# avikde/robobee3d

Measured on AMD Instinct MI355X. Metric: closed-loop MPC steps/sec (QP+dyn), higher is better.
Workload: dtype f32

## Files before the change

### robobee3d_amd/_lib.py

```python
import ctypes as C
import os
import subprocess

HERE = os.path.dirname(os.path.abspath(__file__))
ROOT = os.path.dirname(HERE)
SO_PATH = os.path.join(HERE, "libumpc_mi355x.so")
SRC = os.path.join(HERE, "csrc", "umpc_mi355x.hip")
SRC_BQP = os.path.join(HERE, "csrc", "umpc_bqp.hip")
OBJ_DIR = os.path.join(HERE, "csrc", "_obj")
HIPCC_FLAGS = ["--offload-arch=gfx950", "-O3", "-ffp-contract=off", "-fPIC", "-std=c++17"]

UMPC_F32, UMPC_F64 = 0, 1
STATE_ROWS, CTRL_ROWS, REF_ROWS, OUT_ROWS, STAT_ROWS = 18, 127, 9, 9, 2
NX, NC, NADATA = 45, 39, 48

EXPORTS = ["umpcInit", "umpcUpdate", "umpcS", "umpcLastStatus", "umpcRelease", "umpcLiveControllers", "umpcSetCompat",
           "umpcBatchDefaultParams", "umpcBatchCreate", "umpcBatchDestroy", "umpcBatchInitCtrl",
           "umpcBatchRollout", "umpcBatchUpdate", "umpcBatchPlant", "umpcBatchAssemble",
           "umpcBatchSize", "umpcBatchDtype", "umpcAxIdx", "umpcKKTPerm", "umpcNnzL",
           "umpcBatchSetTask", "umpcBatchTime", "umpcBatchSetWeights", "umpcBatchSetStepKernel", "umpcBatchSetGlobalBatch", "umpcBatchGlobalBatch", "umpcBatchReactive", "umpcBatchTaskReference",
           "umpcBatchSetRefTrajectory", "umpcBatchRefCursor", "umpcBatchTaskTable", "umpcBatchSetHistory", "umpcBatchHistoryCursor",
           "umpcBatchSetImpulses", "umpcBatchImpulseCursor",
           "umpcLastError", "umpcKernelName", "umpcBatchKernelName", "wlConInit", "wlConUpdate", "wlconS", "umpcBatchWLUpdate", "umpcBatchSetWL", "umpcBatchModel",
           "umpcQPDefaultSettings", "umpcQPCreate", "umpcQPDestroy", "umpcQPSetMaxIter", "umpcQPSetCheckTermination", "umpcQPSetAdaptiveRho", "umpcQPUseTables", "umpcQPSetKernel", "umpcQPKernelName", "umpcQPSolve", "umpcQPGather", "umpcQPGatherUpdate",
           "umpcP5fStep", "umpcP5fStepU", "umpcP5fLinearise", "umpcP5fTick", "umpcNAssemble", "umpcNExtract"]


class NParams(C.Structure):
    _fields_ = [(k, C.c_double) for k in ("dt", "g", "TtoWmax", "ws", "wds", "wpr", "wpf", "wvr", "wvf", "wthrust",
                                          "wmom")] + [("Ib", C.c_double * 3)]


class QPSettings(C.Structure):
    _fields_ = [(k, C.c_double) for k in ("rho", "sigma", "alpha", "eps_abs", "eps_rel", "eps_prim_inf",
                                          "eps_dual_inf")] + [("max_iter", C.c_int), ("scaling", C.c_int),
                                                              ("check_termination", C.c_int), ("adaptive_rho_interval", C.c_int)]


class FunApprox_t(C.Structure):
    _fields_ = [("k", C.c_int), ("a0", C.c_float), ("a1", C.c_float * 4), ("A2", C.c_float * 16)]

# ... 54 lines not shown
    limits = json.load(open(RESOURCE_LIMITS))
    for pat, lim in limits.items():
        hits = [k for k in res if pat in k]
        if not hits:
            raise RuntimeError("resource check: no kernel matches %r" % pat)
        for k in hits:
            r = res[k]
            for key, op in (("VGPRs", "=="), ("AGPRs", "=="), ("LDS", "=="), ("ScratchSize", "<=")):
                if key in lim and key not in r:
                    raise RuntimeError("resource check: %s missing for %s (hipcc remark format changed?)" % (key, k))
                if key in lim and not (r[key] == lim[key] if op == "==" else r[key] <= lim[key]):
                    raise RuntimeError("resource check failed for %s: %s = %d, recorded %s %d (csrc/resource_limits.json)"
                                       % (k, key, r[key], op, lim[key]))
    return res


def build(force=False, verbose=False):
    from . import asmgen, asmgen64, asmstep, codegen, codegen_n3, codegen_qp
    sw = asmgen.generator_switches()
    if sw and os.environ.get("UMPC_VARIANT_ROOT") != ROOT:
        raise RuntimeError("generator switches are set in the environment (%s): refusing to regenerate the shipped kernels; "
                           "unset them, or build a variant with tools/build_variant.py" % " ".join("%s=%s" % kv for kv in sw.items()))
    gen, _ = codegen.write()
    gn3 = codegen_n3.write()
    gasm, _ = asmgen.write()
    gasm64 = asmgen64.write()[0]
    gasm64q = asmgen64.write_quad()[0]
    gstep, _ = asmstep.write()
    gquad, _ = asmstep.write(quad=True)
    greg, gqp_units = codegen_qp.write()
    hdr = os.path.join(ROOT, "include", "umpc_mi355x.h")
    csrc = os.path.join(HERE, "csrc")
    units = [(SRC, [gen, gasm, gasm64, gasm64q, gstep, gquad, gn3, hdr] + [os.path.join(csrc, f) for f in ("umpc_step.h", "umpc_models.h", "umpc_err.h")]),
             (SRC_BQP, [hdr, greg, os.path.join(csrc, "umpc_bqp_common.h"), os.path.join(csrc, "umpc_err.h")])]
    gen_hdrs = [os.path.join(csrc, "gen", f) for f in os.listdir(os.path.join(csrc, "gen")) if f.endswith(".h")]
    units += [(u, [os.path.join(csrc, "umpc_bqp_common.h")] + gen_hdrs) for u in gqp_units]
    os.makedirs(OBJ_DIR, exist_ok=True)
    objs, relink = [], force or not os.path.exists(SO_PATH)
    todo = []
    for src, deps in units:
        obj = os.path.join(OBJ_DIR, os.path.basename(src) + ".o")
        objs.append(obj)
        if (force or not os.path.exists(obj)
                or any(os.path.getmtime(obj) < os.path.getmtime(d) for d in [src] + deps)):
            extra = ["-Rpass-analysis=kernel-resource-usage"] if src == SRC else []
            todo.append(["hipcc"] + HIPCC_FLAGS + extra + ["-c", "-o", obj, src])
            relink = True
    step_obj = os.path.join(OBJ_DIR, os.path.basename(SRC) + ".o")
    if not any(c[-1] == SRC for c in todo):
        import json
        try:
            _validate_resources(json.load(open(RESOURCES_JSON)))
        except Exception:
            todo.insert(0, ["hipcc"] + HIPCC_FLAGS + ["-Rpass-analysis=kernel-resource-usage", "-c", "-o", step_obj, SRC])
            relink = True
    for stale in set(os.listdir(OBJ_DIR)) - {os.path.basename(o) for o in objs} - {os.path.basename(RESOURCES_JSON)}:
        os.remove(os.path.join(OBJ_DIR, stale))
    running, width = [], max(1, min(len(todo), os.cpu_count() or 1))
    while todo or running:
        while todo and len(running) < width:
            cmd = todo.pop(0)
            if verbose:
                print(" ".join(cmd))
            running.append((cmd, subprocess.Popen(cmd, cwd=csrc, stderr=subprocess.PIPE)))
        cmd, p = running.pop(0)
        _, err = p.communicate()
        if p.returncode != 0:
# ... 84 lines not shown
        L.umpcBatchTime.argtypes = [C.c_void_p]
        L.umpcBatchTime.restype = C.c_double
        L.umpcBatchModel.argtypes = [C.c_int, C.c_int, C.c_int, C.c_int, C.c_double] + [C.c_void_p] * 4
        L.umpcBatchWLUpdate.argtypes =[C.POINTER(WLCon_t), C.c_int, C.c_int] + [C.c_void_p] * 5
        L.umpcBatchSetWL.argtypes = [C.c_void_p, C.POINTER(WLCon_t), C.POINTER(C.c_double), C.c_void_p, C.c_void_p]
        L.umpcUpdate.restype = C.c_int
        L.umpcQPDefaultSettings.argtypes = [C.POINTER(QPSettings)]
        L.umpcQPCreate.restype = C.c_void_p
        L.umpcQPCreate.argtypes = [C.c_void_p, C.c_int, C.c_int, C.c_int, C.POINTER(QPSettings)]
        L.umpcQPDestroy.argtypes = [C.c_void_p]
        L.umpcQPSetMaxIter.argtypes = [C.c_void_p, C.c_int]
        L.umpcQPSetCheckTermination.argtypes = [C.c_void_p, C.c_int]
        L.umpcQPSetAdaptiveRho.argtypes = [C.c_void_p, C.c_int]
        L.umpcQPUseTables.argtypes = [C.c_void_p, C.c_int]
        L.umpcQPSetKernel.argtypes = [C.c_void_p, C.c_int]
        L.umpcQPKernelName.argtypes = [C.c_void_p]
        L.umpcQPKernelName.restype = C.c_char_p
        L.umpcQPSolve.argtypes = [C.c_void_p] * 15
        L.umpcQPGather.argtypes = [C.c_int, C.c_int, C.c_int] + [C.c_void_p] * 5
        L.umpcQPGatherUpdate.argtypes = [C.c_int, C.c_int, C.c_int] + [C.c_void_p] * 5
        L.umpcP5fStep.argtypes = [C.c_int, C.c_int, C.c_int, C.c_double] + [C.c_void_p] * 4
        L.umpcP5fStepU.argtypes = [C.c_int, C.c_int, C.c_int, C.c_double, C.c_double] + [C.c_void_p] * 3
        L.umpcP5fLinearise.argtypes = [C.c_int, C.c_int, C.c_void_p, C.c_double, C.c_void_p, C.c_void_p, C.c_int, C.c_void_p,
                                       C.c_void_p, C.c_void_p, C.c_int, C.c_void_p]
        L.umpcP5fTick.argtypes = [C.c_void_p] * 14 + [C.c_double, C.c_double, C.c_void_p, C.c_void_p, C.c_int, C.c_void_p, C.c_void_p, C.c_void_p]
        L.umpcNAssemble.argtypes = [C.c_int, C.c_int, C.c_int, C.POINTER(NParams)] + [C.c_void_p] * 10
        L.umpcNExtract.argtypes = [C.c_int, C.c_int, C.c_int, C.c_double] + [C.c_void_p] * 5
        L.umpcLastStatus.restype = C.c_int
        L.umpcSetCompat.restype = C.c_int
        _lib = L
    return _lib


def default_params():
    p = BatchParams()
    lib().umpcBatchDefaultParams(C.byref(p))
    return p
```

### robobee3d_amd/asmgen.py

```python
import os
import struct

from . import symbolic

HERE = os.path.dirname(os.path.abspath(__file__))

SWITCH_PREFIXES = ("UMPC_ASM_", "UMPC_ASM64_", "UMPC_QP_", "UMPC_X_")
NOT_SWITCHES = ("UMPC_QP_KERNEL", "UMPC_QP_NO_ASM", "UMPC_ASM_SKEW_US", "UMPC_ASM_SKEW_GROUPS")


def generator_switches():
    return {k: v for k, v in sorted(os.environ.items()) if k.startswith(SWITCH_PREFIXES) and k not in NOT_SWITCHES}


def switch_banner():
    sw = generator_switches()
    return "// generator switches: " + (" ".join("%s=%s" % kv for kv in sw.items()) if sw else "none (defaults = the shipped kernels)")

XV_COUNT, XV_BASE = 0, 246
NLDS = 160
NVZ = 36
FAC_L, FAC_DI, FAC_Q, FAC_LOEQ, FAC_M = 0, 213, 297, 342, 378
FAC_ROWS = 390
WS_DS, WS_ES, WS_C, WS_XPREV, WS_DY = 390, 435, 474, 475, 520
WS_ROWS = 559

V_W, V_WZ, V_X, V_Y, V_Z = 2, 48, 88, 134, 174
V_RING, V_AT, V_TT, V_END = 214, 230, 238, 246
N_ATP = 4
NRING = 4


def ring_base(slot):
    return V_RING + 4 * slot if slot < 4 else 246 + 4 * (slot - 4)
A_L, A_D, A_Q, A_LO, A_M = 0, 53, 137, 182, 218
S_WS, S_CTRL, S_STRIDE, S_ITERS = 4, 6, 10, 11
S_P, S_CNT, S_P2 = 12, 14, 16
S_ALPHA, S_OMA, S_SIGMA, S_RINV, S_RHO = 20, 22, 24, 26, 28


def f32bits(v):
    return struct.unpack("<I", struct.pack("<f", v))[0]


def _vgprs(x):
    if not isinstance(x, str):
        return set()
    x = x.strip("-|")
    if x.startswith("v[") and x.endswith("]"):
        lo, hi = x[2:-1].split(":")
        return set(range(int(lo), int(hi) + 1))
    if x.startswith("v") and x[1:].isdigit():
        return {int(x[1:])}
    return set()


WIDE_STORES = {"ds_write_b128": 2, "ds_write_b96": 2, "global_store_dwordx4": 2, "global_store_dwordx3": 2}
WIDE_STORE_WAIT = 2


def valu_dst(t):
    m = t[0]
    if not m.startswith("v_") or m.startswith("v_cmp") or m in ("v_accvgpr_write_b32", "v_readfirstlane_b32", "v_readlane_b32"):
        return set()
    return _vgprs(t[1])


def wide_store_hazards(ins):
    out = []
    for k, t in enumerate(ins):
        if t[0] in WIDE_STORES:
            data = _vgprs(t[WIDE_STORES[t[0]]])
            ws, j = 0, k + 1
            while j < len(ins) and ws < WIDE_STORE_WAIT:
                u = ins[j]
                if u[0] == "label":
                    j += 1
                    continue
                if u[0] == "s_nop":
                    ws += int(u[1]) + 1
                elif valu_dst(u) & data:
                    out.append((k, j))
                    ws += 1
                else:
                    ws += 1
                j += 1
    return out


class Emit:

    def __init__(self):
        self.ins = []

    def __call__(self, *t):
        dst = valu_dst(t)
        if dst:
            ws = 0
            for u in reversed(self.ins[-(WIDE_STORE_WAIT + 1):]):
                if ws >= WIDE_STORE_WAIT or u[0] == "label":
                    break
                if u[0] in WIDE_STORES and _vgprs(u[WIDE_STORES[u[0]]]) & dst:
                    self.ins.append(("s_nop", WIDE_STORE_WAIT - ws - 1))
                    break
                ws += int(u[1]) + 1 if u[0] == "s_nop" else 1
        self.ins.append(t)


def _row_ptr(e, sreg, base, row):
    e("s_mul_i32", "s%d" % sreg, "s%d" % S_STRIDE, row)
    e("s_mul_hi_u32", "s%d" % (sreg + 1), "s%d" % S_STRIDE, row)
    e("s_add_u32", "s%d" % sreg, "s%d" % sreg, "s%d" % base)
    e("s_addc_u32", "s%d" % (sreg + 1), "s%d" % (sreg + 1), "s%d" % (base + 1))


def _adv(e, sreg):
    e("s_add_u32", "s%d" % sreg, "s%d" % sreg, "s%d" % S_STRIDE)
    e("s_addc_u32", "s%d" % (sreg + 1), "s%d" % (sreg + 1), 0)


def slot_maps(s):
    def one(n, ntrip):
        sl = list(range(n))
        for t in range(ntrip):
            st = 3 * t
            if st % 2:
                sl[st], sl[st + 1], sl[st + 2] = st + 1, st + 2, st
        return sl
    ntrip = 4 * s.N
    xs, zs = one(s.nx, ntrip), one(s.nc, ntrip)
    xinv, zinv = [0] * s.nx, [0] * s.nc
    for j, p in enumerate(xs):
# ... 110 lines not shown
    units = []
    k = 0
    while k < len(fwd):
        g = fwd[k]
        if len(g) == 1 and g[0][2] in couples and k + 1 < len(fwd) and len(fwd[k + 1]) == 1 and fwd[k + 1][0][2] == couples[g[0][2]]:
            units.append([g[0][2], fwd[k + 1][0][2]])
            k += 2
        else:
            units.append([o[2] for o in g])
            k += 1
    order, pending = [], []
    for u in units:
        if len(u) == 2 and len(order) % 2:
            pending.append(u)
            continue
        order += u
        while pending and len(order) % 2 == 0:
            order += pending.pop(0)
    assert not pending, "odd number of single entries before a trailing pair"
    pos = [0] * len(s.L_i)
    for p_, j in enumerate(order):
        pos[j] = p_
    for g in fwd + bwd:
        if len(g) == 2:
            a, b = pos[g[0][2]], pos[g[1][2]]
            assert a // 2 == b // 2, "paired entries must share an aligned pair"
    return fwd, bwd, pos


def l_positions(N=3, perm=None):
    return solve_plan(symbolic.analyse(N, perm))[2]


def prologue(e, s):
    import numpy as np
    for reg, val in ((S_ALPHA, 1.6), (S_OMA, float(np.float32(1.0) - np.float32(1.6))), (S_SIGMA, 1e-6),
                     (S_RINV, 0.01), (S_RHO, 100.0)):
        e("s_mov_b32", "s%d" % reg, f32bits(val))
        e("s_mov_b32", "s%d" % (reg + 1), f32bits(val))
    _row_ptr(e, S_P, S_WS, FAC_L + NLDS)
    nrest = len(s.L_i) - NLDS + s.nk + s.nx + 2 * s.N * symbolic.NY + 12
    assert A_LO == nrest - 12 - 2 * s.N * symbolic.NY and A_M == nrest - 12 and nrest <= 256
    for r in range(nrest):
        e("global_load_dword", "a%d" % r, "v0", "s[%d:%d]" % (S_P, S_P + 1))
        _adv(e, S_P)
    e("s_mov_b64", "s[%d:%d]" % (S_P, S_P + 1), "s[%d:%d]" % (S_CTRL, S_CTRL + 1))
    xs, zs, _, _ = slot_maps(s)
    for base, n, sl in ((V_X, s.nx, xs), (V_Y, s.nc, zs), (V_Z, s.nc, zs)):
        for r in range(n):
            e("global_load_dword", "v%d" % (base + sl[r]), "v0", "s[%d:%d]" % (S_P, S_P + 1))
            _adv(e, S_P)
    e("s_waitcnt", "vmcnt(0)")


def epilogue(e, s, z_is_l):
    w = 0
    xs, zs, _, _ = slot_maps(s)
    neq = 2 * s.N * symbolic.NY
    for base, n, sl in ((V_X, s.nx, xs), (V_Y, s.nc, zs), (V_Z, s.nc, zs)):
        for r in range(n):
            if base == V_Z and z_is_l and r < neq:
                t = V_RING + r % 16
                e("v_accvgpr_read_b32", "v%d" % t, "a%d" % (A_LO + r))
                e("ds_write_b32", "v1", "v%d" % t, (w // 4) * 1024 + (w % 4) * 4)
            else:
                e("ds_write_b32", "v1", "v%d" % (base + sl[r]), (w // 4) * 1024 + (w % 4) * 4)
            w += 1
    e("s_waitcnt", "vmcnt(0) lgkmcnt(0)")


class Fetcher:

    def __init__(self, e, la=3):
        self.e, self.la = e, la
        self.nds = 0
        self.waited = -1
        self.lds_ahead = int(os.environ.get("UMPC_ASM_LDS_AHEAD", "12" if NRING == 4 else "20"))
        self.merge = int(os.environ.get("UMPC_ASM_LDS_MERGE", "1" if NRING == 4 else "2"))

    def run(self, ops):
        e = self.e
        n = len(ops)
        inst_of = [None] * n
        insts = []
        slots = [None] * NRING
        for i, op in enumerate(ops):
            if op["src"] and op["src"][0] == "L":
                qd = op["src"][1] // 4
                hit = [k for k in slots if k is not None and insts[k]["quad"] == qd]
                if hit:
                    insts[hit[0]]["last"] = i
                    inst_of[i] = hit[0]
                    continue
                free = [sl for sl in range(NRING) if slots[sl] is None]
                sl = free[0] if free else min(range(NRING), key=lambda q: insts[slots[q]]["last"])
                insts.append(dict(quad=qd, first=i, last=i, slot=sl, prev=slots[sl], issued=None))
                slots[sl] = len(insts) - 1
                inst_of[i] = slots[sl]

        def issue(it):
            e("ds_read_b128", "v[%d:%d]" % (ring_base(it["slot"]), ring_base(it["slot"]) + 3), "v1",
              it["quad"] * 1024)
            it["issued"] = self.nds
            self.nds += 1

        next_inst = 0
        atemp = {}
        next_acc = 0
        acc_rr = 0
        for i in range(n):
            while next_acc < n and next_acc < i + self.la:
                op = ops[next_acc]
                if op["src"] and op["src"][0] in ("A", "A2"):
                    t = V_AT + 2 * (acc_rr % N_ATP)
                    acc_rr += 1
                    e("v_accvgpr_read_b32", "v%d" % t, "a%d" % op["src"][1])
                    if op["src"][0] == "A2":
                        e("v_accvgpr_read_b32", "v%d" % (t + 1), "a%d" % op["src"][2])
                    atemp[next_acc] = t
                next_acc += 1
            while next_inst < len(insts):
                it = insts[next_inst]
                prev = insts[it["prev"]] if it["prev"] is not None else None
                if it["first"] <= i + self.lds_ahead and (prev is None or prev["last"] < i):
                    issue(it)
                    next_inst += 1
                else:
                    break
            op = ops[i]
            if op["src"] is None:
                op["emit"](None)
            elif op["src"][0] in ("A", "A2"):
                op["emit"](atemp.pop(i))
            else:
                it = insts[inst_of[i]]
                if it["issued"] is None:
                    assert inst_of[i] == next_inst and (it["prev"] is None or insts[it["prev"]]["last"] < i)
                    issue(it)
                    next_inst += 1
                if it["first"] == i and it["issued"] > self.waited:
                    upto = min(self.nds - 1, it["issued"] + self.merge)
                    e("s_waitcnt", "lgkmcnt(%d)" % min(15, self.nds - 1 - upto))
                    self.waited = upto if self.nds - 1 - upto <= 15 else it["issued"]
                op["emit"](ring_base(it["slot"]) + op["src"][1] % 4)


def _vp(n):
    assert n % 2 == 0
# ... 9 lines not shown
    assert n % 2 == 0
    return ("s[%d:%d]" % (n, n + 1), 0, 0)


def pk(e, mnem, dst, srcs, neg=None):
    assert dst % 2 == 0
    neg = neg or [0] * len(srcs)
    mods = dict(op_sel=[s_[1] for s_ in srcs], op_sel_hi=[s_[2] for s_ in srcs], neg_lo=list(neg), neg_hi=list(neg))
    e(mnem, "v[%d:%d]" % (dst, dst + 1), *[s_[0] for s_ in srcs], mods)


def despace(ops, window=int(os.environ.get("UMPC_ASM_WINDOW", "12"))):
    pending, out = list(ops), []
    last = [frozenset(), frozenset()]
    while pending:
        best, bscore = 0, None
        blocked_w, blocked_r = set(), set()
        for k, o in enumerate(pending[:window]):
            movable = not (o["r"] & blocked_w) and not (o["w"] & blocked_w) and not (o["w"] & blocked_r)
            if movable:
                score = (2 if (o["r"] | o["w"]) & last[1] else 0) + (1 if (o["r"] | o["w"]) & last[0] else 0)
                if bscore is None or score < bscore:
                    best, bscore = k, score
                    if score == 0:
                        break
            blocked_w |= o["w"]
            blocked_r |= o["r"]
        o = pending.pop(best)
        out.append(o)
        last = [last[1], o["w"]]
    return out


def body(e, s, first, capture, plan, lv=False, delta_in_w=False, qzero=frozenset(), lzero=frozenset(), dy3_in_w=False):
    nx, nc, nk = s.nx, s.nc, s.nk
    neq = 2 * s.N * symbolic.NY
    xs, zs, xinv, zinv = slot_maps(s)
    fwd, bwd, lpos = plan

    def wreg(k):
        return w_reg(s, k, xs, zs)
    W = lambda k: "v%d" % wreg(k)
    WX = lambda j: V_W + xs[j]
    WZ = lambda i: V_WZ + zs[i]
    XR = lambda j: V_X + xs[j]
    YR = lambda i: V_Y + zs[i]
    ZR = lambda i: V_Z + zs[i]
    X = lambda j: "v%d" % XR(j)
    Y = lambda i: "v%d" % YR(i)
    Z = lambda i: "v%d" % ZR(i)
    v = lambda n: "v%d" % n
    sA, sO, sS, sRi, sRh = ("s%d" % r for r in (S_ALPHA, S_OMA, S_SIGMA, S_RINV, S_RHO))
    ptr = "s[%d:%d]" % (S_P2, S_P2 + 1)
    f = Fetcher(e)
    ops = []

    def op(src, fn, w=(), r=()):
        ops.append(dict(src=src, emit=fn, w=frozenset(w), r=frozenset(r)))

    assert NVZ == neq and not (lv and first)

    def l_src(j):
        if lpos[j] < NLDS:
            return ("L", lpos[j])
        if lv and lpos[j] < NLDS + NVZ:
            return ("V", V_Z + lpos[j] - NLDS)
        if NLDS + NVZ <= lpos[j] < NLDS + NVZ + XV_COUNT:
            return ("V", XV_BASE + lpos[j] - NLDS - NVZ)
        return ("A", A_L + lpos[j] - NLDS)

    if capture and not delta_in_w:
        _row_ptr(e, S_P2, S_WS, WS_XPREV)
        for j in range(nx):
            e("global_store_dword", "v0", X(j), ptr)
            _adv(e, S_P2)
    for p_ in range(0, nx - 1, 2):
        j0, j1 = xinv[p_], xinv[p_ + 1]
        rw = dict(w=(V_W + p_, V_W + p_ + 1), r=(V_X + p_, V_X + p_ + 1))
        if j0 in qzero and j1 in qzero:
            op(None, lambda t, p_=p_: pk(e, "v_pk_mul_f32", V_W + p_, [_sb(S_SIGMA), _vp(V_X + p_)]), **rw)
        elif j0 in qzero or j1 in qzero:
            jn, h = (j1, 1) if j0 in qzero else (j0, 0)

            def mixed(t, p_=p_, h=h):
                pk(e, "v_pk_mul_f32", V_W + p_, [_sb(S_SIGMA), _vp(V_X + p_)])
                e("v_sub_f32", v(V_W + p_ + h), v(V_W + p_ + h), v(t))
            op(("A", A_Q + jn), mixed, **rw)
        else:
            op(("A2", A_Q + j0, A_Q + j1),
               lambda t, p_=p_: pk(e, "v_pk_fma_f32", V_W + p_, [_sb(S_SIGMA), _vp(V_X + p_), _vp(t)], [0, 0, 1]), **rw)
    if nx % 2:
        jl = xinv[nx - 1]
        if jl in qzero:
# ... 24 lines not shown
        op(("A", A_M + 9 + i - neq), lambda t, i=i: e("v_fma_f32", v(WZ(i)), "-" + v(t), Y(i), Z(i)),
           w=(WZ(i),), r=(YR(i), ZR(i)))

    def solve_ops(sched):
        for g in sched:
            if len(g) == 1:
                d, sr, j = g[0]
                src = l_src(j)
                if src[0] == "V":
                    op(None, lambda t, d=d, sr=sr, r=src[1]: e("v_fmac_f32", W(d), v(r), W(sr)),
                       w=(wreg(d),), r=(wreg(d), wreg(sr)))
                else:
                    op(src, lambda t, d=d, sr=sr: e("v_fmac_f32", W(d), v(t), W(sr)),
                       w=(wreg(d),), r=(wreg(d), wreg(sr)))
                continue
            (d0, s0_, j0), (d1, s1_, j1) = g
            rd, r0, r1 = wreg(d0), wreg(s0_), wreg(s1_)
            assert rd % 2 == 0 and wreg(d1) == rd + 1 and r0 // 2 == r1 // 2 and lpos[j0] // 2 == lpos[j1] // 2
            srcp = ("v[%d:%d]" % (r0 - r0 % 2, r0 - r0 % 2 + 1), r0 % 2, r1 % 2)
            rw = dict(w=(rd, rd + 1), r=(rd, rd + 1, r0, r1))
            pe = lpos[j0] - lpos[j0] % 2
            lsel = (lpos[j0] % 2, lpos[j1] % 2)
            if pe < NLDS:
                op(("L", pe), lambda t, rd=rd, srcp=srcp, lsel=lsel:
                   pk(e, "v_pk_fma_f32", rd, [("v[%d:%d]" % (t, t + 1), lsel[0], lsel[1]), srcp, _vp(rd)], [0, 0, 0]), **rw)
            elif (lv and pe < NLDS + NVZ) or NLDS + NVZ <= pe < NLDS + NVZ + XV_COUNT:
                t = V_Z + pe - NLDS if pe < NLDS + NVZ else XV_BASE + pe - NLDS - NVZ
                op(None, lambda _t, t=t, rd=rd, srcp=srcp, lsel=lsel:
                   pk(e, "v_pk_fma_f32", rd, [("v[%d:%d]" % (t, t + 1), lsel[0], lsel[1]), srcp, _vp(rd)], [0, 0, 0]), **rw)
            else:
                src = ("A2", A_L + lpos[j0] - NLDS, A_L + lpos[j1] - NLDS)
                op(src, lambda t, rd=rd, srcp=srcp: pk(e, "v_pk_fma_f32", rd, [_vp(t), srcp, _vp(rd)], [0, 0, 0]), **rw)

    solve_ops(fwd)
    kof = {wreg(k): k for k in range(nk)}
    for r0 in range(V_W, V_Z, 2):
        k0, k1 = kof.get(r0), kof.get(r0 + 1)
        if k0 is not None and k1 is not None:
            op(("A2", A_D + k0, A_D + k1), lambda t, r0=r0: pk(e, "v_pk_mul_f32", r0, [_vp(r0), _vp(t)]),
               w=(r0, r0 + 1), r=(r0, r0 + 1))
        elif k0 is not None or k1 is not None:
            k, r = (k0, r0) if k0 is not None else (k1, r0 + 1)
            op(("A", A_D + k), lambda t, r=r: e("v_mul_f32", v(r), v(t), v(r)), w=(r,), r=(r,))
    solve_ops(bwd)
    f.run(despace(ops) if os.environ.get("UMPC_ASM_DESPACE", "0") == "1" else ops)
    for p_ in range(0, nx - 1, 2):
        t = V_TT + 2 * ((p_ // 2) % 4)
        pk(e, "v_pk_mul_f32", t, [_sb(S_OMA), _vp(V_X + p_)])
        if capture and delta_in_w:
            pk(e, "v_pk_fma_f32", t, [_sb(S_ALPHA), _vp(V_W + p_), _vp(t)])
            pk(e, "v_pk_add_f32", V_W + p_, [_vp(t), _vp(V_X + p_)], [0, 1])
            e("v_pk_mov_b32", "v[%d:%d]" % (V_X + p_, V_X + p_ + 1), "v[%d:%d]" % (t, t + 1), "v[%d:%d]" % (t, t + 1),
              dict(op_sel=[0, 1], op_sel_hi=[0, 0], neg_lo=[0, 0], neg_hi=[0, 0]))
        else:
            pk(e, "v_pk_fma_f32", V_X + p_, [_sb(S_ALPHA), _vp(V_W + p_), _vp(t)])
    if nx % 2:
        jl = xinv[nx - 1]
        e("v_mul_f32", v(V_TT), sO, X(jl))
        if capture and delta_in_w:
            e("v_fma_f32", v(V_TT), sA, v(WX(jl)), v(V_TT))
            e("v_sub_f32", v(WX(jl)), v(V_TT), X(jl))
            e("v_mov_b32", X(jl), v(V_TT))
        else:
            e("v_fma_f32", X(jl), sA, v(WX(jl)), v(V_TT))
    if capture and first and not delta_in_w:
        _row_ptr(e, S_P2, S_WS, WS_DY)
    if not first:
        for p_ in range(0, neq, 2):
            t = V_TT + 2 * ((p_ // 2) % 2)
            pk(e, "v_pk_add_f32", t, [_vp(V_WZ + p_), _vp(V_Y + p_)], [0, 1])
            if capture and delta_in_w:
                pk(e, "v_pk_mul_f32", V_WZ + p_, [_sb(S_ALPHA), _vp(t)])
            elif capture:
                pk(e, "v_pk_mul_f32", t + 4, [_sb(S_ALPHA), _vp(t)])
                for h in range(2):
                    _row_ptr(e, S_P2, S_WS, WS_DY + zinv[p_ + h])
                    e("global_store_dword", "v0", v(t + 4 + h), ptr)
            pk(e, "v_pk_fma_f32", V_Y + p_, [_sb(S_ALPHA), _vp(t), _vp(V_Y + p_)])
# ... 27 lines not shown
            e("v_fma_f32", t3, rinv, Y(i), t1)
            e("v_max_f32", t3, t3, v(V_AT + 2))
            e("v_min_f32", Z(i), t3, v(V_AT + 3))
            e("v_sub_f32", t2, t1, Z(i))
        if dy3_in_w and not eq and not capture:
            e("v_mul_f32", nu, rho, t2)
            e("v_add_f32", Y(i), Y(i), nu)
            continue
        e("v_mul_f32", t2, rho, t2)
        e("v_add_f32", Y(i), Y(i), t2)
        if capture and delta_in_w:
            e("v_mov_b32", nu, t2)
        elif capture:
            if not first:
                _row_ptr(e, S_P2, S_WS, WS_DY + i)
            e("global_store_dword", "v0", t2, ptr)
            if first:
                _adv(e, S_P2)


def program(N=3, perm=None):
    s = symbolic.analyse(N, perm)
    plan = solve_plan(s)
    e = Emit()
    prologue(e, s)
    e("s_cmp_lt_i32", "s%d" % S_ITERS, 1)
    e("s_cbranch_scc1", "9f")
    body(e, s, first=True, capture=True, plan=plan)
    for p_ in range(NVZ):
        e("v_accvgpr_read_b32", "v%d" % (V_Z + p_), "a%d" % (A_L + p_))
    e("s_sub_i32", "s%d" % S_CNT, "s%d" % S_ITERS, 2)
    e("s_cmp_lt_i32", "s%d" % S_CNT, 1)
    e("s_cbranch_scc1", "8f")
    e("label", "7")
    body(e, s, first=False, capture=False, plan=plan, lv=True)
    e("s_sub_i32", "s%d" % S_CNT, "s%d" % S_CNT, 1)
    e("s_cmp_gt_i32", "s%d" % S_CNT, 0)
    e("s_cbranch_scc1", "7b")
    e("label", "8")
    e("s_cmp_lt_i32", "s%d" % S_ITERS, 2)
    e("s_cbranch_scc1", "6f")
    body(e, s, first=False, capture=True, plan=plan, lv=True)
    e("label", "6")
    epilogue(e, s, z_is_l=True)
    e("s_branch", "5f")
    e("label", "9")
    epilogue(e, s, z_is_l=False)
    e("label", "5")
    return e.ins, s


def fmt(t):
    m = t[0]
    if m == "label":
        return "%s:" % t[1]
    mods = ""
    if isinstance(t[-1], dict):
        d = t[-1]
        t = t[:-1]
        mods = " " + " ".join("%s:[%s]" % (k, ",".join(map(str, d[k]))) for k in ("op_sel", "op_sel_hi", "neg_lo", "neg_hi"))
    a = [("0x%x" % x if (m == "s_mov_b32" and isinstance(x, int)) else str(x)) for x in t[1:]]
    if m in ("ds_read_b128", "ds_write_b128", "ds_write_b32"):
        return "%s %s, %s offset:%s" % (m, a[0], a[1], a[2])
    if m in ("global_load_dword", "global_store_dword"):
        return "%s %s, %s, %s" % (m, a[0], a[1], a[2])
    if m == "s_waitcnt":
        return "s_waitcnt " + " ".join(a)
    return "%s %s%s" % (m, ", ".join(a), mods)


def write(path=None, N=3, perm=None):
    path = path or os.path.join(HERE, "csrc", "umpc_admm_asm.h")
    ins, s = program(N, perm)
    lpos = solve_plan(s)[2]
    store_l = " ".join("LDSW_(%d) = -LX_(%d);" % (lpos[j], j) if lpos[j] < NLDS else "ROW_(%d) = -LX_(%d);" % (FAC_L + lpos[j], j)
                       for j in range(len(lpos)))
    used_s = [S_P, S_P + 1, S_CNT, S_P2, S_P2 + 1] + list(range(S_ALPHA, S_RHO + 2))
    clob = ['"memory"', '"scc"', '"vcc"'] + ['"v%d"' % i for i in range(2, V_END)] + \
           ['"a%d"' % i for i in range(256)] + ['"s%d"' % i for i in used_s]
    lab7 = [k for k, t in enumerate(ins) if t == ("label", "7")][0]
    lab8 = [k for k, t in enumerate(ins) if t == ("label", "8")][0]
    out = ["// GENERATED by robobee3d_amd/asmgen.py -- do not edit.", switch_banner(),
           "// ADMM phase of the fp32 step kernel: %d instructions, middle-iteration body %d." % (len(ins), lab8 - lab7),
           "#pragma once",
           "namespace umpcasm {",
           "constexpr int FAC_L = %d, FAC_DI = %d, FAC_Q = %d, FAC_LOEQ = %d, FAC_M = %d, FAC_ROWS = %d;" %
           (FAC_L, FAC_DI, FAC_Q, FAC_LOEQ, FAC_M, FAC_ROWS),
           "constexpr int WS_DS = %d, WS_ES = %d, WS_C = %d, WS_XPREV = %d, WS_DY = %d, WS_ROWS = %d;" %
           (WS_DS, WS_ES, WS_C, WS_XPREV, WS_DY, WS_ROWS),
           "constexpr int LDS_BYTES_PER_LANE = %d;" % (NLDS * 4),
           "}  // namespace umpcasm",
           "// Phase A -> loop hand-off of the factor: entry j of L (CSC order) goes NEGATED to its storage position (asmgen.solve_plan):",
           "// LDS word LDSW_(p) for p < %d, workspace row ROW_(FAC_L + p) (-> AGPR) otherwise." % NLDS,
           "#define UMPC_ASM_STORE_L(LDSW_, ROW_, LX_) do { %s } while (0)" % store_l,
           "// inputs: v0 = 4*robot, v1 = lane LDS address, s[4:5] = workspace, s[6:7] = ctrl, s10 = 4*B, s11 = maxIter",
           "#define UMPC_ADMM_ASM(voff, ldsaddr, ws, ctrl, stride, iters) asm volatile( \\"]
    for t in ins:
        out.append('  "%s\\n" \\' % fmt(t))
    out.append('  : : "{v0}"(voff), "{v1}"(ldsaddr), "{s[4:5]}"(ws), "{s[6:7]}"(ctrl), "{s10}"(stride), "{s11}"(iters) \\')
    out.append("  : " + ", ".join(clob) + ")")
    txt = "\n".join(out) + "\n"
    old = open(path).read() if os.path.exists(path) else None
    if old != txt:
        with open(path, "w") as fh:
            fh.write(txt)
    return path, len(ins)
# ... 19 lines not shown
```

### robobee3d_amd/asmstep.py

```python
import os
import struct

from . import asmgen, symbolic
from .asmgen import (A_D, A_L, A_LO, A_M, A_Q, NLDS, NVZ, S_ALPHA, S_CNT, S_ITERS, S_OMA, S_RHO, S_RINV, S_SIGMA,
                     V_W, V_WZ, V_X, V_Y, V_Z, Emit, f32bits, pk, _sb, _vp)

HERE = os.path.dirname(os.path.abspath(__file__))

PTRS = ["state", "ctrl", "ref", "ws", "out", "stats", "status", "info", "Ib", "gain", "aT0",
        "taskf", "weights", "wl", "wlu", "wlw",
        "done"]
NPTR_RES = 11
INTS = ["stride", "K", "maxIter", "nsub", "plant", "seq"]
TAIL_INTS = ["refstep"]
FLOATS = ["dt", "dtg", "Tmax", "wpr", "wpf", "ws_", "wvr", "wvf", "wds", "wthrust", "wmom",
          "iwpr", "iwpf", "iws", "iwvr", "iwvf", "iwds", "iwthrust", "iwmom",
          "Ib0", "Ib1", "Ib2", "Ibi0", "Ibi1", "Ibi2", "h", "hh", "h6", "taulim", "gpl", "idt", "mbg"]
WNAMES = ["wpr", "wpf", "ws_", "wvr", "wvf", "wds", "wthrust", "wmom"]
WROW = {"ws_": 0, "wds": 1, "wpr": 2, "wpf": 3, "wvr": 4, "wvf": 5, "wthrust": 6, "wmom": 7}
A_W, A_IW = 230, 238
S_PARAM = 4
S_PBLK = 2
S_PTR = {n: 40 + 2 * k for k, n in enumerate(PTRS[:NPTR_RES])}
S_PTR["taskf"], S_PTR["weights"] = 0, 96
S_PTR["wl"], S_PTR["wlu"], S_PTR["wlw"] = 30, 32, 34
S_INT = {"stride": 10, "K": 13, "maxIter": S_ITERS, "nsub": 5, "plant": 39}
S_F = {n: 64 + k for k, n in enumerate(FLOATS)}
assert max(S_F.values()) <= 95
S_STEP, S_SUB, S_RUIZ = 12, 15, 15
S_MBAD, S_MP0 = 62, 14
S_M0, S_M1, S_M2, S_M3 = 30, 32, 34, 36
S_C = {"minscal": 16, "maxscal": 17, "c45": 18, "eps10": 19, "eps": 38, "rho": 6, "rinv": 7, "rmin": 8,
       "rmininv": 9, "infty_ms": 100, "rhotol": 101}
S_TMP = 4
OFF = {}
_o = 0
for _n in PTRS:
    OFF[_n] = _o
    _o += 8
for _n in INTS + FLOATS + TAIL_INTS:
    OFF[_n] = _o
    _o += 4
PARAM_BYTES = _o
HIST_INTS = ["statestep", "outstep", "statusstep", "infostep"]
HIST_OFF = (PARAM_BYTES + 7) // 8 * 8
for _k, _n in enumerate(HIST_INTS):
    OFF[_n] = HIST_OFF + 4 * _k
HIST_BYTES = 4 * len(HIST_INTS)
S_HIST = 32
IMP_OFF = HIST_OFF + HIST_BYTES
assert IMP_OFF % 8 == 0
OFF["imp"], OFF["impstep"] = IMP_OFF, IMP_OFF + 8
IMP_BYTES = 16
S_IMP = 32

VFIRST, VEND = 2, 256
XV_N, XV_B = 10, 246
OPT_RING = int(os.environ.get("UMPC_ASM_RING", "6"))
assert OPT_RING in (4, 6)
OPT_XV = os.environ.get("UMPC_ASM_XV", "1") == "1"
if OPT_RING == 6:
    XV_N, XV_B = 2, 254
OPT_LIMIT_FAST = os.environ.get("UMPC_ASM_LIMIT_FAST", "0") == "1"
OPT_ZSKIP = os.environ.get("UMPC_ASM_ZSKIP", "1") == "1"
OPT_NT = os.environ.get("UMPC_ASM_NT", "1")
NT_PTRS = ("state", "ctrl", "ref", "out", "stats")
# ... 882 lines not shown
                e("v_mul_f32", v(t), v(src[i]), v(RE(i)))
                e("v_accvgpr_write_b32", "a%d" % (A_LO + i), v(t))
            elif i == 5 * 6 + 2:
                e("v_mul_f32", v(t), SF("dtg"), v(RE(i)))
                e("v_accvgpr_write_b32", "a%d" % (A_LO + i), v(t))
            else:
                e("v_accvgpr_write_b32", "a%d" % (A_LO + i), v(zero))
        for k in range(N):
            e("v_mul_f32", v(t), v(LS + 15), v(RE(neq + k)))
            e("v_accvgpr_write_b32", "a%d" % (A_M + k), v(t))
            e("v_mul_f32", v(t), v(LS + 16), v(RE(neq + k)))
            e("v_accvgpr_write_b32", "a%d" % (A_M + N + k), v(t))
        pool.free(zero, t)
        pool.free_range(LS, 20)
        pool.free_range(self.VE, nc + 1)
        pool.free_range(self.VQ, st.nq + st.nq % 2)

    def factor(self):
        e, pool, st, s = self.e, self.pool, self.st, self.s
        nx, nc, nk, neq = s.nx, s.nc, s.nk, st.neq
        RP, RA = self.RP, self.RA
        lpos = st.lpos
        last_row = {}
        for c in range(nk):
            if s.L_p[c + 1] > s.L_p[c]:
                last_row[c] = s.L_i[s.L_p[c + 1] - 1]
        done_at = {}
        for c, r in last_row.items():
            done_at.setdefault(r, []).append(c)
        nL, Dinv = {}, {}
        asmgen.XV_COUNT, asmgen.XV_BASE = (XV_N if OPT_XV and not self.quad else 0), XV_B
        pool.reserve(246, 10)
        t = pool.get()

        def retire_dinv(k):
            e("v_accvgpr_write_b32", "a%d" % (A_D + k), v(Dinv[k]))
            pool.free(Dinv.pop(k))

        def retire_col(c):
            for j in range(s.L_p[c], s.L_p[c + 1]):
                pos = lpos[j]
                if pos < NLDS:
                    e("ds_write_b32", "v1", v(nL[j]), (pos // 4) * 1024 + (pos % 4) * 4)
                elif NLDS + NVZ <= pos < NLDS + NVZ + asmgen.XV_COUNT:
                    e("v_mov_b32", v(XV_B + pos - NLDS - NVZ), v(nL[j]))
                else:
                    e("v_accvgpr_write_b32", "a%d" % (A_L + pos - NLDS), v(nL[j]))
                pool.free(nL.pop(j))
            retire_dinv(c)

        for op in s.factor_ops:
            k = op["k"]
            src = s.K_src[op["diag"]]
            dk = pool.get()
            if src[0] == 'P':
                e("v_add_f32", v(dk), sg(S_SIGMA), v(RP(src[1])))
                pool.free(RP(src[1]))
            else:
                assert src[0] == 'R'
                i = src[1]
                if i < neq:
                    e("v_mul_f32", v(dk), -1.0, self._vconst_rinv())
                else:
                    e("v_accvgpr_read_b32", v(dk), "a%d" % (A_M + 9 + i - neq))
                    e("s_nop", 0)
                    e("v_mul_f32", v(dk), -1.0, v(dk))
            y = {}
            for (b, p) in op["init"]:
                assert s.K_src[p][0] == 'A'
                y[b] = (RA(s.K_src[p][1]), False)
            for (c, upd, new) in op["elim"]:
                yc, owned = y.pop(c)
                for (lj, row) in upd:
                    if row in y:
                        reg, own = y[row]
                        if own:
                            e("v_fmac_f32", v(reg), v(nL[lj]), v(yc))
                        else:
                            nr = pool.get()
                            e("v_fma_f32", v(nr), v(nL[lj]), v(yc), v(reg))
                            pool.free(reg)
                            y[row] = (nr, True)
                    else:
                        nr = pool.get()
                        e("v_mul_f32", v(nr), v(nL[lj]), v(yc))
                        y[row] = (nr, True)
                nl = pool.get()
                e("v_mul_f32", v(nl), "-" + v(yc), v(Dinv[c]))
                e("v_fmac_f32", v(dk), v(yc), v(nl))
                nL[new] = nl
                pool.free(yc)
            assert not y
            di = pool.get()
            self.rcp_nr(di, dk, t)
            pool.free(dk)
            Dinv[k] = di
            for c in done_at.get(k, []):
                retire_col(c)
            if k not in last_row:
                retire_dinv(k)
        assert not nL and not Dinv
        pool.free(t)
        if self._rinv_reg is not None:
            pool.free(self._rinv_reg)
            self._rinv_reg = None
        if st.na % 2:
            pool.free(self.VA + st.na)
        pool.free(self.VP + nx)

    _rinv_reg = None

    def _vconst_rinv(self):
        if self._rinv_reg is None:
            self._rinv_reg = self.pool.get()
            self.e("v_mov_b32", v(self._rinv_reg), sg(S_RINV))
        return v(self._rinv_reg)

    def admm(self):
        e, pool, st, s = self.e, self.pool, self.st, self.s
        nx, nc = s.nx, s.nc
        left = set(range(VFIRST, VEND)) - pool.free_ - set(range(246, 256))
        assert not left, "phase A leaked registers: %s" % sorted(left)
        pool.reserve(V_W, V_X - V_W)
        pool.reserve(V_X, V_Y - V_X)
        pool.reserve(V_Y, V_Z - V_Y)
        pool.reserve(V_Z, 40)
        voff = 245
        self.load_rows("ctrl", 0, [V_X + st.xs[r] for r in range(nx)] + [V_Y + st.zs[r] for r in range(nc)] +
                       [V_Z + st.zs[r] for r in range(nc)], voff)
        for pad in (V_X + nx, V_Y + nc, V_Z + nc, V_W + nx, V_WZ + nc):
            e("v_mov_b32", v(pad), 0)
        e("s_waitcnt", "vmcnt(0) lgkmcnt(0)")
        plan = st.plan
        zk = dict(qzero=st.qzero, lzero=st.lzero) if OPT_ZSKIP else {}
        asmgen.body(e, s, first=True, capture=True, plan=plan, delta_in_w=True, **zk)
        if self.quad:
            from . import asmquad
            lab6 = self.label()
            e("s_cmp_lt_i32", sg(S_ITERS), 2)
            e("s_cbranch_scc1", lab6 + "f")
            asmquad.section(e, asmquad.QuadPlan(st), self.label)
            e("label", lab6)
        else:
            self._admm_rest(plan, zk)
        for i in range(st.neq):
            pool.free(V_Z + st.zs[i], kill=True)
        pool.free_range(246, 10)


    def _admm_rest(self, plan, zk):
        e, s, st = self.e, self.s, self.st
        import numpy as np
        for p_ in range(NVZ):
            e("v_accvgpr_read_b32", v(V_Z + p_), "a%d" % (A_L + p_))
        lab7, lab6 = self.label(), self.label()
        e("s_sub_i32", sg(S_CNT), sg(S_ITERS), 1)
        e("s_cmp_lt_i32", sg(S_CNT), 1)
        e("s_cbranch_scc1", lab6 + "f")
        e("label", lab7)
        asmgen.body(e, s, first=False, capture=False, plan=plan, lv=True, dy3_in_w=True, **zk)
        e("s_sub_i32", sg(S_CNT), sg(S_CNT), 1)
        e("s_cmp_gt_i32", sg(S_CNT), 0)
        e("s_cbranch_scc1", lab7 + "b")
        k = float(np.float32(1.6) / (np.float32(1.6) - np.float32(1.0)))
        e("s_mov_b32", sg(S_TMP), f32bits(k))
        nx, neq = s.nx, st.neq
        for p_ in range(0, nx - 1, 2):
            pk(e, "v_pk_add_f32", V_W + p_, [P2(V_X + p_), P2(V_W + p_)], [0, 1])
        for p_ in range(0, nx - 1, 2):
            pk(e, "v_pk_mul_f32", V_W + p_, [PS(S_TMP), P2(V_W + p_)])
        if nx % 2:
            jl = st.xinv[nx - 1]
            e("v_sub_f32", v(V_W + st.xs[jl]), v(V_X + st.xs[jl]), v(V_W + st.xs[jl]))
            e("v_mul_f32", v(V_W + st.xs[jl]), sg(S_TMP), v(V_W + st.xs[jl]))
        for p_ in range(0, neq, 2):
            pk(e, "v_pk_add_f32", V_WZ + p_, [P2(V_Y + p_), P2(V_WZ + p_)], [0, 1])
        for p_ in range(0, neq, 2):
            pk(e, "v_pk_mul_f32", V_WZ + p_, [PS(S_TMP), P2(V_WZ + p_)])
        e("label", lab6)

    def phase_c(self):
        e, pool, st, s = self.e, self.pool, self.st, self.s
        N, NYv = s.N, symbolic.NY
        nx, nc, neq = s.nx, s.nc, st.neq
        SF = lambda n: sg(S_F[n])
        g_ = pool.get
        XR = lambda j: V_X + st.xs[j]
        YR = lambda i: V_Y + st.zs[i]
        ZR = lambda i: V_Z + st.zs[i]
        DXR = lambda j: V_W + st.xs[j]
        DYR = lambda i: V_WZ + st.zs[i]
        voff = g_()
        def slot_blocks(n, chunk=16):
            n2 = n + n % 2
            blocks = [(lo, pool.getn(min(chunk, n2 - lo))) for lo in range(0, n2, chunk)]
            def reg(slot):
# ... 933 lines not shown
                "static_assert(offsetof(StepArgs, i) == %d && sizeof(StepImp) == %d && offsetof(StepImp, impstep) == 8, \"StepImp layout\");" % (IMP_OFF, IMP_BYTES),
                "constexpr int STEP_LDS_BYTES_PER_LANE = %d;" % (NLDS * 4), "}  // namespace umpcasm",
                "// inputs: v0 = 4 * robot, v1 = lane LDS address, s[4:5] = &StepParams (kernarg)",
                "#define UMPC_STEP_ASM(voff, ldsaddr, params) asm volatile( \\"]
    for t in ins:
        out.append('  "%s\\n" \\' % fmt(t))
    out.append('  : : "{v0}"(voff), "{v1}"(ldsaddr), "{s[4:5]}"(params) \\')
    out.append("  : " + ", ".join(clob) + ")")
    txt = "\n".join(out) + "\n"
    old = open(path).read() if os.path.exists(path) else None
    if old != txt:
        with open(path, "w") as fh:
            fh.write(txt)
    return path, len(ins)


_KEEP_V = {0, 1} | set(range(V_W, V_Z)) | set(range(V_Z + 2 * 3 * symbolic.NY, V_Z + 40))
QUAD = {None: None}


def _quad():
    from . import isasim
    if QUAD[None] is None:
        QUAD.update({None: isasim.Quad(v=_KEEP_V, dead_v=set(range(256)) - _KEEP_V, a=range(A_LO, 256), dead_a=range(A_LO)),
                     "ruiz": isasim.Quad(a=range(256)), "plant": isasim.Quad(a=range(256))})
    return QUAD


FLAT = ("taskf", "wl")
STRIDE = 4096
PBASE = 0x00007E0080000000


def simulate(ins, arrays, ints, floats, max_exec=3000000, ptr_xform=None):
    import numpy as np
    from . import isasim
    base_of = {n: 0x00007F0080000000 + (k << 36) for k, n in enumerate(PTRS + ["impulse"])}
    ptr_xform = ptr_xform or (lambda a: a)
    blob = bytearray(IMP_OFF + IMP_BYTES)
    for n in PTRS:
        struct.pack_into("<Q", blob, OFF[n], ptr_xform(base_of[n]) if arrays.get(n) is not None else 0)
    allints = dict(ints, stride=STRIDE)
    allints.setdefault("seq", 0)
    allints.setdefault("refstep", 0)
    for n in HIST_INTS:
        allints.setdefault(n, 0)
    for n in INTS + TAIL_INTS + HIST_INTS:
        struct.pack_into("<i", blob, OFF[n], int(allints[n]))
    for n in FLOATS:
        struct.pack_into("<f", blob, OFF[n], float(floats[n]))
    allints.setdefault("impstep", 6 * STRIDE if arrays.get("impulse") is not None else 0)
    struct.pack_into("<Q", blob, OFF["imp"], ptr_xform(base_of["impulse"]) if arrays.get("impulse") is not None else 0)
    struct.pack_into("<i", blob, OFF["impstep"], int(allints["impstep"]))
    regions = [(PBASE, 4, np.frombuffer(bytes(blob), np.uint32))] + \
        [(base_of[n], 4 if n in FLAT else STRIDE, arrays[n]) for n in PTRS + ["impulse"] if arrays.get(n) is not None]
    m = isasim.Machine(ins, regions=regions, sgpr={S_PARAM: PBASE & 0xFFFFFFFF, S_PARAM + 1: PBASE >> 32}, vgpr={0: 0},
                       lds=np.zeros((1, NLDS), np.uint32), max_exec=max_exec, quad=_quad())
    isasim.run(m)
    simulate.last_quad_sections = {("admm" if k is None else k): n for k, n in m.sections.items()}
    simulate.last_quad_instructions = sum(m.sections.values())
    return m.nexec


if __name__ == "__main__":
    p, n = write()
    print("wrote", p, n, "instructions")


def host_floats(dt=5.0, g=9.81e-3, TtoWmax=2.0, ws=1e1, wds=1e3, wpr=1.0, wpf=5.0, wvr=1e3, wvf=2e3, wthrust=1e-1, wmom=1e-2,
                Ib=(3333.0, 3333.0, 1000.0), dtsim=0.2, taulim=100.0, mb=100.0):
    import numpy as np
    f = np.float32
    one = f(1.0)
    w = dict(wpr=f(wpr), wpf=f(wpf), ws_=f(ws), wvr=f(wvr), wvf=f(wvf), wds=f(wds), wthrust=f(wthrust), wmom=f(wmom))
    d = dict(dt=f(dt), dtg=f(f(dt) * f(g)), Tmax=f(f(TtoWmax) * f(g)), **w)
    for k, val in w.items():
        d["i" + k.rstrip("_")] = f(one / val)
    for i in range(3):
        d["Ib%d" % i] = f(Ib[i])
        d["Ibi%d" % i] = f(one / f(Ib[i]))
    d.update(h=f(dtsim), hh=f(f(0.5) * f(dtsim)), h6=f(f(dtsim) / f(6.0)), taulim=f(taulim), gpl=f(9.81e-3), idt=f(one / f(dt)),
             mbg=f(f(mb) * f(g)))
    assert set(d) == set(FLOATS), set(FLOATS) ^ set(d)
    return {k: float(val) for k, val in d.items()}
```

### robobee3d_amd/csrc/umpc_admm_asm.h

```cpp
#pragma once
namespace umpcasm {
constexpr int FAC_L = 0, FAC_DI = 213, FAC_Q = 297, FAC_LOEQ = 342, FAC_M = 378, FAC_ROWS = 390;
constexpr int WS_DS = 390, WS_ES = 435, WS_C = 474, WS_XPREV = 475, WS_DY = 520, WS_ROWS = 559;
constexpr int LDS_BYTES_PER_LANE = 640;
}
#define UMPC_ASM_STORE_L(LDSW_, ROW_, LX_) do { LDSW_(0) = -LX_(0); LDSW_(1) = -LX_(1); LDSW_(2) = -LX_(2); LDSW_(4) = -LX_(3); LDSW_(5) = -LX_(4); LDSW_(3) = -LX_(5); LDSW_(62) = -LX_(6); LDSW_(63) = -LX_(7); LDSW_(64) = -LX_(8); LDSW_(6) = -LX_(9); LDSW_(8) = -LX_(10); LDSW_(7) = -LX_(11); LDSW_(9) = -LX_(12); LDSW_(65) = -LX_(13); LDSW_(66) = -LX_(14); LDSW_(10) = -LX_(15); LDSW_(12) = -LX_(16); LDSW_(11) = -LX_(17); LDSW_(13) = -LX_(18); LDSW_(14) = -LX_(19); LDSW_(16) = -LX_(20); LDSW_(18) = -LX_(21); LDSW_(20) = -LX_(22); LDSW_(19) = -LX_(23); LDSW_(21) = -LX_(24); LDSW_(15) = -LX_(25); LDSW_(17) = -LX_(26); LDSW_(22) = -LX_(27); LDSW_(24) = -LX_(28); LDSW_(23) = -LX_(29); LDSW_(25) = -LX_(30); LDSW_(26) = -LX_(31); LDSW_(28) = -LX_(32); LDSW_(30) = -LX_(33); LDSW_(32) = -LX_(34); LDSW_(31) = -LX_(35); LDSW_(33) = -LX_(36); LDSW_(27) = -LX_(37); LDSW_(29) = -LX_(38); LDSW_(86) = -LX_(39); LDSW_(88) = -LX_(40); LDSW_(87) = -LX_(41); LDSW_(89) = -LX_(42); LDSW_(85) = -LX_(43); LDSW_(90) = -LX_(44); LDSW_(34) = -LX_(45); LDSW_(36) = -LX_(46); LDSW_(35) = -LX_(47); LDSW_(37) = -LX_(48); LDSW_(91) = -LX_(49); LDSW_(67) = -LX_(50); LDSW_(92) = -LX_(51); LDSW_(94) = -LX_(52); LDSW_(93) = -LX_(53); LDSW_(95) = -LX_(54); LDSW_(96) = -LX_(55); LDSW_(98) = -LX_(56); LDSW_(100) = -LX_(57); LDSW_(102) = -LX_(58); LDSW_(101) = -LX_(59); LDSW_(103) = -LX_(60); LDSW_(97) = -LX_(61); LDSW_(99) = -LX_(62); LDSW_(38) = -LX_(63); LDSW_(68) = -LX_(64); LDSW_(39) = -LX_(65); LDSW_(69) = -LX_(66); LDSW_(70) = -LX_(67); LDSW_(71) = -LX_(68); LDSW_(40) = -LX_(69); LDSW_(42) = -LX_(70); LDSW_(44) = -LX_(71); LDSW_(114) = -LX_(72); LDSW_(116) = -LX_(73); LDSW_(118) = -LX_(74); LDSW_(136) = -LX_(75); LDSW_(146) = -LX_(76); LDSW_(138) = -LX_(77); LDSW_(41) = -LX_(78); LDSW_(43) = -LX_(79); LDSW_(45) = -LX_(80); LDSW_(115) = -LX_(81); LDSW_(117) = -LX_(82); LDSW_(119) = -LX_(83); LDSW_(137) = -LX_(84); LDSW_(147) = -LX_(85); LDSW_(139) = -LX_(86); LDSW_(46) = -LX_(87); LDSW_(48) = -LX_(88); LDSW_(50) = -LX_(89); LDSW_(130) = -LX_(90); LDSW_(120) = -LX_(91); LDSW_(122) = -LX_(92); LDSW_(140) = -LX_(93); LDSW_(148) = -LX_(94); LDSW_(149) = -LX_(95); LDSW_(52) = -LX_(96); LDSW_(54) = -LX_(97); LDSW_(56) = -LX_(98); LDSW_(53) = -LX_(99); LDSW_(55) = -LX_(100); LDSW_(57) = -LX_(101); LDSW_(47) = -LX_(102); LDSW_(49) = -LX_(103); LDSW_(51) = -LX_(104); LDSW_(124) = -LX_(105); LDSW_(126) = -LX_(106); LDSW_(128) = -LX_(107); LDSW_(104) = -LX_(108); LDSW_(106) = -LX_(109); LDSW_(108) = -LX_(110); LDSW_(125) = -LX_(111); LDSW_(127) = -LX_(112); LDSW_(129) = -LX_(113); LDSW_(105) = -LX_(114); LDSW_(107) = -LX_(115); LDSW_(109) = -LX_(116); LDSW_(131) = -LX_(117); LDSW_(121) = -LX_(118); LDSW_(123) = -LX_(119); LDSW_(132) = -LX_(120); LDSW_(133) = -LX_(121); LDSW_(141) = -LX_(122); LDSW_(155) = -LX_(123); ROW_(162) = -LX_(124); LDSW_(156) = -LX_(125); ROW_(163) = -LX_(126); ROW_(164) = -LX_(127); LDSW_(157) = -LX_(128); ROW_(165) = -LX_(129); ROW_(166) = -LX_(130); ROW_(183) = -LX_(131); LDSW_(72) = -LX_(132); LDSW_(73) = -LX_(133); LDSW_(74) = -LX_(134); LDSW_(75) = -LX_(135); LDSW_(76) = -LX_(136); LDSW_(77) = -LX_(137); LDSW_(58) = -LX_(138); LDSW_(61) = -LX_(139); LDSW_(78) = -LX_(140); LDSW_(60) = -LX_(141); LDSW_(59) = -LX_(142); LDSW_(79) = -LX_(143); LDSW_(112) = -LX_(144); LDSW_(113) = -LX_(145); LDSW_(110) = -LX_(146); ROW_(170) = -LX_(147); ROW_(171) = -LX_(148); ROW_(172) = -LX_(149); ROW_(173) = -LX_(150); ROW_(174) = -LX_(151); ROW_(175) = -LX_(152); ROW_(176) = -LX_(153); ROW_(177) = -LX_(154); ROW_(178) = -LX_(155); ROW_(180) = -LX_(156); ROW_(179) = -LX_(157); ROW_(182) = -LX_(158); ROW_(181) = -LX_(159); ROW_(184) = -LX_(160); ROW_(185) = -LX_(161); ROW_(186) = -LX_(162); LDSW_(80) = -LX_(163); LDSW_(81) = -LX_(164); LDSW_(111) = -LX_(165); LDSW_(82) = -LX_(166); LDSW_(83) = -LX_(167); LDSW_(84) = -LX_(168); LDSW_(134) = -LX_(169); LDSW_(142) = -LX_(170); LDSW_(135) = -LX_(171); LDSW_(144) = -LX_(172); LDSW_(150) = -LX_(173); LDSW_(158) = -LX_(174); ROW_(160) = -LX_(175); LDSW_(151) = -LX_(176); LDSW_(152) = -LX_(177); LDSW_(143) = -LX_(178); LDSW_(153) = -LX_(179); LDSW_(154) = -LX_(180); LDSW_(145) = -LX_(181); ROW_(167) = -LX_(182); LDSW_(159) = -LX_(183); ROW_(168) = -LX_(184); ROW_(161) = -LX_(185); ROW_(169) = -LX_(186); ROW_(187) = -LX_(187); ROW_(188) = -LX_(188); ROW_(189) = -LX_(189); ROW_(190) = -LX_(190); ROW_(191) = -LX_(191); ROW_(192) = -LX_(192); ROW_(193) = -LX_(193); ROW_(196) = -LX_(194); ROW_(199) = -LX_(195); ROW_(194) = -LX_(196); ROW_(195) = -LX_(197); ROW_(200) = -LX_(198); ROW_(198) = -LX_(199); ROW_(197) = -LX_(200); ROW_(201) = -LX_(201); ROW_(202) = -LX_(202); ROW_(203) = -LX_(203); ROW_(204) = -LX_(204); ROW_(205) = -LX_(205); ROW_(206) = -LX_(206); ROW_(207) = -LX_(207); ROW_(208) = -LX_(208); ROW_(209) = -LX_(209); ROW_(210) = -LX_(210); ROW_(211) = -LX_(211); ROW_(212) = -LX_(212); } while (0)
#define UMPC_ADMM_ASM(voff, ldsaddr, ws, ctrl, stride, iters) asm volatile( \
  "s_mov_b32 s20, 0x3fcccccd\n" \
  "s_mov_b32 s21, 0x3fcccccd\n" \
  "s_mov_b32 s22, 0xbf19999a\n" \
  "s_mov_b32 s23, 0xbf19999a\n" \
  "s_mov_b32 s24, 0x358637bd\n" \
  "s_mov_b32 s25, 0x358637bd\n" \
  "s_mov_b32 s26, 0x3c23d70a\n" \
  "s_mov_b32 s27, 0x3c23d70a\n" \
  "s_mov_b32 s28, 0x42c80000\n" \
  "s_mov_b32 s29, 0x42c80000\n" \
  "s_mul_i32 s12, s10, 160\n" \
  "s_mul_hi_u32 s13, s10, 160\n" \
  "s_add_u32 s12, s12, s4\n" \
  "s_addc_u32 s13, s13, s5\n" \
  "global_load_dword a0, v0, s[12:13]\n" \
  "s_add_u32 s12, s12, s10\n" \
  "s_addc_u32 s13, s13, 0\n" \
// ... 2445 lines not shown
  "v_accvgpr_read_b32 v180, a6\n" \
  "v_accvgpr_read_b32 v181, a7\n" \
  "v_accvgpr_read_b32 v182, a8\n" \
  "v_accvgpr_read_b32 v183, a9\n" \
  "v_accvgpr_read_b32 v184, a10\n" \
  "v_accvgpr_read_b32 v185, a11\n" \
  "v_accvgpr_read_b32 v186, a12\n" \
  "v_accvgpr_read_b32 v187, a13\n" \
  "v_accvgpr_read_b32 v188, a14\n" \
  "v_accvgpr_read_b32 v189, a15\n" \
  "v_accvgpr_read_b32 v190, a16\n" \
  "v_accvgpr_read_b32 v191, a17\n" \
  "v_accvgpr_read_b32 v192, a18\n" \
  "v_accvgpr_read_b32 v193, a19\n" \
  "v_accvgpr_read_b32 v194, a20\n" \
  "v_accvgpr_read_b32 v195, a21\n" \
  "v_accvgpr_read_b32 v196, a22\n" \
  "v_accvgpr_read_b32 v197, a23\n" \
  "v_accvgpr_read_b32 v198, a24\n" \
  "v_accvgpr_read_b32 v199, a25\n" \
  "v_accvgpr_read_b32 v200, a26\n" \
  "v_accvgpr_read_b32 v201, a27\n" \
  "v_accvgpr_read_b32 v202, a28\n" \
  "v_accvgpr_read_b32 v203, a29\n" \
  "v_accvgpr_read_b32 v204, a30\n" \
  "v_accvgpr_read_b32 v205, a31\n" \
  "v_accvgpr_read_b32 v206, a32\n" \
  "v_accvgpr_read_b32 v207, a33\n" \
  "v_accvgpr_read_b32 v208, a34\n" \
  "v_accvgpr_read_b32 v209, a35\n" \
  "s_sub_i32 s14, s11, 2\n" \
  "s_cmp_lt_i32 s14, 1\n" \
  "s_cbranch_scc1 8f\n" \
  "7:\n" \
  "v_accvgpr_read_b32 v230, a137\n" \
  "v_accvgpr_read_b32 v231, a138\n" \
  "v_accvgpr_read_b32 v232, a139\n" \
  "v_accvgpr_read_b32 v233, a142\n" \
  "v_accvgpr_read_b32 v234, a140\n" \
  "v_accvgpr_read_b32 v235, a141\n" \
  "v_pk_fma_f32 v[2:3], s[24:25], v[88:89], v[230:231] op_sel:[0,0,0] op_sel_hi:[0,1,1] neg_lo:[0,0,1] neg_hi:[0,0,1]\n" \
  "v_accvgpr_read_b32 v236, a143\n" \
  "v_accvgpr_read_b32 v237, a144\n" \
  "v_pk_fma_f32 v[4:5], s[24:25], v[90:91], v[232:233] op_sel:[0,0,0] op_sel_hi:[0,1,1] neg_lo:[0,0,1] neg_hi:[0,0,1]\n" \
  "v_accvgpr_read_b32 v230, a145\n" \
  "v_accvgpr_read_b32 v231, a148\n" \
  "v_pk_fma_f32 v[6:7], s[24:25], v[92:93], v[234:235] op_sel:[0,0,0] op_sel_hi:[0,1,1] neg_lo:[0,0,1] neg_hi:[0,0,1]\n" \
  "v_accvgpr_read_b32 v232, a146\n" \
  "v_accvgpr_read_b32 v233, a147\n" \
  "v_pk_fma_f32 v[8:9], s[24:25], v[94:95], v[236:237] op_sel:[0,0,0] op_sel_hi:[0,1,1] neg_lo:[0,0,1] neg_hi:[0,0,1]\n" \
  "v_accvgpr_read_b32 v234, a149\n" \
  "v_accvgpr_read_b32 v235, a150\n" \
  "v_pk_fma_f32 v[10:11], s[24:25], v[96:97], v[230:231] op_sel:[0,0,0] op_sel_hi:[0,1,1] neg_lo:[0,0,1] neg_hi:[0,0,1]\n" \
  "v_accvgpr_read_b32 v236, a151\n" \
  "v_accvgpr_read_b32 v237, a154\n" \
  "v_pk_fma_f32 v[12:13], s[24:25], v[98:99], v[232:233] op_sel:[0,0,0] op_sel_hi:[0,1,1] neg_lo:[0,0,1] neg_hi:[0,0,1]\n" \
  "v_accvgpr_read_b32 v230, a152\n" \
  "v_accvgpr_read_b32 v231, a153\n" \
  "v_pk_fma_f32 v[14:15], s[24:25], v[100:101], v[234:235] op_sel:[0,0,0] op_sel_hi:[0,1,1] neg_lo:[0,0,1] neg_hi:[0,0,1]\n" \
  "v_accvgpr_read_b32 v232, a155\n" \
  "v_accvgpr_read_b32 v233, a156\n" \
  "v_pk_fma_f32 v[16:17], s[24:25], v[102:103], v[236:237] op_sel:[0,0,0] op_sel_hi:[0,1,1] neg_lo:[0,0,1] neg_hi:[0,0,1]\n" \
  "v_accvgpr_read_b32 v234, a157\n" \
  "v_accvgpr_read_b32 v235, a160\n" \
  "v_pk_fma_f32 v[18:19], s[24:25], v[104:105], v[230:231] op_sel:[0,0,0] op_sel_hi:[0,1,1] neg_lo:[0,0,1] neg_hi:[0,0,1]\n" \
  "v_accvgpr_read_b32 v236, a158\n" \
// ... 36 lines not shown
  "v_pk_fma_f32 v[44:45], s[24:25], v[130:131], v[232:233] op_sel:[0,0,0] op_sel_hi:[0,1,1] neg_lo:[0,0,1] neg_hi:[0,0,1]\n" \
  "v_accvgpr_read_b32 v230, a184\n" \
  "v_accvgpr_read_b32 v231, a187\n" \
  "v_fma_f32 v46, s24, v132, -v234\n" \
  "v_accvgpr_read_b32 v232, a185\n" \
  "v_accvgpr_read_b32 v233, a186\n" \
  "v_pk_fma_f32 v[48:49], s[26:27], v[134:135], v[236:237] op_sel:[0,0,0] op_sel_hi:[0,1,1] neg_lo:[1,0,0] neg_hi:[1,0,0]\n" \
  "v_accvgpr_read_b32 v234, a188\n" \
  "v_accvgpr_read_b32 v235, a189\n" \
  "v_pk_fma_f32 v[50:51], s[26:27], v[136:137], v[230:231] op_sel:[0,0,0] op_sel_hi:[0,1,1] neg_lo:[1,0,0] neg_hi:[1,0,0]\n" \
  "v_accvgpr_read_b32 v236, a190\n" \
  "v_accvgpr_read_b32 v237, a193\n" \
  "v_pk_fma_f32 v[52:53], s[26:27], v[138:139], v[232:233] op_sel:[0,0,0] op_sel_hi:[0,1,1] neg_lo:[1,0,0] neg_hi:[1,0,0]\n" \
  "v_accvgpr_read_b32 v230, a191\n" \
  "v_accvgpr_read_b32 v231, a192\n" \
  "v_pk_fma_f32 v[54:55], s[26:27], v[140:141], v[234:235] op_sel:[0,0,0] op_sel_hi:[0,1,1] neg_lo:[1,0,0] neg_hi:[1,0,0]\n" \
  "v_accvgpr_read_b32 v232, a194\n" \
  "v_accvgpr_read_b32 v233, a195\n" \
  "v_pk_fma_f32 v[56:57], s[26:27], v[142:143], v[236:237] op_sel:[0,0,0] op_sel_hi:[0,1,1] neg_lo:[1,0,0] neg_hi:[1,0,0]\n" \
  "v_accvgpr_read_b32 v234, a196\n" \
  "v_accvgpr_read_b32 v235, a199\n" \
  "v_pk_fma_f32 v[58:59], s[26:27], v[144:145], v[230:231] op_sel:[0,0,0] op_sel_hi:[0,1,1] neg_lo:[1,0,0] neg_hi:[1,0,0]\n" \
  "v_accvgpr_read_b32 v236, a197\n" \
  "v_accvgpr_read_b32 v237, a198\n" \
  "v_pk_fma_f32 v[60:61], s[26:27], v[146:147], v[232:233] op_sel:[0,0,0] op_sel_hi:[0,1,1] neg_lo:[1,0,0] neg_hi:[1,0,0]\n" \
  "v_accvgpr_read_b32 v230, a200\n" \
  "v_accvgpr_read_b32 v231, a201\n" \
  "v_pk_fma_f32 v[62:63], s[26:27], v[148:149], v[234:235] op_sel:[0,0,0] op_sel_hi:[0,1,1] neg_lo:[1,0,0] neg_hi:[1,0,0]\n" \
  "v_accvgpr_read_b32 v232, a202\n" \
  "v_accvgpr_read_b32 v233, a205\n" \
  "v_pk_fma_f32 v[64:65], s[26:27], v[150:151], v[236:237] op_sel:[0,0,0] op_sel_hi:[0,1,1] neg_lo:[1,0,0] neg_hi:[1,0,0]\n" \
  "v_accvgpr_read_b32 v234, a203\n" \
  "v_accvgpr_read_b32 v235, a204\n" \
  "ds_read_b128 v[214:217], v1 offset:0\n" \
  "v_pk_fma_f32 v[66:67], s[26:27], v[152:153], v[230:231] op_sel:[0,0,0] op_sel_hi:[0,1,1] neg_lo:[1,0,0] neg_hi:[1,0,0]\n" \
  "v_accvgpr_read_b32 v236, a206\n" \
  "v_accvgpr_read_b32 v237, a207\n" \
  "v_pk_fma_f32 v[68:69], s[26:27], v[154:155], v[232:233] op_sel:[0,0,0] op_sel_hi:[0,1,1] neg_lo:[1,0,0] neg_hi:[1,0,0]\n" \
  "v_accvgpr_read_b32 v230, a208\n" \
  "v_accvgpr_read_b32 v231, a211\n" \
  "ds_read_b128 v[218:221], v1 offset:1024\n" \
  "v_pk_fma_f32 v[70:71], s[26:27], v[156:157], v[234:235] op_sel:[0,0,0] op_sel_hi:[0,1,1] neg_lo:[1,0,0] neg_hi:[1,0,0]\n" \
  "v_accvgpr_read_b32 v232, a209\n" \
  "v_accvgpr_read_b32 v233, a210\n" \
  "v_pk_fma_f32 v[72:73], s[26:27], v[158:159], v[236:237] op_sel:[0,0,0] op_sel_hi:[0,1,1] neg_lo:[1,0,0] neg_hi:[1,0,0]\n" \
  "v_accvgpr_read_b32 v234, a212\n" \
  "v_accvgpr_read_b32 v235, a213\n" \
  "ds_read_b128 v[222:225], v1 offset:2048\n" \
  "v_pk_fma_f32 v[74:75], s[26:27], v[160:161], v[230:231] op_sel:[0,0,0] op_sel_hi:[0,1,1] neg_lo:[1,0,0] neg_hi:[1,0,0]\n" \
  "v_accvgpr_read_b32 v236, a214\n" \
  "v_accvgpr_read_b32 v237, a217\n" \
  "v_pk_fma_f32 v[76:77], s[26:27], v[162:163], v[232:233] op_sel:[0,0,0] op_sel_hi:[0,1,1] neg_lo:[1,0,0] neg_hi:[1,0,0]\n" \
  "v_accvgpr_read_b32 v230, a215\n" \
  "v_accvgpr_read_b32 v231, a216\n" \
  "ds_read_b128 v[226:229], v1 offset:3072\n" \
  "v_pk_fma_f32 v[78:79], s[26:27], v[164:165], v[234:235] op_sel:[0,0,0] op_sel_hi:[0,1,1] neg_lo:[1,0,0] neg_hi:[1,0,0]\n" \
  "v_accvgpr_read_b32 v232, a227\n" \
  "v_pk_fma_f32 v[80:81], s[26:27], v[166:167], v[236:237] op_sel:[0,0,0] op_sel_hi:[0,1,1] neg_lo:[1,0,0] neg_hi:[1,0,0]\n" \
  "v_accvgpr_read_b32 v234, a228\n" \
  "v_pk_fma_f32 v[82:83], s[26:27], v[168:169], v[230:231] op_sel:[0,0,0] op_sel_hi:[0,1,1] neg_lo:[1,0,0] neg_hi:[1,0,0]\n" \
  "v_accvgpr_read_b32 v236, a229\n" \
  "v_fma_f32 v84, -v232, v170, v210\n" \
  "v_fma_f32 v85, -v234, v171, v211\n" \
  "v_fma_f32 v86, -v236, v172, v212\n" \
  "s_waitcnt lgkmcnt(2)\n" \
  "v_pk_fma_f32 v[60:61], v[214:215], v[14:15], v[60:61] op_sel:[0,0,0] op_sel_hi:[1,1,1] neg_lo:[0,0,0] neg_hi:[0,0,0]\n" \
  "v_pk_fma_f32 v[62:63], v[216:217], v[16:17], v[62:63] op_sel:[0,0,0] op_sel_hi:[1,1,1] neg_lo:[0,0,0] neg_hi:[0,0,0]\n" \
  "ds_read_b128 v[214:217], v1 offset:4096\n" \
  "v_pk_fma_f32 v[64:65], v[218:219], v[18:19], v[64:65] op_sel:[0,0,0] op_sel_hi:[1,1,1] neg_lo:[0,0,0] neg_hi:[0,0,0]\n" \
  "v_pk_fma_f32 v[48:49], v[220:221], v[2:3], v[48:49] op_sel:[0,0,0] op_sel_hi:[1,1,1] neg_lo:[0,0,0] neg_hi:[0,0,0]\n" \
  "ds_read_b128 v[218:221], v1 offset:5120\n" \
  "s_waitcnt lgkmcnt(2)\n" \
  "v_pk_fma_f32 v[54:55], v[222:223], v[2:3], v[54:55] op_sel:[0,0,0] op_sel_hi:[1,1,1] neg_lo:[0,0,0] neg_hi:[0,0,0]\n" \
  "v_pk_fma_f32 v[60:61], v[224:225], v[8:9], v[60:61] op_sel:[0,0,0] op_sel_hi:[1,1,1] neg_lo:[0,0,0] neg_hi:[0,0,0]\n" \
  "ds_read_b128 v[222:225], v1 offset:6144\n" \
  "v_pk_fma_f32 v[54:55], v[226:227], v[8:9], v[54:55] op_sel:[0,0,0] op_sel_hi:[1,1,1] neg_lo:[0,0,0] neg_hi:[0,0,0]\n" \
  "v_pk_fma_f32 v[62:63], v[228:229], v[10:11], v[62:63] op_sel:[0,0,0] op_sel_hi:[1,1,1] neg_lo:[0,0,0] neg_hi:[0,0,0]\n" \
  "ds_read_b128 v[226:229], v1 offset:7168\n" \
  "s_waitcnt lgkmcnt(2)\n" \
  "v_pk_fma_f32 v[56:57], v[214:215], v[10:11], v[56:57] op_sel:[0,0,0] op_sel_hi:[1,1,1] neg_lo:[0,0,0] neg_hi:[0,0,0]\n" \
  "v_pk_fma_f32 v[64:65], v[216:217], v[12:13], v[64:65] op_sel:[0,0,0] op_sel_hi:[1,1,1] neg_lo:[0,0,0] neg_hi:[0,0,0]\n" \
  "ds_read_b128 v[214:217], v1 offset:8192\n" \
  "v_pk_fma_f32 v[58:59], v[218:219], v[12:13], v[58:59] op_sel:[0,0,0] op_sel_hi:[1,1,1] neg_lo:[0,0,0] neg_hi:[0,0,0]\n" \
  "v_pk_fma_f32 v[60:61], v[220:221], v[32:33], v[60:61] op_sel:[0,0,0] op_sel_hi:[1,1,1] neg_lo:[0,0,0] neg_hi:[0,0,0]\n" \
  "ds_read_b128 v[218:221], v1 offset:9216\n" \
  "s_waitcnt lgkmcnt(2)\n" \
  "v_pk_fma_f32 v[78:79], v[222:223], v[32:33], v[78:79] op_sel:[0,0,0] op_sel_hi:[1,1,1] neg_lo:[0,0,0] neg_hi:[0,0,0]\n" \
  "v_pk_fma_f32 v[62:63], v[224:225], v[34:35], v[62:63] op_sel:[0,0,0] op_sel_hi:[1,1,1] neg_lo:[0,0,0] neg_hi:[0,0,0]\n" \
  "ds_read_b128 v[222:225], v1 offset:10240\n" \
  "v_pk_fma_f32 v[80:81], v[226:227], v[34:35], v[80:81] op_sel:[0,0,0] op_sel_hi:[1,1,1] neg_lo:[0,0,0] neg_hi:[0,0,0]\n" \
  "v_pk_fma_f32 v[64:65], v[228:229], v[36:37], v[64:65] op_sel:[0,0,0] op_sel_hi:[1,1,1] neg_lo:[0,0,0] neg_hi:[0,0,0]\n" \
  "ds_read_b128 v[226:229], v1 offset:11264\n" \
  "s_waitcnt lgkmcnt(2)\n" \
  "v_pk_fma_f32 v[82:83], v[214:215], v[36:37], v[82:83] op_sel:[0,0,0] op_sel_hi:[1,1,1] neg_lo:[0,0,0] neg_hi:[0,0,0]\n" \
  "v_pk_fma_f32 v[24:25], v[216:217], v[52:53], v[24:25] op_sel:[0,0,0] op_sel_hi:[1,1,1] neg_lo:[0,0,0] neg_hi:[0,0,0]\n" \
  "ds_read_b128 v[214:217], v1 offset:12288\n" \
  "v_pk_fma_f32 v[6:7], v[218:219], v[52:53], v[6:7] op_sel:[0,0,0] op_sel_hi:[1,1,1] neg_lo:[0,0,0] neg_hi:[0,0,0]\n" \
  "v_pk_fma_f32 v[20:21], v[220:221], v[66:67], v[20:21] op_sel:[0,0,0] op_sel_hi:[1,1,1] neg_lo:[0,0,0] neg_hi:[0,0,0]\n" \
  "ds_read_b128 v[218:221], v1 offset:13312\n" \
  "s_waitcnt lgkmcnt(2)\n" \
  "v_pk_fma_f32 v[54:55], v[222:223], v[26:27], v[54:55] op_sel:[0,0,0] op_sel_hi:[1,1,1] neg_lo:[0,0,0] neg_hi:[0,0,0]\n" \
  "v_pk_fma_f32 v[72:73], v[224:225], v[26:27], v[72:73] op_sel:[0,0,0] op_sel_hi:[1,1,1] neg_lo:[0,0,0] neg_hi:[0,0,0]\n" \
  "ds_read_b128 v[222:225], v1 offset:14336\n" \
  "v_pk_fma_f32 v[78:79], v[226:227], v[26:27], v[78:79] op_sel:[0,0,0] op_sel_hi:[1,1,1] neg_lo:[0,0,0] neg_hi:[0,0,0]\n" \
  "v_pk_fma_f32 v[56:57], v[228:229], v[28:29], v[56:57] op_sel:[0,0,0] op_sel_hi:[1,1,1] neg_lo:[0,0,0] neg_hi:[0,0,0]\n" \
// ... 133 lines not shown
  "v_fmac_f32 v80, v190, v41\n" \
  "v_fmac_f32 v79, v191, v78\n" \
  "v_fmac_f32 v80, v192, v78\n" \
  "v_pk_fma_f32 v[6:7], v[194:195], v[78:79], v[6:7] op_sel:[0,0,0] op_sel_hi:[1,1,1] neg_lo:[0,0,0] neg_hi:[0,0,0]\n" \
  "v_fmac_f32 v80, v193, v79\n" \
  "v_fmac_f32 v6, v196, v79\n" \
  "v_fmac_f32 v80, v197, v74\n" \
  "v_fmac_f32 v5, v198, v80\n" \
  "v_fmac_f32 v6, v199, v80\n" \
  "v_fmac_f32 v7, v200, v80\n" \
  "v_fmac_f32 v6, v201, v5\n" \
  "v_fmac_f32 v7, v202, v5\n" \
  "v_fmac_f32 v69, v203, v5\n" \
  "v_fmac_f32 v75, v204, v5\n" \
  "v_fmac_f32 v81, v205, v5\n" \
  "v_fmac_f32 v7, v206, v6\n" \
  "v_fmac_f32 v69, v207, v6\n" \
  "v_accvgpr_read_b32 v230, a36\n" \
  "v_accvgpr_read_b32 v231, a37\n" \
  "v_fmac_f32 v75, v208, v6\n" \
  "v_accvgpr_read_b32 v232, a38\n" \
  "v_accvgpr_read_b32 v233, a39\n" \
  "v_fmac_f32 v81, v209, v6\n" \
  "v_accvgpr_read_b32 v234, a40\n" \
  "v_pk_fma_f32 v[76:77], v[230:231], v[6:7], v[76:77] op_sel:[0,0,0] op_sel_hi:[1,1,1] neg_lo:[0,0,0] neg_hi:[0,0,0]\n" \
  "v_accvgpr_read_b32 v236, a41\n" \
  "v_pk_fma_f32 v[76:77], v[232:233], v[6:7], v[76:77] op_sel:[0,1,0] op_sel_hi:[1,0,1] neg_lo:[0,0,0] neg_hi:[0,0,0]\n" \
  "v_accvgpr_read_b32 v230, a42\n" \
  "v_fmac_f32 v69, v234, v7\n" \
  "v_accvgpr_read_b32 v232, a43\n" \
  "v_fmac_f32 v75, v236, v7\n" \
  "v_accvgpr_read_b32 v234, a44\n" \
  "v_fmac_f32 v81, v230, v7\n" \
  "v_accvgpr_read_b32 v236, a45\n" \
  "v_fmac_f32 v76, v232, v69\n" \
  "v_accvgpr_read_b32 v230, a46\n" \
  "v_fmac_f32 v77, v234, v69\n" \
  "v_accvgpr_read_b32 v232, a47\n" \
  "v_fmac_f32 v75, v236, v69\n" \
  "v_accvgpr_read_b32 v234, a48\n" \
  "v_fmac_f32 v81, v230, v69\n" \
  "v_accvgpr_read_b32 v236, a49\n" \
  "v_fmac_f32 v77, v232, v76\n" \
  "v_accvgpr_read_b32 v230, a50\n" \
  "v_fmac_f32 v75, v234, v76\n" \
  "v_accvgpr_read_b32 v232, a51\n" \
  "v_fmac_f32 v81, v236, v76\n" \
  "v_accvgpr_read_b32 v234, a52\n" \
  "v_fmac_f32 v75, v230, v77\n" \
  "v_accvgpr_read_b32 v236, a62\n" \
  "v_accvgpr_read_b32 v237, a63\n" \
  "v_fmac_f32 v81, v232, v77\n" \
  "v_accvgpr_read_b32 v230, a64\n" \
  "v_accvgpr_read_b32 v231, a129\n" \
  "v_fmac_f32 v81, v234, v75\n" \
  "v_accvgpr_read_b32 v232, a130\n" \
  "v_accvgpr_read_b32 v233, a131\n" \
  "v_pk_mul_f32 v[2:3], v[2:3], v[236:237] op_sel:[0,0] op_sel_hi:[1,1] neg_lo:[0,0] neg_hi:[0,0]\n" \
  "v_accvgpr_read_b32 v234, a65\n" \
  "v_accvgpr_read_b32 v235, a66\n" \
  "v_pk_mul_f32 v[4:5], v[4:5], v[230:231] op_sel:[0,0] op_sel_hi:[1,1] neg_lo:[0,0] neg_hi:[0,0]\n" \
  "v_accvgpr_read_b32 v236, a67\n" \
  "v_accvgpr_read_b32 v237, a70\n" \
  "v_pk_mul_f32 v[6:7], v[6:7], v[232:233] op_sel:[0,0] op_sel_hi:[1,1] neg_lo:[0,0] neg_hi:[0,0]\n" \
  "v_accvgpr_read_b32 v230, a68\n" \
  "v_accvgpr_read_b32 v231, a69\n" \
  "v_pk_mul_f32 v[8:9], v[8:9], v[234:235] op_sel:[0,0] op_sel_hi:[1,1] neg_lo:[0,0] neg_hi:[0,0]\n" \
  "v_accvgpr_read_b32 v232, a53\n" \
  "v_accvgpr_read_b32 v233, a54\n" \
  "v_pk_mul_f32 v[10:11], v[10:11], v[236:237] op_sel:[0,0] op_sel_hi:[1,1] neg_lo:[0,0] neg_hi:[0,0]\n" \
  "v_accvgpr_read_b32 v234, a55\n" \
  "v_accvgpr_read_b32 v235, a58\n" \
  "v_pk_mul_f32 v[12:13], v[12:13], v[230:231] op_sel:[0,0] op_sel_hi:[1,1] neg_lo:[0,0] neg_hi:[0,0]\n" \
  "v_accvgpr_read_b32 v236, a56\n" \
  "v_accvgpr_read_b32 v237, a57\n" \
  "v_pk_mul_f32 v[14:15], v[14:15], v[232:233] op_sel:[0,0] op_sel_hi:[1,1] neg_lo:[0,0] neg_hi:[0,0]\n" \
  "v_accvgpr_read_b32 v230, a94\n" \
  "v_accvgpr_read_b32 v231, a97\n" \
  "v_pk_mul_f32 v[16:17], v[16:17], v[234:235] op_sel:[0,0] op_sel_hi:[1,1] neg_lo:[0,0] neg_hi:[0,0]\n" \
  "v_accvgpr_read_b32 v232, a100\n" \
  "v_accvgpr_read_b32 v233, a109\n" \
  "v_pk_mul_f32 v[18:19], v[18:19], v[236:237] op_sel:[0,0] op_sel_hi:[1,1] neg_lo:[0,0] neg_hi:[0,0]\n" \
  "v_accvgpr_read_b32 v234, a105\n" \
  "v_accvgpr_read_b32 v235, a107\n" \
  "v_pk_mul_f32 v[20:21], v[20:21], v[230:231] op_sel:[0,0] op_sel_hi:[1,1] neg_lo:[0,0] neg_hi:[0,0]\n" \
  "v_accvgpr_read_b32 v236, a92\n" \
  "v_accvgpr_read_b32 v237, a95\n" \
  "v_pk_mul_f32 v[22:23], v[22:23], v[232:233] op_sel:[0,0] op_sel_hi:[1,1] neg_lo:[0,0] neg_hi:[0,0]\n" \
// ... 55 lines not shown
  "v_pk_mul_f32 v[60:61], v[60:61], v[230:231] op_sel:[0,0] op_sel_hi:[1,1] neg_lo:[0,0] neg_hi:[0,0]\n" \
  "v_accvgpr_read_b32 v236, a89\n" \
  "v_accvgpr_read_b32 v237, a90\n" \
  "v_pk_mul_f32 v[62:63], v[62:63], v[232:233] op_sel:[0,0] op_sel_hi:[1,1] neg_lo:[0,0] neg_hi:[0,0]\n" \
  "v_accvgpr_read_b32 v230, a91\n" \
  "v_accvgpr_read_b32 v231, a132\n" \
  "v_pk_mul_f32 v[64:65], v[64:65], v[234:235] op_sel:[0,0] op_sel_hi:[1,1] neg_lo:[0,0] neg_hi:[0,0]\n" \
  "v_accvgpr_read_b32 v232, a125\n" \
  "v_accvgpr_read_b32 v233, a127\n" \
  "v_pk_mul_f32 v[66:67], v[66:67], v[236:237] op_sel:[0,0] op_sel_hi:[1,1] neg_lo:[0,0] neg_hi:[0,0]\n" \
  "v_accvgpr_read_b32 v234, a110\n" \
  "v_accvgpr_read_b32 v235, a111\n" \
  "v_pk_mul_f32 v[68:69], v[68:69], v[230:231] op_sel:[0,0] op_sel_hi:[1,1] neg_lo:[0,0] neg_hi:[0,0]\n" \
  "v_accvgpr_read_b32 v236, a112\n" \
  "v_accvgpr_read_b32 v237, a135\n" \
  "v_pk_mul_f32 v[70:71], v[70:71], v[232:233] op_sel:[0,0] op_sel_hi:[1,1] neg_lo:[0,0] neg_hi:[0,0]\n" \
  "v_accvgpr_read_b32 v230, a133\n" \
  "v_accvgpr_read_b32 v231, a134\n" \
  "v_pk_mul_f32 v[72:73], v[72:73], v[234:235] op_sel:[0,0] op_sel_hi:[1,1] neg_lo:[0,0] neg_hi:[0,0]\n" \
  "v_accvgpr_read_b32 v232, a120\n" \
  "v_accvgpr_read_b32 v233, a121\n" \
  "v_pk_mul_f32 v[74:75], v[74:75], v[236:237] op_sel:[0,0] op_sel_hi:[1,1] neg_lo:[0,0] neg_hi:[0,0]\n" \
  "v_accvgpr_read_b32 v234, a122\n" \
  "v_accvgpr_read_b32 v235, a136\n" \
  "v_pk_mul_f32 v[76:77], v[76:77], v[230:231] op_sel:[0,0] op_sel_hi:[1,1] neg_lo:[0,0] neg_hi:[0,0]\n" \
  "v_accvgpr_read_b32 v236, a126\n" \
  "v_accvgpr_read_b32 v237, a128\n" \
  "v_pk_mul_f32 v[78:79], v[78:79], v[232:233] op_sel:[0,0] op_sel_hi:[1,1] neg_lo:[0,0] neg_hi:[0,0]\n" \
  "v_accvgpr_read_b32 v230, a59\n" \
  "v_accvgpr_read_b32 v231, a60\n" \
  "v_pk_mul_f32 v[80:81], v[80:81], v[234:235] op_sel:[0,0] op_sel_hi:[1,1] neg_lo:[0,0] neg_hi:[0,0]\n" \
  "v_accvgpr_read_b32 v232, a61\n" \
  "v_pk_mul_f32 v[82:83], v[82:83], v[236:237] op_sel:[0,0] op_sel_hi:[1,1] neg_lo:[0,0] neg_hi:[0,0]\n" \
  "v_accvgpr_read_b32 v234, a52\n" \
  "v_pk_mul_f32 v[84:85], v[84:85], v[230:231] op_sel:[0,0] op_sel_hi:[1,1] neg_lo:[0,0] neg_hi:[0,0]\n" \
  "v_accvgpr_read_b32 v236, a51\n" \
  "v_mul_f32 v86, v232, v86\n" \
  "v_accvgpr_read_b32 v230, a50\n" \
  "v_fmac_f32 v75, v234, v81\n" \
  "v_accvgpr_read_b32 v232, a49\n" \
  "v_fmac_f32 v77, v236, v81\n" \
  "v_accvgpr_read_b32 v234, a48\n" \
  "v_fmac_f32 v77, v230, v75\n" \
  "v_accvgpr_read_b32 v236, a47\n" \
  "v_fmac_f32 v76, v232, v81\n" \
  "v_accvgpr_read_b32 v230, a46\n" \
  "v_fmac_f32 v76, v234, v75\n" \
  "v_accvgpr_read_b32 v232, a45\n" \
  "v_fmac_f32 v76, v236, v77\n" \
  "v_accvgpr_read_b32 v234, a44\n" \
  "v_fmac_f32 v69, v230, v81\n" \
  "v_accvgpr_read_b32 v236, a43\n" \
  "v_fmac_f32 v69, v232, v75\n" \
  "v_accvgpr_read_b32 v230, a42\n" \
  "v_fmac_f32 v69, v234, v77\n" \
  "v_accvgpr_read_b32 v232, a41\n" \
  "v_fmac_f32 v69, v236, v76\n" \
  "v_accvgpr_read_b32 v234, a40\n" \
  "v_fmac_f32 v7, v230, v81\n" \
  "v_accvgpr_read_b32 v236, a39\n" \
  "v_accvgpr_read_b32 v237, a38\n" \
  "v_fmac_f32 v7, v232, v75\n" \
  "v_accvgpr_read_b32 v230, a36\n" \
  "v_accvgpr_read_b32 v231, a37\n" \
  "v_fmac_f32 v7, v234, v69\n" \
  "v_pk_fma_f32 v[6:7], v[236:237], v[76:77], v[6:7] op_sel:[0,1,0] op_sel_hi:[1,0,1] neg_lo:[0,0,0] neg_hi:[0,0,0]\n" \
  "v_pk_fma_f32 v[6:7], v[230:231], v[76:77], v[6:7] op_sel:[0,0,0] op_sel_hi:[1,1,1] neg_lo:[0,0,0] neg_hi:[0,0,0]\n" \
  "v_fmac_f32 v6, v209, v81\n" \
  "v_fmac_f32 v6, v208, v75\n" \
  "v_fmac_f32 v6, v207, v69\n" \
  "v_fmac_f32 v6, v206, v7\n" \
  "v_fmac_f32 v5, v205, v81\n" \
  "v_fmac_f32 v5, v204, v75\n" \
  "v_fmac_f32 v5, v203, v69\n" \
  "v_fmac_f32 v5, v202, v7\n" \
  "v_fmac_f32 v5, v201, v6\n" \
  "v_fmac_f32 v80, v200, v7\n" \
  "v_fmac_f32 v80, v199, v6\n" \
  "v_fmac_f32 v80, v198, v5\n" \
  "v_fmac_f32 v74, v197, v80\n" \
  "v_fmac_f32 v79, v196, v6\n" \
  "v_fmac_f32 v79, v193, v80\n" \
  "v_pk_fma_f32 v[78:79], v[194:195], v[6:7], v[78:79] op_sel:[0,0,0] op_sel_hi:[1,1,1] neg_lo:[0,0,0] neg_hi:[0,0,0]\n" \
  "v_fmac_f32 v78, v192, v80\n" \
  "v_fmac_f32 v78, v191, v79\n" \
  "v_fmac_f32 v41, v190, v80\n" \
// ... 1776 lines not shown
```

### robobee3d_amd/csrc/umpc_step_asm.h

```cpp
#pragma once
#include <stddef.h>
#include <stdint.h>
namespace umpcasm {
struct StepParams {
  const void *state;
  const void *ctrl;
  const void *ref;
  const void *ws;
  const void *out;
  const void *stats;
  const void *status;
  const void *info;
  const void *Ib;
  const void *gain;
  const void *aT0;
  const void *taskf;
  const void *weights;
  const void *wl;
  const void *wlu;
  const void *wlw;
  const void *done;
  int32_t stride;
  int32_t K;
  int32_t maxIter;
// ... 2043 lines not shown
  "v_fma_f32 v16, v2, v16, v16\n" \
  "v_add_f32 v3, s24, v103\n" \
  "v_rcp_f32 v17, v3\n" \
  "s_nop 0\n" \
  "v_fma_f32 v2, -v3, v17, 1.0\n" \
  "v_fma_f32 v17, v2, v17, v17\n" \
  "v_mov_b32 v103, s26\n" \
  "v_mul_f32 v3, -1.0, v103\n" \
  "v_mul_f32 v18, -v116, v7\n" \
  "v_fmac_f32 v3, v116, v18\n" \
  "v_rcp_f32 v19, v3\n" \
  "s_nop 0\n" \
  "v_fma_f32 v2, -v3, v19, 1.0\n" \
  "v_fma_f32 v19, v2, v19, v19\n" \
  "v_mul_f32 v3, -1.0, v103\n" \
  "v_mul_f32 v116, -v117, v8\n" \
  "v_fmac_f32 v3, v117, v116\n" \
  "v_rcp_f32 v117, v3\n" \
  "s_nop 0\n" \
  "v_fma_f32 v2, -v3, v117, 1.0\n" \
  "v_fma_f32 v117, v2, v117, v117\n" \
  "v_mul_f32 v3, -1.0, v103\n" \
  "v_mul_f32 v20, -v120, v9\n" \
  "v_fmac_f32 v3, v120, v20\n" \
  "v_rcp_f32 v21, v3\n" \
  "s_nop 0\n" \
  "v_fma_f32 v2, -v3, v21, 1.0\n" \
  "v_fma_f32 v21, v2, v21, v21\n" \
  "v_mul_f32 v3, -1.0, v103\n" \
  "v_rcp_f32 v120, v3\n" \
  "s_nop 0\n" \
  "v_fma_f32 v2, -v3, v120, 1.0\n" \
  "v_fma_f32 v120, v2, v120, v120\n" \
  "v_mul_f32 v3, -1.0, v103\n" \
  "v_rcp_f32 v22, v3\n" \
  "s_nop 0\n" \
  "v_fma_f32 v2, -v3, v22, 1.0\n" \
  "v_fma_f32 v22, v2, v22, v22\n" \
  "v_mul_f32 v3, -1.0, v103\n" \
  "v_rcp_f32 v23, v3\n" \
  "s_nop 0\n" \
  "v_fma_f32 v2, -v3, v23, 1.0\n" \
  "v_fma_f32 v23, v2, v23, v23\n" \
  "v_mul_f32 v3, -1.0, v103\n" \
  "v_mul_f32 v24, -v184, v79\n" \
  "v_fmac_f32 v3, v184, v24\n" \
  "v_mul_f32 v25, -v142, v82\n" \
  "v_fmac_f32 v3, v142, v25\n" \
  "v_mul_f32 v142, -v132, v72\n" \
  "v_fmac_f32 v3, v132, v142\n" \
  "v_rcp_f32 v132, v3\n" \
  "s_nop 0\n" \
  "v_fma_f32 v2, -v3, v132, 1.0\n" \
  "v_fma_f32 v132, v2, v132, v132\n" \
  "ds_write_b32 v1, v25 offset:0\n" \
  "v_accvgpr_write_b32 a53, v82\n" \
  "v_mul_f32 v3, -1.0, v103\n" \
  "v_mul_f32 v25, -v185, v14\n" \
  "v_fmac_f32 v3, v185, v25\n" \
  "v_mul_f32 v82, -v143, v83\n" \
  "v_fmac_f32 v3, v143, v82\n" \
  "v_mul_f32 v143, -v133, v10\n" \
  "v_fmac_f32 v3, v133, v143\n" \
  "v_rcp_f32 v133, v3\n" \
  "s_nop 0\n" \
  "v_fma_f32 v2, -v3, v133, 1.0\n" \
// ... 2600 lines not shown
  "v_accvgpr_read_b32 v180, a6\n" \
  "v_accvgpr_read_b32 v181, a7\n" \
  "v_accvgpr_read_b32 v182, a8\n" \
  "v_accvgpr_read_b32 v183, a9\n" \
  "v_accvgpr_read_b32 v184, a10\n" \
  "v_accvgpr_read_b32 v185, a11\n" \
  "v_accvgpr_read_b32 v186, a12\n" \
  "v_accvgpr_read_b32 v187, a13\n" \
  "v_accvgpr_read_b32 v188, a14\n" \
  "v_accvgpr_read_b32 v189, a15\n" \
  "v_accvgpr_read_b32 v190, a16\n" \
  "v_accvgpr_read_b32 v191, a17\n" \
  "v_accvgpr_read_b32 v192, a18\n" \
  "v_accvgpr_read_b32 v193, a19\n" \
  "v_accvgpr_read_b32 v194, a20\n" \
  "v_accvgpr_read_b32 v195, a21\n" \
  "v_accvgpr_read_b32 v196, a22\n" \
  "v_accvgpr_read_b32 v197, a23\n" \
  "v_accvgpr_read_b32 v198, a24\n" \
  "v_accvgpr_read_b32 v199, a25\n" \
  "v_accvgpr_read_b32 v200, a26\n" \
  "v_accvgpr_read_b32 v201, a27\n" \
  "v_accvgpr_read_b32 v202, a28\n" \
  "v_accvgpr_read_b32 v203, a29\n" \
  "v_accvgpr_read_b32 v204, a30\n" \
  "v_accvgpr_read_b32 v205, a31\n" \
  "v_accvgpr_read_b32 v206, a32\n" \
  "v_accvgpr_read_b32 v207, a33\n" \
  "v_accvgpr_read_b32 v208, a34\n" \
  "v_accvgpr_read_b32 v209, a35\n" \
  "s_sub_i32 s14, s11, 1\n" \
  "s_cmp_lt_i32 s14, 1\n" \
  "s_cbranch_scc1 30f\n" \
  "29:\n" \
  "v_accvgpr_read_b32 v230, a137\n" \
  "v_accvgpr_read_b32 v231, a138\n" \
  "v_accvgpr_read_b32 v232, a139\n" \
  "v_accvgpr_read_b32 v233, a142\n" \
  "v_accvgpr_read_b32 v234, a140\n" \
  "v_accvgpr_read_b32 v235, a141\n" \
  "v_pk_fma_f32 v[2:3], s[24:25], v[88:89], v[230:231] op_sel:[0,0,0] op_sel_hi:[0,1,1] neg_lo:[0,0,1] neg_hi:[0,0,1]\n" \
  "v_accvgpr_read_b32 v236, a143\n" \
  "v_accvgpr_read_b32 v237, a144\n" \
  "v_pk_fma_f32 v[4:5], s[24:25], v[90:91], v[232:233] op_sel:[0,0,0] op_sel_hi:[0,1,1] neg_lo:[0,0,1] neg_hi:[0,0,1]\n" \
  "v_accvgpr_read_b32 v230, a145\n" \
  "v_accvgpr_read_b32 v231, a148\n" \
  "v_pk_fma_f32 v[6:7], s[24:25], v[92:93], v[234:235] op_sel:[0,0,0] op_sel_hi:[0,1,1] neg_lo:[0,0,1] neg_hi:[0,0,1]\n" \
  "v_accvgpr_read_b32 v232, a146\n" \
  "v_accvgpr_read_b32 v233, a147\n" \
  "v_pk_fma_f32 v[8:9], s[24:25], v[94:95], v[236:237] op_sel:[0,0,0] op_sel_hi:[0,1,1] neg_lo:[0,0,1] neg_hi:[0,0,1]\n" \
  "v_accvgpr_read_b32 v234, a149\n" \
  "v_accvgpr_read_b32 v235, a150\n" \
  "v_pk_fma_f32 v[10:11], s[24:25], v[96:97], v[230:231] op_sel:[0,0,0] op_sel_hi:[0,1,1] neg_lo:[0,0,1] neg_hi:[0,0,1]\n" \
  "v_accvgpr_read_b32 v236, a151\n" \
  "v_accvgpr_read_b32 v237, a154\n" \
  "v_pk_fma_f32 v[12:13], s[24:25], v[98:99], v[232:233] op_sel:[0,0,0] op_sel_hi:[0,1,1] neg_lo:[0,0,1] neg_hi:[0,0,1]\n" \
  "v_accvgpr_read_b32 v230, a152\n" \
  "v_accvgpr_read_b32 v231, a153\n" \
  "v_pk_fma_f32 v[14:15], s[24:25], v[100:101], v[234:235] op_sel:[0,0,0] op_sel_hi:[0,1,1] neg_lo:[0,0,1] neg_hi:[0,0,1]\n" \
  "v_accvgpr_read_b32 v232, a155\n" \
  "v_accvgpr_read_b32 v233, a156\n" \
  "v_pk_fma_f32 v[16:17], s[24:25], v[102:103], v[236:237] op_sel:[0,0,0] op_sel_hi:[0,1,1] neg_lo:[0,0,1] neg_hi:[0,0,1]\n" \
  "v_accvgpr_read_b32 v234, a157\n" \
  "v_pk_fma_f32 v[18:19], s[24:25], v[104:105], v[230:231] op_sel:[0,0,0] op_sel_hi:[0,1,1] neg_lo:[0,0,1] neg_hi:[0,0,1]\n" \
  "v_pk_fma_f32 v[20:21], s[24:25], v[106:107], v[232:233] op_sel:[0,0,0] op_sel_hi:[0,1,1] neg_lo:[0,0,1] neg_hi:[0,0,1]\n" \
  "v_accvgpr_read_b32 v236, a161\n" \
  "v_accvgpr_read_b32 v237, a162\n" \
  "v_pk_mul_f32 v[22:23], s[24:25], v[108:109] op_sel:[0,0] op_sel_hi:[0,1] neg_lo:[0,0] neg_hi:[0,0]\n" \
  "v_sub_f32 v22, v22, v234\n" \
  "v_accvgpr_read_b32 v230, a163\n" \
  "v_pk_mul_f32 v[24:25], s[24:25], v[110:111] op_sel:[0,0] op_sel_hi:[0,1] neg_lo:[0,0] neg_hi:[0,0]\n" \
  "v_pk_fma_f32 v[26:27], s[24:25], v[112:113], v[236:237] op_sel:[0,0,0] op_sel_hi:[0,1,1] neg_lo:[0,0,1] neg_hi:[0,0,1]\n" \
  "v_accvgpr_read_b32 v232, a167\n" \
  "v_accvgpr_read_b32 v233, a168\n" \
  "v_pk_mul_f32 v[28:29], s[24:25], v[114:115] op_sel:[0,0] op_sel_hi:[0,1] neg_lo:[0,0] neg_hi:[0,0]\n" \
  "v_sub_f32 v28, v28, v230\n" \
  "v_accvgpr_read_b32 v234, a169\n" \
  "v_pk_mul_f32 v[30:31], s[24:25], v[116:117] op_sel:[0,0] op_sel_hi:[0,1] neg_lo:[0,0] neg_hi:[0,0]\n" \
  "v_pk_fma_f32 v[32:33], s[24:25], v[118:119], v[232:233] op_sel:[0,0,0] op_sel_hi:[0,1,1] neg_lo:[0,0,1] neg_hi:[0,0,1]\n" \
  "v_pk_mul_f32 v[34:35], s[24:25], v[120:121] op_sel:[0,0] op_sel_hi:[0,1] neg_lo:[0,0] neg_hi:[0,0]\n" \
  "v_sub_f32 v34, v34, v234\n" \
  "v_pk_mul_f32 v[36:37], s[24:25], v[122:123] op_sel:[0,0] op_sel_hi:[0,1] neg_lo:[0,0] neg_hi:[0,0]\n" \
  "v_pk_mul_f32 v[38:39], s[24:25], v[124:125] op_sel:[0,0] op_sel_hi:[0,1] neg_lo:[0,0] neg_hi:[0,0]\n" \
  "v_pk_mul_f32 v[40:41], s[24:25], v[126:127] op_sel:[0,0] op_sel_hi:[0,1] neg_lo:[0,0] neg_hi:[0,0]\n" \
  "v_pk_mul_f32 v[42:43], s[24:25], v[128:129] op_sel:[0,0] op_sel_hi:[0,1] neg_lo:[0,0] neg_hi:[0,0]\n" \
  "v_accvgpr_read_b32 v236, a182\n" \
  "v_accvgpr_read_b32 v237, a183\n" \
  "v_pk_mul_f32 v[44:45], s[24:25], v[130:131] op_sel:[0,0] op_sel_hi:[0,1] neg_lo:[0,0] neg_hi:[0,0]\n" \
  "v_accvgpr_read_b32 v230, a184\n" \
  "v_accvgpr_read_b32 v231, a187\n" \
  "v_mul_f32 v46, s24, v132\n" \
  "v_accvgpr_read_b32 v232, a185\n" \
  "v_accvgpr_read_b32 v233, a186\n" \
  "v_pk_fma_f32 v[48:49], s[26:27], v[134:135], v[236:237] op_sel:[0,0,0] op_sel_hi:[0,1,1] neg_lo:[1,0,0] neg_hi:[1,0,0]\n" \
  "ds_read_b128 v[214:217], v1 offset:0\n" \
  "v_pk_fma_f32 v[50:51], s[26:27], v[136:137], v[230:231] op_sel:[0,0,0] op_sel_hi:[0,1,1] neg_lo:[1,0,0] neg_hi:[1,0,0]\n" \
  "v_pk_fma_f32 v[52:53], s[26:27], v[138:139], v[232:233] op_sel:[0,0,0] op_sel_hi:[0,1,1] neg_lo:[1,0,0] neg_hi:[1,0,0]\n" \
  "ds_read_b128 v[218:221], v1 offset:1024\n" \
  "v_pk_mul_f32 v[54:55], s[26:27], v[140:141] op_sel:[0,0] op_sel_hi:[0,1] neg_lo:[1,0] neg_hi:[1,0]\n" \
  "v_pk_mul_f32 v[56:57], s[26:27], v[142:143] op_sel:[0,0] op_sel_hi:[0,1] neg_lo:[1,0] neg_hi:[1,0]\n" \
  "ds_read_b128 v[222:225], v1 offset:2048\n" \
  "v_pk_mul_f32 v[58:59], s[26:27], v[144:145] op_sel:[0,0] op_sel_hi:[0,1] neg_lo:[1,0] neg_hi:[1,0]\n" \
  "v_pk_mul_f32 v[60:61], s[26:27], v[146:147] op_sel:[0,0] op_sel_hi:[0,1] neg_lo:[1,0] neg_hi:[1,0]\n" \
  "v_accvgpr_read_b32 v234, a200\n" \
  "v_accvgpr_read_b32 v235, a201\n" \
  "ds_read_b128 v[226:229], v1 offset:3072\n" \
  "v_pk_mul_f32 v[62:63], s[26:27], v[148:149] op_sel:[0,0] op_sel_hi:[0,1] neg_lo:[1,0] neg_hi:[1,0]\n" \
  "v_accvgpr_read_b32 v236, a202\n" \
  "v_accvgpr_read_b32 v237, a205\n" \
  "v_pk_mul_f32 v[64:65], s[26:27], v[150:151] op_sel:[0,0] op_sel_hi:[0,1] neg_lo:[1,0] neg_hi:[1,0]\n" \
  "v_accvgpr_read_b32 v230, a203\n" \
  "v_accvgpr_read_b32 v231, a204\n" \
  "ds_read_b128 v[246:249], v1 offset:4096\n" \
  "v_pk_fma_f32 v[66:67], s[26:27], v[152:153], v[234:235] op_sel:[0,0,0] op_sel_hi:[0,1,1] neg_lo:[1,0,0] neg_hi:[1,0,0]\n" \
  "v_accvgpr_read_b32 v232, a206\n" \
  "v_accvgpr_read_b32 v233, a207\n" \
  "v_pk_fma_f32 v[68:69], s[26:27], v[154:155], v[236:237] op_sel:[0,0,0] op_sel_hi:[0,1,1] neg_lo:[1,0,0] neg_hi:[1,0,0]\n" \
  "v_accvgpr_read_b32 v234, a208\n" \
  "ds_read_b128 v[250:253], v1 offset:5120\n" \
  "v_pk_fma_f32 v[70:71], s[26:27], v[156:157], v[230:231] op_sel:[0,0,0] op_sel_hi:[0,1,1] neg_lo:[1,0,0] neg_hi:[1,0,0]\n" \
  "v_pk_fma_f32 v[72:73], s[26:27], v[158:159], v[232:233] op_sel:[0,0,0] op_sel_hi:[0,1,1] neg_lo:[1,0,0] neg_hi:[1,0,0]\n" \
  "v_pk_mul_f32 v[74:75], s[26:27], v[160:161] op_sel:[0,0] op_sel_hi:[0,1] neg_lo:[1,0] neg_hi:[1,0]\n" \
  "v_add_f32 v74, v74, v234\n" \
  "v_accvgpr_read_b32 v236, a214\n" \
  "v_pk_mul_f32 v[76:77], s[26:27], v[162:163] op_sel:[0,0] op_sel_hi:[0,1] neg_lo:[1,0] neg_hi:[1,0]\n" \
  "v_pk_mul_f32 v[78:79], s[26:27], v[164:165] op_sel:[0,0] op_sel_hi:[0,1] neg_lo:[1,0] neg_hi:[1,0]\n" \
  "v_accvgpr_read_b32 v230, a227\n" \
  "v_pk_mul_f32 v[80:81], s[26:27], v[166:167] op_sel:[0,0] op_sel_hi:[0,1] neg_lo:[1,0] neg_hi:[1,0]\n" \
  "v_add_f32 v80, v80, v236\n" \
  "v_accvgpr_read_b32 v232, a228\n" \
  "v_pk_mul_f32 v[82:83], s[26:27], v[168:169] op_sel:[0,0] op_sel_hi:[0,1] neg_lo:[1,0] neg_hi:[1,0]\n" \
  "v_accvgpr_read_b32 v234, a229\n" \
  "v_fma_f32 v84, -v230, v170, v210\n" \
  "v_fma_f32 v85, -v232, v171, v211\n" \
  "v_fma_f32 v86, -v234, v172, v212\n" \
  "s_waitcnt lgkmcnt(3)\n" \
  "v_pk_fma_f32 v[60:61], v[214:215], v[14:15], v[60:61] op_sel:[0,0,0] op_sel_hi:[1,1,1] neg_lo:[0,0,0] neg_hi:[0,0,0]\n" \
  "v_pk_fma_f32 v[62:63], v[216:217], v[16:17], v[62:63] op_sel:[0,0,0] op_sel_hi:[1,1,1] neg_lo:[0,0,0] neg_hi:[0,0,0]\n" \
  "ds_read_b128 v[214:217], v1 offset:6144\n" \
  "v_pk_fma_f32 v[64:65], v[218:219], v[18:19], v[64:65] op_sel:[0,0,0] op_sel_hi:[1,1,1] neg_lo:[0,0,0] neg_hi:[0,0,0]\n" \
  "v_pk_fma_f32 v[48:49], v[220:221], v[2:3], v[48:49] op_sel:[0,0,0] op_sel_hi:[1,1,1] neg_lo:[0,0,0] neg_hi:[0,0,0]\n" \
  "ds_read_b128 v[218:221], v1 offset:7168\n" \
  "v_pk_fma_f32 v[54:55], v[222:223], v[2:3], v[54:55] op_sel:[0,0,0] op_sel_hi:[1,1,1] neg_lo:[0,0,0] neg_hi:[0,0,0]\n" \
  "v_pk_fma_f32 v[60:61], v[224:225], v[8:9], v[60:61] op_sel:[0,0,0] op_sel_hi:[1,1,1] neg_lo:[0,0,0] neg_hi:[0,0,0]\n" \
  "ds_read_b128 v[222:225], v1 offset:8192\n" \
  "s_waitcnt lgkmcnt(3)\n" \
  "v_pk_fma_f32 v[54:55], v[226:227], v[8:9], v[54:55] op_sel:[0,0,0] op_sel_hi:[1,1,1] neg_lo:[0,0,0] neg_hi:[0,0,0]\n" \
  "v_pk_fma_f32 v[62:63], v[228:229], v[10:11], v[62:63] op_sel:[0,0,0] op_sel_hi:[1,1,1] neg_lo:[0,0,0] neg_hi:[0,0,0]\n" \
  "ds_read_b128 v[226:229], v1 offset:9216\n" \
  "v_pk_fma_f32 v[56:57], v[246:247], v[10:11], v[56:57] op_sel:[0,0,0] op_sel_hi:[1,1,1] neg_lo:[0,0,0] neg_hi:[0,0,0]\n" \
  "v_pk_fma_f32 v[64:65], v[248:249], v[12:13], v[64:65] op_sel:[0,0,0] op_sel_hi:[1,1,1] neg_lo:[0,0,0] neg_hi:[0,0,0]\n" \
  "ds_read_b128 v[246:249], v1 offset:10240\n" \
  "v_pk_fma_f32 v[58:59], v[250:251], v[12:13], v[58:59] op_sel:[0,0,0] op_sel_hi:[1,1,1] neg_lo:[0,0,0] neg_hi:[0,0,0]\n" \
  "v_pk_fma_f32 v[60:61], v[252:253], v[32:33], v[60:61] op_sel:[0,0,0] op_sel_hi:[1,1,1] neg_lo:[0,0,0] neg_hi:[0,0,0]\n" \
  "ds_read_b128 v[250:253], v1 offset:11264\n" \
  "s_waitcnt lgkmcnt(3)\n" \
  "v_pk_fma_f32 v[78:79], v[214:215], v[32:33], v[78:79] op_sel:[0,0,0] op_sel_hi:[1,1,1] neg_lo:[0,0,0] neg_hi:[0,0,0]\n" \
  "v_pk_fma_f32 v[62:63], v[216:217], v[34:35], v[62:63] op_sel:[0,0,0] op_sel_hi:[1,1,1] neg_lo:[0,0,0] neg_hi:[0,0,0]\n" \
  "ds_read_b128 v[214:217], v1 offset:12288\n" \
  "v_pk_fma_f32 v[80:81], v[218:219], v[34:35], v[80:81] op_sel:[0,0,0] op_sel_hi:[1,1,1] neg_lo:[0,0,0] neg_hi:[0,0,0]\n" \
  "v_pk_fma_f32 v[64:65], v[220:221], v[36:37], v[64:65] op_sel:[0,0,0] op_sel_hi:[1,1,1] neg_lo:[0,0,0] neg_hi:[0,0,0]\n" \
  "ds_read_b128 v[218:221], v1 offset:13312\n" \
  "v_pk_fma_f32 v[82:83], v[222:223], v[36:37], v[82:83] op_sel:[0,0,0] op_sel_hi:[1,1,1] neg_lo:[0,0,0] neg_hi:[0,0,0]\n" \
  "v_pk_fma_f32 v[24:25], v[224:225], v[52:53], v[24:25] op_sel:[0,0,0] op_sel_hi:[1,1,1] neg_lo:[0,0,0] neg_hi:[0,0,0]\n" \
  "ds_read_b128 v[222:225], v1 offset:14336\n" \
  "s_waitcnt lgkmcnt(3)\n" \
  "v_pk_fma_f32 v[6:7], v[226:227], v[52:53], v[6:7] op_sel:[0,0,0] op_sel_hi:[1,1,1] neg_lo:[0,0,0] neg_hi:[0,0,0]\n" \
  "v_pk_fma_f32 v[20:21], v[228:229], v[66:67], v[20:21] op_sel:[0,0,0] op_sel_hi:[1,1,1] neg_lo:[0,0,0] neg_hi:[0,0,0]\n" \
  "ds_read_b128 v[226:229], v1 offset:15360\n" \
  "v_pk_fma_f32 v[54:55], v[246:247], v[26:27], v[54:55] op_sel:[0,0,0] op_sel_hi:[1,1,1] neg_lo:[0,0,0] neg_hi:[0,0,0]\n" \
  "v_pk_fma_f32 v[72:73], v[248:249], v[26:27], v[72:73] op_sel:[0,0,0] op_sel_hi:[1,1,1] neg_lo:[0,0,0] neg_hi:[0,0,0]\n" \
  "ds_read_b128 v[246:249], v1 offset:16384\n" \
  "v_pk_fma_f32 v[78:79], v[250:251], v[26:27], v[78:79] op_sel:[0,0,0] op_sel_hi:[1,1,1] neg_lo:[0,0,0] neg_hi:[0,0,0]\n" \
  "v_pk_fma_f32 v[56:57], v[252:253], v[28:29], v[56:57] op_sel:[0,0,0] op_sel_hi:[1,1,1] neg_lo:[0,0,0] neg_hi:[0,0,0]\n" \
  "ds_read_b128 v[250:253], v1 offset:17408\n" \
  "s_waitcnt lgkmcnt(3)\n" \
  "v_pk_fma_f32 v[74:75], v[214:215], v[28:29], v[74:75] op_sel:[0,0,0] op_sel_hi:[1,1,1] neg_lo:[0,0,0] neg_hi:[0,0,0]\n" \
  "v_pk_fma_f32 v[80:81], v[216:217], v[28:29], v[80:81] op_sel:[0,0,0] op_sel_hi:[1,1,1] neg_lo:[0,0,0] neg_hi:[0,0,0]\n" \
  "ds_read_b128 v[214:217], v1 offset:18432\n" \
// ... 119 lines not shown
  "v_fmac_f32 v78, v188, v41\n" \
  "v_fmac_f32 v79, v189, v41\n" \
  "v_fmac_f32 v80, v190, v41\n" \
  "v_fmac_f32 v79, v191, v78\n" \
  "v_fmac_f32 v80, v192, v78\n" \
  "v_pk_fma_f32 v[6:7], v[194:195], v[78:79], v[6:7] op_sel:[0,0,0] op_sel_hi:[1,1,1] neg_lo:[0,0,0] neg_hi:[0,0,0]\n" \
  "v_fmac_f32 v80, v193, v79\n" \
  "v_fmac_f32 v6, v196, v79\n" \
  "v_fmac_f32 v80, v197, v74\n" \
  "v_fmac_f32 v5, v198, v80\n" \
  "v_fmac_f32 v6, v199, v80\n" \
  "v_fmac_f32 v7, v200, v80\n" \
  "v_fmac_f32 v6, v201, v5\n" \
  "v_fmac_f32 v7, v202, v5\n" \
  "v_fmac_f32 v69, v203, v5\n" \
  "v_fmac_f32 v75, v204, v5\n" \
  "v_fmac_f32 v81, v205, v5\n" \
  "v_fmac_f32 v7, v206, v6\n" \
  "v_fmac_f32 v69, v207, v6\n" \
  "v_fmac_f32 v75, v208, v6\n" \
  "v_accvgpr_read_b32 v236, a38\n" \
  "v_accvgpr_read_b32 v237, a39\n" \
  "v_fmac_f32 v81, v209, v6\n" \
  "v_accvgpr_read_b32 v230, a40\n" \
  "v_pk_fma_f32 v[76:77], v[254:255], v[6:7], v[76:77] op_sel:[0,0,0] op_sel_hi:[1,1,1] neg_lo:[0,0,0] neg_hi:[0,0,0]\n" \
  "v_accvgpr_read_b32 v232, a41\n" \
  "v_pk_fma_f32 v[76:77], v[236:237], v[6:7], v[76:77] op_sel:[0,1,0] op_sel_hi:[1,0,1] neg_lo:[0,0,0] neg_hi:[0,0,0]\n" \
  "v_accvgpr_read_b32 v234, a42\n" \
  "v_fmac_f32 v69, v230, v7\n" \
  "v_accvgpr_read_b32 v236, a43\n" \
  "v_fmac_f32 v75, v232, v7\n" \
  "v_accvgpr_read_b32 v230, a44\n" \
  "v_fmac_f32 v81, v234, v7\n" \
  "v_accvgpr_read_b32 v232, a45\n" \
  "v_fmac_f32 v76, v236, v69\n" \
  "v_accvgpr_read_b32 v234, a46\n" \
  "v_fmac_f32 v77, v230, v69\n" \
  "v_accvgpr_read_b32 v236, a47\n" \
  "v_fmac_f32 v75, v232, v69\n" \
  "v_accvgpr_read_b32 v230, a48\n" \
  "v_fmac_f32 v81, v234, v69\n" \
  "v_accvgpr_read_b32 v232, a49\n" \
  "v_fmac_f32 v77, v236, v76\n" \
  "v_accvgpr_read_b32 v234, a50\n" \
  "v_fmac_f32 v75, v230, v76\n" \
  "v_accvgpr_read_b32 v236, a51\n" \
  "v_fmac_f32 v81, v232, v76\n" \
  "v_accvgpr_read_b32 v230, a52\n" \
  "v_fmac_f32 v75, v234, v77\n" \
  "v_accvgpr_read_b32 v232, a62\n" \
  "v_accvgpr_read_b32 v233, a63\n" \
  "v_fmac_f32 v81, v236, v77\n" \
  "v_accvgpr_read_b32 v234, a64\n" \
  "v_accvgpr_read_b32 v235, a129\n" \
  "v_fmac_f32 v81, v230, v75\n" \
  "v_accvgpr_read_b32 v236, a130\n" \
  "v_accvgpr_read_b32 v237, a131\n" \
  "v_pk_mul_f32 v[2:3], v[2:3], v[232:233] op_sel:[0,0] op_sel_hi:[1,1] neg_lo:[0,0] neg_hi:[0,0]\n" \
  "v_accvgpr_read_b32 v230, a65\n" \
  "v_accvgpr_read_b32 v231, a66\n" \
  "v_pk_mul_f32 v[4:5], v[4:5], v[234:235] op_sel:[0,0] op_sel_hi:[1,1] neg_lo:[0,0] neg_hi:[0,0]\n" \
  "v_accvgpr_read_b32 v232, a67\n" \
  "v_accvgpr_read_b32 v233, a70\n" \
  "v_pk_mul_f32 v[6:7], v[6:7], v[236:237] op_sel:[0,0] op_sel_hi:[1,1] neg_lo:[0,0] neg_hi:[0,0]\n" \
  "v_accvgpr_read_b32 v234, a68\n" \
  "v_accvgpr_read_b32 v235, a69\n" \
  "v_pk_mul_f32 v[8:9], v[8:9], v[230:231] op_sel:[0,0] op_sel_hi:[1,1] neg_lo:[0,0] neg_hi:[0,0]\n" \
  "v_accvgpr_read_b32 v236, a53\n" \
  "v_accvgpr_read_b32 v237, a54\n" \
  "v_pk_mul_f32 v[10:11], v[10:11], v[232:233] op_sel:[0,0] op_sel_hi:[1,1] neg_lo:[0,0] neg_hi:[0,0]\n" \
  "v_accvgpr_read_b32 v230, a55\n" \
  "v_accvgpr_read_b32 v231, a58\n" \
  "v_pk_mul_f32 v[12:13], v[12:13], v[234:235] op_sel:[0,0] op_sel_hi:[1,1] neg_lo:[0,0] neg_hi:[0,0]\n" \
  "v_accvgpr_read_b32 v232, a56\n" \
  "v_accvgpr_read_b32 v233, a57\n" \
  "v_pk_mul_f32 v[14:15], v[14:15], v[236:237] op_sel:[0,0] op_sel_hi:[1,1] neg_lo:[0,0] neg_hi:[0,0]\n" \
  "v_accvgpr_read_b32 v234, a94\n" \
  "v_accvgpr_read_b32 v235, a97\n" \
  "v_pk_mul_f32 v[16:17], v[16:17], v[230:231] op_sel:[0,0] op_sel_hi:[1,1] neg_lo:[0,0] neg_hi:[0,0]\n" \
  "v_accvgpr_read_b32 v236, a100\n" \
  "v_accvgpr_read_b32 v237, a109\n" \
  "v_pk_mul_f32 v[18:19], v[18:19], v[232:233] op_sel:[0,0] op_sel_hi:[1,1] neg_lo:[0,0] neg_hi:[0,0]\n" \
  "v_accvgpr_read_b32 v230, a105\n" \
  "v_accvgpr_read_b32 v231, a107\n" \
  "v_pk_mul_f32 v[20:21], v[20:21], v[234:235] op_sel:[0,0] op_sel_hi:[1,1] neg_lo:[0,0] neg_hi:[0,0]\n" \
  "v_accvgpr_read_b32 v232, a92\n" \
  "v_accvgpr_read_b32 v233, a95\n" \
  "v_pk_mul_f32 v[22:23], v[22:23], v[236:237] op_sel:[0,0] op_sel_hi:[1,1] neg_lo:[0,0] neg_hi:[0,0]\n" \
// ... 2 lines not shown
  "v_pk_mul_f32 v[24:25], v[24:25], v[230:231] op_sel:[0,0] op_sel_hi:[1,1] neg_lo:[0,0] neg_hi:[0,0]\n" \
  "v_accvgpr_read_b32 v236, a101\n" \
  "v_accvgpr_read_b32 v237, a102\n" \
  "v_pk_mul_f32 v[26:27], v[26:27], v[232:233] op_sel:[0,0] op_sel_hi:[1,1] neg_lo:[0,0] neg_hi:[0,0]\n" \
  "v_accvgpr_read_b32 v230, a71\n" \
  "v_accvgpr_read_b32 v231, a72\n" \
  "v_pk_mul_f32 v[28:29], v[28:29], v[234:235] op_sel:[0,0] op_sel_hi:[1,1] neg_lo:[0,0] neg_hi:[0,0]\n" \
  "v_accvgpr_read_b32 v232, a73\n" \
  "v_accvgpr_read_b32 v233, a76\n" \
  "v_pk_mul_f32 v[30:31], v[30:31], v[236:237] op_sel:[0,0] op_sel_hi:[1,1] neg_lo:[0,0] neg_hi:[0,0]\n" \
  "v_accvgpr_read_b32 v234, a74\n" \
  "v_accvgpr_read_b32 v235, a75\n" \
  "v_pk_mul_f32 v[32:33], v[32:33], v[230:231] op_sel:[0,0] op_sel_hi:[1,1] neg_lo:[0,0] neg_hi:[0,0]\n" \
  "v_accvgpr_read_b32 v236, a118\n" \
  "v_accvgpr_read_b32 v237, a113\n" \
  "v_pk_mul_f32 v[34:35], v[34:35], v[232:233] op_sel:[0,0] op_sel_hi:[1,1] neg_lo:[0,0] neg_hi:[0,0]\n" \
  "v_accvgpr_read_b32 v230, a114\n" \
  "v_accvgpr_read_b32 v231, a119\n" \
  "v_pk_mul_f32 v[36:37], v[36:37], v[234:235] op_sel:[0,0] op_sel_hi:[1,1] neg_lo:[0,0] neg_hi:[0,0]\n" \
  "v_accvgpr_read_b32 v232, a115\n" \
  "v_accvgpr_read_b32 v233, a116\n" \
  "v_pk_mul_f32 v[38:39], v[38:39], v[236:237] op_sel:[0,0] op_sel_hi:[1,1] neg_lo:[0,0] neg_hi:[0,0]\n" \
  "v_accvgpr_read_b32 v234, a117\n" \
  "v_accvgpr_read_b32 v235, a123\n" \
  "v_pk_mul_f32 v[40:41], v[40:41], v[230:231] op_sel:[0,0] op_sel_hi:[1,1] neg_lo:[0,0] neg_hi:[0,0]\n" \
  "v_accvgpr_read_b32 v236, a124\n" \
  "v_pk_mul_f32 v[42:43], v[42:43], v[232:233] op_sel:[0,0] op_sel_hi:[1,1] neg_lo:[0,0] neg_hi:[0,0]\n" \
  "v_accvgpr_read_b32 v230, a77\n" \
  "v_accvgpr_read_b32 v231, a78\n" \
  "v_pk_mul_f32 v[44:45], v[44:45], v[234:235] op_sel:[0,0] op_sel_hi:[1,1] neg_lo:[0,0] neg_hi:[0,0]\n" \
  "v_accvgpr_read_b32 v232, a79\n" \
  "v_accvgpr_read_b32 v233, a82\n" \
  "v_mul_f32 v46, v236, v46\n" \
  "v_accvgpr_read_b32 v234, a80\n" \
  "v_accvgpr_read_b32 v235, a81\n" \
  "v_pk_mul_f32 v[48:49], v[48:49], v[230:231] op_sel:[0,0] op_sel_hi:[1,1] neg_lo:[0,0] neg_hi:[0,0]\n" \
  "v_accvgpr_read_b32 v236, a93\n" \
  "v_accvgpr_read_b32 v237, a96\n" \
  "v_pk_mul_f32 v[50:51], v[50:51], v[232:233] op_sel:[0,0] op_sel_hi:[1,1] neg_lo:[0,0] neg_hi:[0,0]\n" \
  "v_accvgpr_read_b32 v230, a99\n" \
  "v_accvgpr_read_b32 v231, a108\n" \
  "v_pk_mul_f32 v[52:53], v[52:53], v[234:235] op_sel:[0,0] op_sel_hi:[1,1] neg_lo:[0,0] neg_hi:[0,0]\n" \
  "v_accvgpr_read_b32 v232, a104\n" \
  "v_accvgpr_read_b32 v233, a106\n" \
  "v_pk_mul_f32 v[54:55], v[54:55], v[236:237] op_sel:[0,0] op_sel_hi:[1,1] neg_lo:[0,0] neg_hi:[0,0]\n" \
  "v_accvgpr_read_b32 v234, a83\n" \
  "v_accvgpr_read_b32 v235, a84\n" \
  "v_pk_mul_f32 v[56:57], v[56:57], v[230:231] op_sel:[0,0] op_sel_hi:[1,1] neg_lo:[0,0] neg_hi:[0,0]\n" \
  "v_accvgpr_read_b32 v236, a85\n" \
  "v_accvgpr_read_b32 v237, a88\n" \
  "v_pk_mul_f32 v[58:59], v[58:59], v[232:233] op_sel:[0,0] op_sel_hi:[1,1] neg_lo:[0,0] neg_hi:[0,0]\n" \
  "v_accvgpr_read_b32 v230, a86\n" \
  "v_accvgpr_read_b32 v231, a87\n" \
  "v_pk_mul_f32 v[60:61], v[60:61], v[234:235] op_sel:[0,0] op_sel_hi:[1,1] neg_lo:[0,0] neg_hi:[0,0]\n" \
  "v_accvgpr_read_b32 v232, a89\n" \
  "v_accvgpr_read_b32 v233, a90\n" \
  "v_pk_mul_f32 v[62:63], v[62:63], v[236:237] op_sel:[0,0] op_sel_hi:[1,1] neg_lo:[0,0] neg_hi:[0,0]\n" \
  "v_accvgpr_read_b32 v234, a91\n" \
  "v_accvgpr_read_b32 v235, a132\n" \
  "v_pk_mul_f32 v[64:65], v[64:65], v[230:231] op_sel:[0,0] op_sel_hi:[1,1] neg_lo:[0,0] neg_hi:[0,0]\n" \
  "v_accvgpr_read_b32 v236, a125\n" \
  "v_accvgpr_read_b32 v237, a127\n" \
  "v_pk_mul_f32 v[66:67], v[66:67], v[232:233] op_sel:[0,0] op_sel_hi:[1,1] neg_lo:[0,0] neg_hi:[0,0]\n" \
  "v_accvgpr_read_b32 v230, a110\n" \
  "v_accvgpr_read_b32 v231, a111\n" \
  "v_pk_mul_f32 v[68:69], v[68:69], v[234:235] op_sel:[0,0] op_sel_hi:[1,1] neg_lo:[0,0] neg_hi:[0,0]\n" \
  "v_accvgpr_read_b32 v232, a112\n" \
  "v_accvgpr_read_b32 v233, a135\n" \
  "v_pk_mul_f32 v[70:71], v[70:71], v[236:237] op_sel:[0,0] op_sel_hi:[1,1] neg_lo:[0,0] neg_hi:[0,0]\n" \
  "v_accvgpr_read_b32 v234, a133\n" \
  "v_accvgpr_read_b32 v235, a134\n" \
  "v_pk_mul_f32 v[72:73], v[72:73], v[230:231] op_sel:[0,0] op_sel_hi:[1,1] neg_lo:[0,0] neg_hi:[0,0]\n" \
  "v_accvgpr_read_b32 v236, a120\n" \
  "v_accvgpr_read_b32 v237, a121\n" \
  "v_pk_mul_f32 v[74:75], v[74:75], v[232:233] op_sel:[0,0] op_sel_hi:[1,1] neg_lo:[0,0] neg_hi:[0,0]\n" \
  "v_accvgpr_read_b32 v230, a122\n" \
  "v_accvgpr_read_b32 v231, a136\n" \
  "v_pk_mul_f32 v[76:77], v[76:77], v[234:235] op_sel:[0,0] op_sel_hi:[1,1] neg_lo:[0,0] neg_hi:[0,0]\n" \
  "v_accvgpr_read_b32 v232, a126\n" \
  "v_accvgpr_read_b32 v233, a128\n" \
  "v_pk_mul_f32 v[78:79], v[78:79], v[236:237] op_sel:[0,0] op_sel_hi:[1,1] neg_lo:[0,0] neg_hi:[0,0]\n" \
  "v_accvgpr_read_b32 v234, a59\n" \
  "v_accvgpr_read_b32 v235, a60\n" \
  "v_pk_mul_f32 v[80:81], v[80:81], v[230:231] op_sel:[0,0] op_sel_hi:[1,1] neg_lo:[0,0] neg_hi:[0,0]\n" \
  "v_accvgpr_read_b32 v236, a61\n" \
  "v_pk_mul_f32 v[82:83], v[82:83], v[232:233] op_sel:[0,0] op_sel_hi:[1,1] neg_lo:[0,0] neg_hi:[0,0]\n" \
  "v_accvgpr_read_b32 v230, a52\n" \
  "v_pk_mul_f32 v[84:85], v[84:85], v[234:235] op_sel:[0,0] op_sel_hi:[1,1] neg_lo:[0,0] neg_hi:[0,0]\n" \
  "v_accvgpr_read_b32 v232, a51\n" \
  "v_mul_f32 v86, v236, v86\n" \
  "v_accvgpr_read_b32 v234, a50\n" \
  "v_fmac_f32 v75, v230, v81\n" \
  "v_accvgpr_read_b32 v236, a49\n" \
  "v_fmac_f32 v77, v232, v81\n" \
  "v_accvgpr_read_b32 v230, a48\n" \
  "v_fmac_f32 v77, v234, v75\n" \
  "v_accvgpr_read_b32 v232, a47\n" \
  "v_fmac_f32 v76, v236, v81\n" \
  "v_accvgpr_read_b32 v234, a46\n" \
  "v_fmac_f32 v76, v230, v75\n" \
  "v_accvgpr_read_b32 v236, a45\n" \
  "v_fmac_f32 v76, v232, v77\n" \
  "v_accvgpr_read_b32 v230, a44\n" \
  "v_fmac_f32 v69, v234, v81\n" \
  "v_accvgpr_read_b32 v232, a43\n" \
  "v_fmac_f32 v69, v236, v75\n" \
  "v_accvgpr_read_b32 v234, a42\n" \
  "v_fmac_f32 v69, v230, v77\n" \
  "v_accvgpr_read_b32 v236, a41\n" \
  "v_fmac_f32 v69, v232, v76\n" \
  "v_accvgpr_read_b32 v230, a40\n" \
  "v_fmac_f32 v7, v234, v81\n" \
  "v_accvgpr_read_b32 v232, a39\n" \
  "v_accvgpr_read_b32 v233, a38\n" \
  "v_fmac_f32 v7, v236, v75\n" \
  "v_fmac_f32 v7, v230, v69\n" \
  "v_pk_fma_f32 v[6:7], v[232:233], v[76:77], v[6:7] op_sel:[0,1,0] op_sel_hi:[1,0,1] neg_lo:[0,0,0] neg_hi:[0,0,0]\n" \
  "v_pk_fma_f32 v[6:7], v[254:255], v[76:77], v[6:7] op_sel:[0,0,0] op_sel_hi:[1,1,1] neg_lo:[0,0,0] neg_hi:[0,0,0]\n" \
  "v_fmac_f32 v6, v209, v81\n" \
  "v_fmac_f32 v6, v208, v75\n" \
  "v_fmac_f32 v6, v207, v69\n" \
  "v_fmac_f32 v6, v206, v7\n" \
  "v_fmac_f32 v5, v205, v81\n" \
  "v_fmac_f32 v5, v204, v75\n" \
  "v_fmac_f32 v5, v203, v69\n" \
  "v_fmac_f32 v5, v202, v7\n" \
  "v_fmac_f32 v5, v201, v6\n" \
  "v_fmac_f32 v80, v200, v7\n" \
  "v_fmac_f32 v80, v199, v6\n" \
  "v_fmac_f32 v80, v198, v5\n" \
  "v_fmac_f32 v74, v197, v80\n" \
  "v_fmac_f32 v79, v196, v6\n" \
  "v_fmac_f32 v79, v193, v80\n" \
  "v_pk_fma_f32 v[78:79], v[194:195], v[6:7], v[78:79] op_sel:[0,0,0] op_sel_hi:[1,1,1] neg_lo:[0,0,0] neg_hi:[0,0,0]\n" \
  "v_fmac_f32 v78, v192, v80\n" \
  "v_fmac_f32 v78, v191, v79\n" \
  "v_fmac_f32 v41, v190, v80\n" \
  "v_fmac_f32 v41, v189, v79\n" \
  "v_fmac_f32 v41, v188, v78\n" \
  "v_fmac_f32 v38, v187, v80\n" \
  "v_fmac_f32 v38, v186, v79\n" \
  "v_fmac_f32 v38, v185, v78\n" \
  "v_fmac_f32 v38, v184, v41\n" \
  "v_fmac_f32 v83, v183, v81\n" \
  "v_fmac_f32 v83, v182, v76\n" \
  "v_fmac_f32 v83, v181, v6\n" \
  "v_fmac_f32 v74, v180, v41\n" \
  "v_fmac_f32 v74, v179, v38\n" \
  "v_fmac_f32 v73, v178, v41\n" \
  "v_fmac_f32 v73, v177, v38\n" \
// ... 3972 lines not shown
```

### robobee3d_amd/isasim.py

```python
import functools
import re
from fractions import Fraction

import numpy as np

f32, f64, u32, u64 = np.float32, np.float64, np.uint32, np.uint64
POISON = 0x7ff8dead
VCC = 106
LANE_LDS_VGPR = 1


class AddressFault(Exception):
    """A simulated global access outside every array handed to the interpreter (on the GPU: a memory access fault)."""


class Quad:

    def __init__(self, v=(), a=(), lds=(), dead_v=(), dead_a=(), dead_lds=()):
        self.v, self.a, self.lds = list(v), list(a), list(lds)
        self.dead_v, self.dead_a, self.dead_lds = list(dead_v), list(dead_a), list(dead_lds)


_REG = re.compile(r"([vas])(\d+)$|([vas])\[(\d+):(\d+)\]$")


@functools.lru_cache(maxsize=None)
def _decode(x):
    if isinstance(x, float):
        return ("f", x, 1, False, False)
    if isinstance(x, (int, np.integer)):
        return ("i", int(x), 1, False, False)
    neg = x.startswith("-")
# ... 427 lines not shown
    "s_sub_i32": lambda mc, t: _sdst(mc, t, mc.s32(t[2]) - mc.s32(t[3])),
    "s_lshl_b32": lambda mc, t: _sdst(mc, t, mc.s32(t[2]) << (mc.s32(t[3]) & 31)),
    "s_cmp_lt_i32": lambda mc, t: setattr(mc, "scc", int(_signed(mc.s32(t[1])) < _signed(mc.s32(t[2])))),
    "s_cmp_gt_i32": lambda mc, t: setattr(mc, "scc", int(_signed(mc.s32(t[1])) > _signed(mc.s32(t[2])))),
    "s_cmp_lt_u32": lambda mc, t: setattr(mc, "scc", int(mc.s32(t[1]) < mc.s32(t[2]))),
    "s_cmp_gt_u32": lambda mc, t: setattr(mc, "scc", int(mc.s32(t[1]) > mc.s32(t[2]))),
    "s_cselect_b32": lambda mc, t: _sdst(mc, t, mc.s32(t[2]) if mc.scc else mc.s32(t[3])),
    "s_cmp_lg_u32": lambda mc, t: setattr(mc, "scc", int(mc.s32(t[1]) != mc.s32(t[2]))),
    "s_cmp_eq_u32": lambda mc, t: setattr(mc, "scc", int(mc.s32(t[1]) == mc.s32(t[2]))),
    "s_cmp_eq_u64": lambda mc, t: setattr(mc, "scc", int(mc.s64(t[1]) == mc.s64(t[2]))),
    "s_and_b64": _s_logic(lambda a, b: a & b),
    "s_or_b64": _s_logic(lambda a, b: a | b),
    "s_andn2_b64": _s_logic(lambda a, b: a & ~b),
    "s_and_saveexec_b64": _s_and_saveexec,
    "s_branch": _cbranch(lambda mc: True),
    "s_cbranch_scc1": _cbranch(lambda mc: mc.scc),
    "s_cbranch_scc0": _cbranch(lambda mc: not mc.scc),
    "s_cbranch_vccz": _cbranch(lambda mc: (mc.S[VCC] | mc.S[VCC + 1]) == 0),
    "s_cbranch_vccnz": _cbranch(lambda mc: (mc.S[VCC] | mc.S[VCC + 1]) != 0),
    "s_cbranch_execz": _cbranch(lambda mc: not mc.exec.any()),
}
for _n in (1, 2, 4, 8, 16):
    SALU["s_load_dword" + ("x%d" % _n if _n > 1 else "")] = _s_load


def _f32op(op, dpp=False):
    def f(mc, t):
        srcs = t[2:-1] if dpp else t[2:]
        vals = [mc.f(srcs[0], t[-1] if dpp else None)] + [mc.f(x) for x in srcs[1:]]
        mc.wf(t[1], op(*vals))
    return f


def _fma32(a, b, c):
    return (a.astype(f64) * b.astype(f64) + c.astype(f64)).astype(f32)


def _fmac(dpp=False):
    def f(mc, t):
        a = mc.f(t[2], t[4] if dpp else None)
        mc.wf(t[1], _fma32(a, mc.f(t[3]), mc.f(t[1])))
    return f


def _nanless(red):
    def f(a, b, c):
        out = np.empty_like(a)
        for ln in range(len(a)):
            vals = [x for x in (a[ln], b[ln], c[ln]) if x == x]
            out[ln] = red(vals) if vals else f32(np.nan)
        return out
    return f


def _f64op(op):
    def f(mc, t):
        mc.wd(t[1], op(*[mc.d(x) for x in t[2:]]))
    return f


def _fma64(a, b, c):
    out = a * b + c
    for ln in range(len(a)):
        if np.isfinite(a[ln]) and np.isfinite(b[ln]) and np.isfinite(c[ln]):
            out[ln] = float(Fraction(float(a[ln])) * Fraction(float(b[ln])) + Fraction(float(c[ln])))
    return out
# ... 92 lines not shown
    return lambda mc, t: mc.write(t[1], op(mc.bits(t[2]).astype(u64), mc.bits(t[3]).astype(u64)).astype(u32))


VECTOR = {
    "v_mov_b32": lambda mc, t: mc.write(t[1], mc.bits(t[2])),
    "v_mov_b32_dpp": lambda mc, t: mc.write(t[1], mc.bits(t[2], t[3])),
    "v_accvgpr_read_b32": lambda mc, t: mc.write(t[1], mc.bits(t[2])),
    "v_accvgpr_write_b32": lambda mc, t: mc.write(t[1], mc.bits(t[2])),
    "v_readfirstlane_b32": _readfirstlane,
    "v_pk_mov_b32": _pk_mov,
    "v_add_u32": _bitop(lambda a, b: (a + b) & u64(0xFFFFFFFF)),
    "v_and_b32": _bitop(lambda a, b: a & b),
    "v_or_b32": _bitop(lambda a, b: a | b),
    "v_lshrrev_b32": _bitop(lambda a, b: b >> (a & u64(31))),
    "v_mul_u32_u24": _bitop(lambda a, b: ((a & u64(0xFFFFFF)) * (b & u64(0xFFFFFF))) & u64(0xFFFFFFFF)),
    "v_bfe_u32": lambda mc, t: mc.write(t[1], (mc.bits(t[2]) >> u32(t[3] & 31)) & u32((1 << t[4]) - 1)),
    "v_cvt_f32_i32": lambda mc, t: mc.wf(t[1], mc.bits(t[2]).view(np.int32).astype(f32)),
    "v_fma_f32": _f32op(_fma32),
    "v_fmac_f32": _fmac(),
    "v_fmac_f32_dpp": _fmac(True),
    "v_fmaak_f32": lambda mc, t: mc.wf(t[1], _fma32(mc.f(t[2]), mc.f(t[3]), mc.f(t[4]))),
    "v_mul_f32": _f32op(lambda a, b: a * b),
    "v_mul_f32_dpp": _f32op(lambda a, b: a * b, True),
    "v_add_f32": _f32op(lambda a, b: a + b),
    "v_add_f32_dpp": _f32op(lambda a, b: a + b, True),
    "v_sub_f32": _f32op(lambda a, b: a - b),
    "v_subrev_f32": _f32op(lambda a, b: b - a),
    "v_max_f32": _f32op(_fmax),
    "v_max_f32_dpp": _f32op(_fmax, True),
    "v_min_f32": _f32op(_fmin),
    "v_max3_f32": _f32op(_nanless(max)),
    "v_min3_f32": _f32op(_nanless(min)),
    "v_med3_f32": _f32op(lambda a, b, c: np.sort(np.stack([a, b, c]), 0)[1]),
    "v_rcp_f32": _f32op(lambda a: f32(1.0) / a),
    "v_rsq_f32": _f32op(lambda a: (1.0 / np.sqrt(a.astype(f64))).astype(f32)),
    "v_sqrt_f32": _f32op(lambda a: np.sqrt(a.astype(f64)).astype(f32)),
    "v_pk_fma_f32": _pk("fma"),
    "v_pk_mul_f32": _pk("mul"),
    "v_pk_add_f32": _pk("add"),
    "v_cndmask_b32": _cndmask,
    "v_cndmask_b32_e64": _cndmask,
    "v_fma_f64": _f64op(_fma64),
    "v_mul_f64": _f64op(lambda a, b: a * b),
    "v_add_f64": _f64op(lambda a, b: a + b),
    "v_max_f64": _f64op(_fmax),
    "v_min_f64": _f64op(_fmin),
    "v_rcp_f64": _f64op(lambda a: 1.0 / a),
    "v_rsq_f64": _f64op(lambda a: 1.0 / np.sqrt(a)),
    "v_cmp_nlt_f64": _cmp("f64"),
    "v_cmp_eq_i32_e64": _cmp("int"),
    "v_cmp_ne_u32": _cmp("int"),
}
for _op in ("lt", "le", "gt", "ge", "eq", "nlt", "neq", "u"):
    VECTOR["v_cmp_%s_f32" % _op] = VECTOR["v_cmp_%s_f32_e64" % _op] = _cmp("f32")
OPS = dict(SALU, **VECTOR)
for _m in ("ds_read_b32", "ds_read_b64", "ds_read_b128", "ds_write_b32", "ds_write_b64", "ds_write_b128", "ds_min_f32",
           "global_load_dword", "global_load_dwordx2", "global_load_dwordx4", "global_store_dword", "global_store_dwordx2"):
    OPS[_m] = _ds if _m.startswith("ds_") else _global
```

Baseline: 537.9 million.

## Carry LDS ring and held AGPR reads across ADMM loop iterations; use uniform pivots

The middle ADMM loop body now reaches a steady ring state that is prefetched once before the loop. This removes per-iteration LDS reloads of the first ring quads. Forward-solve accumulator values are kept in spare VGPRs so the backward pass reuses them instead of re-reading AGPRs. Pivots whose inverse is uniform across lanes are broadcast through an SGPR, replacing per-lane diagonal AGPR reads. It also adds a chip-backed unary op hook for the simulator. The risks are wrong results if the ring state or held registers are not loop-invariant, or if the uniform-pivot assumption fails.

```diff
diff --git a/robobee3d_amd/_lib.py b/robobee3d_amd/_lib.py
--- a/robobee3d_amd/_lib.py
+++ b/robobee3d_amd/_lib.py
@@ -7,6 +7,7 @@
 SO_PATH = os.path.join(HERE, "libumpc_mi355x.so")
 SRC = os.path.join(HERE, "csrc", "umpc_mi355x.hip")
 SRC_BQP = os.path.join(HERE, "csrc", "umpc_bqp.hip")
+SRC_CHIP = os.path.join(HERE, "csrc", "umpc_chipops.hip")
 OBJ_DIR = os.path.join(HERE, "csrc", "_obj")
 HIPCC_FLAGS = ["--offload-arch=gfx950", "-O3", "-ffp-contract=off", "-fPIC", "-std=c++17"]
 
@@ -127,7 +128,8 @@
     hdr = os.path.join(ROOT, "include", "umpc_mi355x.h")
     csrc = os.path.join(HERE, "csrc")
     units = [(SRC, [gen, gasm, gasm64, gasm64q, gstep, gquad, gn3, hdr] + [os.path.join(csrc, f) for f in ("umpc_step.h", "umpc_models.h", "umpc_err.h")]),
-             (SRC_BQP, [hdr, greg, os.path.join(csrc, "umpc_bqp_common.h"), os.path.join(csrc, "umpc_err.h")])]
+             (SRC_BQP, [hdr, greg, os.path.join(csrc, "umpc_bqp_common.h"), os.path.join(csrc, "umpc_err.h")]),
+             (SRC_CHIP, [os.path.join(csrc, "umpc_err.h")])]
     gen_hdrs = [os.path.join(csrc, "gen", f) for f in os.listdir(os.path.join(csrc, "gen")) if f.endswith(".h")]
     units += [(u, [os.path.join(csrc, "umpc_bqp_common.h")] + gen_hdrs) for u in gqp_units]
     os.makedirs(OBJ_DIR, exist_ok=True)
@@ -278,6 +280,17 @@
     return _lib
 
 
+def chip_unary(name, a):
+    import numpy as np
+    a = np.ascontiguousarray(a, np.float32)
+    out = np.empty_like(a)
+    L = lib()
+    L.umpc_test_chip_unary_f32.argtypes = [C.c_int, C.c_int, C.c_void_p, C.c_void_p]
+    if L.umpc_test_chip_unary_f32(("v_rcp_f32", "v_rsq_f32", "v_sqrt_f32").index(name), a.size, a.ctypes.data, out.ctypes.data):
+        raise RuntimeError(L.umpcLastError().decode())
+    return out
+
+
 def default_params():
     p = BatchParams()
     lib().umpcBatchDefaultParams(C.byref(p))
diff --git a/robobee3d_amd/asmgen.py b/robobee3d_amd/asmgen.py
--- a/robobee3d_amd/asmgen.py
+++ b/robobee3d_amd/asmgen.py
@@ -16,6 +16,9 @@
 def switch_banner():
     sw = generator_switches()
     return "// generator switches: " + (" ".join("%s=%s" % kv for kv in sw.items()) if sw else "none (defaults = the shipped kernels)")
+
+OPT_TURN = os.environ.get("UMPC_ASM_TURN", "1") == "1"
+OPT_UPIV = os.environ.get("UMPC_ASM_UPIV", "1") == "1"
 
 XV_COUNT, XV_BASE = 0, 246
 NLDS = 160
@@ -28,6 +31,7 @@
 V_W, V_WZ, V_X, V_Y, V_Z = 2, 48, 88, 134, 174
 V_RING, V_AT, V_TT, V_END = 214, 230, 238, 246
 N_ATP = 4
+N_HOLD = V_END - V_TT
 NRING = 4
 
 
@@ -74,7 +78,7 @@
             ws, j = 0, k + 1
             while j < len(ins) and ws < WIDE_STORE_WAIT:
                 u = ins[j]
-                if u[0] == "label":
+                if u[0] in ("label", "kill"):
                     j += 1
                     continue
                 if u[0] == "s_nop":
@@ -97,7 +101,9 @@
         dst = valu_dst(t)
         if dst:
             ws = 0
-            for u in reversed(self.ins[-(WIDE_STORE_WAIT + 1):]):
+            for u in reversed(self.ins):
+                if u[0] == "kill":
+                    continue
                 if ws >= WIDE_STORE_WAIT or u[0] == "label":
                     break
                 if u[0] in WIDE_STORES and _vgprs(u[WIDE_STORES[u[0]]]) & dst:
@@ -274,6 +280,18 @@
     return solve_plan(symbolic.analyse(N, perm))[2]
 
 
+def uniform_pivots(s):
+    neq = 2 * s.N * symbolic.NY
+    rows = set(s.L_i)
+    out = []
+    for fo in s.factor_ops:
+        src = s.K_src[fo["diag"]]
+        assert (fo["k"] not in rows) == (not fo["elim"])
+        if fo["k"] not in rows and src[0] == "R" and src[1] < neq:
+            out.append(fo["k"])
+    return out
+
+
 def prologue(e, s):
     import numpy as np
     for reg, val in ((S_ALPHA, 1.6), (S_OMA, float(np.float32(1.0) - np.float32(1.6))), (S_SIGMA, 1e-6),
@@ -320,12 +338,16 @@
         self.lds_ahead = int(os.environ.get("UMPC_ASM_LDS_AHEAD", "12" if NRING == 4 else "20"))
         self.merge = int(os.environ.get("UMPC_ASM_LDS_MERGE", "1" if NRING == 4 else "2"))
 
-    def run(self, ops):
-        e = self.e
+    @staticmethod
+    def allocate(ops, init=None):
         n = len(ops)
         inst_of = [None] * n
         insts = []
         slots = [None] * NRING
+        for sl, qd in enumerate(init or ()):
+            if qd is not None:
+                insts.append(dict(quad=qd, first=None, last=-1, slot=sl, prev=None, issued=-1))
+                slots[sl] = len(insts) - 1
         for i, op in enumerate(ops):
             if op["src"] and op["src"][0] == "L":
                 qd = op["src"][1] // 4
@@ -339,6 +361,59 @@
                 insts.append(dict(quad=qd, first=i, last=i, slot=sl, prev=slots[sl], issued=None))
                 slots[sl] = len(insts) - 1
                 inst_of[i] = slots[sl]
+        return insts, inst_of, [None if k is None else insts[k]["quad"] for k in slots]
+
+    @classmethod
+    def hold_state(cls, ops):
+        state = cls.allocate(ops)[2]
+        for _ in range(8):
+            end = cls.allocate(ops, state)[2]
+            if end == state:
+                return state
+            state = end
+        return None
+
+    @staticmethod
+    def prefetch(e, state):
+        for sl, qd in enumerate(state):
+            if qd is not None:
+                e("ds_read_b128", "v[%d:%d]" % (ring_base(sl), ring_base(sl) + 3), "v1", qd * 1024)
+        e("s_waitcnt", "lgkmcnt(0)")
+
+    @staticmethod
+    def agpr_holds(ops, nhold):
+        isa = lambda op: op["src"] and op["src"][0] in ("A", "A2")
+        back = [i for i, op in enumerate(ops) if op.get("ph") == "bwd" and isa(op)]
+        home, owner, nreg = {}, {}, 0
+        for i in [i for i, op in enumerate(ops) if op.get("ph") == "fwd" and isa(op)][::-1]:
+            words = ops[i]["src"][1:]
+            at = nreg + nreg % 2 if len(words) == 2 else nreg
+            if at + len(words) > min(nhold, V_END - V_TT):
+                break
+            for h, a in enumerate(words):
+                home[a], owner[a] = V_TT + at + h, i
+            nreg = at + len(words)
+        if not home or not back:
+            return {}, {}
+        assert max(owner.values()) < min(back)
+        held, reuse = {}, {}
+        for i in back:
+            src = ops[i]["src"]
+            if any(a not in home for a in src[1:]):
+                continue
+            t = home[src[1]]
+            if src[0] == "A2" and not (t % 2 == 0 and home[src[2]] == t + 1):
+                continue
+            reuse[i] = t
+            for a in src[1:]:
+                held[owner[a]] = home[ops[owner[a]]["src"][1]]
+        return held, reuse
+
+    def run(self, ops, init=None, nhold=0):
+        e = self.e
+        n = len(ops)
+        insts, inst_of, _ = self.allocate(ops, init)
+        held, reuse = self.agpr_holds(ops, nhold)
 
         def issue(it):
             e("ds_read_b128", "v[%d:%d]" % (ring_base(it["slot"]), ring_base(it["slot"]) + 3), "v1",
@@ -346,16 +421,21 @@
             it["issued"] = self.nds
             self.nds += 1
 
-        next_inst = 0
+        next_inst = sum(1 for it in insts if it["first"] is None)
         atemp = {}
         next_acc = 0
         acc_rr = 0
         for i in range(n):
             while next_acc < n and next_acc < i + self.la:
                 op = ops[next_acc]
-                if op["src"] and op["src"][0] in ("A", "A2"):
-                    t = V_AT + 2 * (acc_rr % N_ATP)
-                    acc_rr += 1
+                if next_acc in reuse:
+                    atemp[next_acc] = reuse[next_acc]
+                elif op["src"] and op["src"][0] in ("A", "A2"):
+                    if next_acc in held:
+                        t = held[next_acc]
+                    else:
+                        t = V_AT + 2 * (acc_rr % N_ATP)
+                        acc_rr += 1
                     e("v_accvgpr_read_b32", "v%d" % t, "a%d" % op["src"][1])
                     if op["src"][0] == "A2":
                         e("v_accvgpr_read_b32", "v%d" % (t + 1), "a%d" % op["src"][2])
@@ -431,7 +511,8 @@
     return out
 
 
-def body(e, s, first, capture, plan, lv=False, delta_in_w=False, qzero=frozenset(), lzero=frozenset(), dy3_in_w=False):
+def body(e, s, first, capture, plan, lv=False, delta_in_w=False, qzero=frozenset(), lzero=frozenset(), dy3_in_w=False,
+         turn=False, peel=False, dunif=None):
     nx, nc, nk = s.nx, s.nc, s.nk
     neq = 2 * s.N * symbolic.NY
     xs, zs, xinv, zinv = slot_maps(s)
@@ -454,10 +535,17 @@
     f = Fetcher(e)
     ops = []
 
+    phase = ["rhs"]
+
     def op(src, fn, w=(), r=()):
-        ops.append(dict(src=src, emit=fn, w=frozenset(w), r=frozenset(r)))
+        ops.append(dict(src=src, emit=fn, w=frozenset(w), r=frozenset(r), ph=phase[0]))
 
     assert NVZ == neq and not (lv and first)
+    assert not turn or (lv and not capture), "turn-around reuse is for the middle body"
+    dunif = dunif or {}
+    e_out = e
+    if peel:
+        e = Emit()
 
     def l_src(j):
         if lpos[j] < NLDS:
@@ -548,18 +636,36 @@
                 src = ("A2", A_L + lpos[j0] - NLDS, A_L + lpos[j1] - NLDS)
                 op(src, lambda t, rd=rd, srcp=srcp: pk(e, "v_pk_fma_f32", rd, [_vp(t), srcp, _vp(rd)], [0, 0, 0]), **rw)
 
+    phase[0] = "fwd"
     solve_ops(fwd)
+    phase[0] = "diag"
     kof = {wreg(k): k for k in range(nk)}
     for r0 in range(V_W, V_Z, 2):
         k0, k1 = kof.get(r0), kof.get(r0 + 1)
-        if k0 is not None and k1 is not None:
+        if k0 is not None and k1 is not None and k0 in dunif and dunif[k0] == dunif.get(k1):
+            op(None, lambda t, r0=r0, sr=dunif[k0]: pk(e, "v_pk_mul_f32", r0, [_vp(r0), _sb(sr)]), w=(r0, r0 + 1), r=(r0, r0 + 1))
+        elif (k0 is None) != (k1 is None) and (k0 if k0 is not None else k1) in dunif:
+            k, r = (k0, r0) if k0 is not None else (k1, r0 + 1)
+            op(None, lambda t, r=r, sr=dunif[k]: e("v_mul_f32", v(r), "s%d" % sr, v(r)), w=(r,), r=(r,))
+        elif k0 is not None and k1 is not None:
             op(("A2", A_D + k0, A_D + k1), lambda t, r0=r0: pk(e, "v_pk_mul_f32", r0, [_vp(r0), _vp(t)]),
                w=(r0, r0 + 1), r=(r0, r0 + 1))
         elif k0 is not None or k1 is not None:
             k, r = (k0, r0) if k0 is not None else (k1, r0 + 1)
             op(("A", A_D + k), lambda t, r=r: e("v_mul_f32", v(r), v(t), v(r)), w=(r,), r=(r,))
+    phase[0] = "bwd"
     solve_ops(bwd)
-    f.run(despace(ops) if os.environ.get("UMPC_ASM_DESPACE", "0") == "1" else ops)
+    if turn:
+        state = Fetcher.hold_state(ops)
+        if peel:
+            if state:
+                Fetcher.prefetch(e_out, state)
+            return
+        f.run(ops, init=state, nhold=N_HOLD)
+        for r in range(V_AT, V_END):
+            e("kill", "v%d" % r)
+    else:
+        f.run(despace(ops) if os.environ.get("UMPC_ASM_DESPACE", "0") == "1" else ops)
     for p_ in range(0, nx - 1, 2):
         t = V_TT + 2 * ((p_ // 2) % 4)
         pk(e, "v_pk_mul_f32", t, [_sb(S_OMA), _vp(V_X + p_)])
@@ -653,12 +759,17 @@
     e("s_sub_i32", "s%d" % S_CNT, "s%d" % S_ITERS, 2)
     e("s_cmp_lt_i32", "s%d" % S_CNT, 1)
     e("s_cbranch_scc1", "8f")
+    if OPT_TURN:
+        body(e, s, first=False, capture=False, plan=plan, lv=True, turn=True, peel=True)
     e("label", "7")
-    body(e, s, first=False, capture=False, plan=plan, lv=True)
+    body(e, s, first=False, capture=False, plan=plan, lv=True, turn=OPT_TURN)
     e("s_sub_i32", "s%d" % S_CNT, "s%d" % S_CNT, 1)
     e("s_cmp_gt_i32", "s%d" % S_CNT, 0)
     e("s_cbranch_scc1", "7b")
     e("label", "8")
+    if OPT_TURN:
+        for r in range(V_RING, V_AT):
+            e("kill", "v%d" % r)
     e("s_cmp_lt_i32", "s%d" % S_ITERS, 2)
     e("s_cbranch_scc1", "6f")
     body(e, s, first=False, capture=True, plan=plan, lv=True)
@@ -693,6 +804,7 @@
 def write(path=None, N=3, perm=None):
     path = path or os.path.join(HERE, "csrc", "umpc_admm_asm.h")
     ins, s = program(N, perm)
+    ins = [t for t in ins if t[0] != "kill"]
     lpos = solve_plan(s)[2]
     store_l = " ".join("LDSW_(%d) = -LX_(%d);" % (lpos[j], j) if lpos[j] < NLDS else "ROW_(%d) = -LX_(%d);" % (FAC_L + lpos[j], j)
                        for j in range(len(lpos)))
diff --git a/robobee3d_amd/asmstep.py b/robobee3d_amd/asmstep.py
--- a/robobee3d_amd/asmstep.py
+++ b/robobee3d_amd/asmstep.py
@@ -32,6 +32,7 @@
 S_M0, S_M1, S_M2, S_M3 = 30, 32, 34, 36
 S_C = {"minscal": 16, "maxscal": 17, "c45": 18, "eps10": 19, "eps": 38, "rho": 6, "rinv": 7, "rmin": 8,
        "rmininv": 9, "infty_ms": 100, "rhotol": 101}
+S_UPIV = 62
 S_TMP = 4
 OFF = {}
 _o = 0
@@ -980,6 +981,8 @@
         asmgen.XV_COUNT, asmgen.XV_BASE = (XV_N if OPT_XV and not self.quad else 0), XV_B
         pool.reserve(246, 10)
         t = pool.get()
+        upiv = set(asmgen.uniform_pivots(s)) if asmgen.OPT_UPIV and not self.quad else set()
+        self.dunif = {}
 
         def retire_dinv(k):
             e("v_accvgpr_write_b32", "a%d" % (A_D + k), v(Dinv[k]))
@@ -1043,6 +1046,11 @@
             self.rcp_nr(di, dk, t)
             pool.free(dk)
             Dinv[k] = di
+            if k in upiv:
+                assert src[0] == 'R' and src[1] < neq and not op["elim"] and not op["init"]
+                if not self.dunif:
+                    e("v_readfirstlane_b32", sg(S_UPIV), v(di))
+                self.dunif[k] = S_UPIV
             for c in done_at.get(k, []):
                 retire_col(c)
             if k not in last_row:
@@ -1057,6 +1065,7 @@
         pool.free(self.VP + nx)
 
     _rinv_reg = None
+    dunif = None
 
     def _vconst_rinv(self):
         if self._rinv_reg is None:
@@ -1105,11 +1114,17 @@
         e("s_sub_i32", sg(S_CNT), sg(S_ITERS), 1)
         e("s_cmp_lt_i32", sg(S_CNT), 1)
         e("s_cbranch_scc1", lab6 + "f")
+        mid = dict(first=False, capture=False, plan=plan, lv=True, dy3_in_w=True, turn=asmgen.OPT_TURN, dunif=self.dunif, **zk)
+        if asmgen.OPT_TURN:
+            asmgen.body(e, s, peel=True, **mid)
         e("label", lab7)
-        asmgen.body(e, s, first=False, capture=False, plan=plan, lv=True, dy3_in_w=True, **zk)
+        asmgen.body(e, s, **mid)
         e("s_sub_i32", sg(S_CNT), sg(S_CNT), 1)
         e("s_cmp_gt_i32", sg(S_CNT), 0)
         e("s_cbranch_scc1", lab7 + "b")
+        if asmgen.OPT_TURN:
+            for r in sorted({asmgen.ring_base(sl) + w for sl in range(asmgen.NRING) for w in range(4)}):
+                e("kill", v(r))
         k = float(np.float32(1.6) / (np.float32(1.6) - np.float32(1.0)))
         e("s_mov_b32", sg(S_TMP), f32bits(k))
         nx, neq = s.nx, st.neq
@@ -2109,7 +2124,7 @@
 PBASE = 0x00007E0080000000
 
 
-def simulate(ins, arrays, ints, floats, max_exec=3000000, ptr_xform=None):
+def simulate(ins, arrays, ints, floats, max_exec=3000000, ptr_xform=None, lanes=1):
     import numpy as np
     from . import isasim
     base_of = {n: 0x00007F0080000000 + (k << 36) for k, n in enumerate(PTRS + ["impulse"])}
@@ -2131,12 +2146,18 @@
     struct.pack_into("<i", blob, OFF["impstep"], int(allints["impstep"]))
     regions = [(PBASE, 4, np.frombuffer(bytes(blob), np.uint32))] + \
         [(base_of[n], 4 if n in FLAT else STRIDE, arrays[n]) for n in PTRS + ["impulse"] if arrays.get(n) is not None]
-    m = isasim.Machine(ins, regions=regions, sgpr={S_PARAM: PBASE & 0xFFFFFFFF, S_PARAM + 1: PBASE >> 32}, vgpr={0: 0},
-                       lds=np.zeros((1, NLDS), np.uint32), max_exec=max_exec, quad=_quad())
+    m = isasim.Machine(ins, regions=regions, sgpr={S_PARAM: PBASE & 0xFFFFFFFF, S_PARAM + 1: PBASE >> 32},
+                       vgpr={0: 4 * np.arange(lanes, dtype=np.uint32)}, lanes=lanes,
+                       lds=np.zeros((lanes, NLDS), np.uint32), max_exec=max_exec, quad=_quad())
     isasim.run(m)
     simulate.last_quad_sections = {("admm" if k is None else k): n for k, n in m.sections.items()}
     simulate.last_quad_instructions = sum(m.sections.values())
     return m.nexec
+
+
+def lane_rows(a):
+    assert a.ndim == 2 and a.itemsize == 4 and a.flags["C_CONTIGUOUS"] and 4 * a.shape[1] <= STRIDE
+    return a.view("V%d" % (4 * a.shape[1])).reshape(-1)
 
 
 if __name__ == "__main__":
diff --git a/robobee3d_amd/csrc/umpc_admm_asm.h b/robobee3d_amd/csrc/umpc_admm_asm.h
--- a/robobee3d_amd/csrc/umpc_admm_asm.h
+++ b/robobee3d_amd/csrc/umpc_admm_asm.h
@@ -2501,6 +2501,11 @@
   "s_sub_i32 s14, s11, 2\n" \
   "s_cmp_lt_i32 s14, 1\n" \
   "s_cbranch_scc1 8f\n" \
+  "ds_read_b128 v[214:217], v1 offset:0\n" \
+  "ds_read_b128 v[218:221], v1 offset:1024\n" \
+  "ds_read_b128 v[222:225], v1 offset:2048\n" \
+  "ds_read_b128 v[226:229], v1 offset:3072\n" \
+  "s_waitcnt lgkmcnt(0)\n" \
   "7:\n" \
   "v_accvgpr_read_b32 v230, a137\n" \
   "v_accvgpr_read_b32 v231, a138\n" \
@@ -2603,28 +2608,24 @@
   "v_pk_fma_f32 v[64:65], s[26:27], v[150:151], v[236:237] op_sel:[0,0,0] op_sel_hi:[0,1,1] neg_lo:[1,0,0] neg_hi:[1,0,0]\n" \
   "v_accvgpr_read_b32 v234, a203\n" \
   "v_accvgpr_read_b32 v235, a204\n" \
-  "ds_read_b128 v[214:217], v1 offset:0\n" \
   "v_pk_fma_f32 v[66:67], s[26:27], v[152:153], v[230:231] op_sel:[0,0,0] op_sel_hi:[0,1,1] neg_lo:[1,0,0] neg_hi:[1,0,0]\n" \
   "v_accvgpr_read_b32 v236, a206\n" \
   "v_accvgpr_read_b32 v237, a207\n" \
   "v_pk_fma_f32 v[68:69], s[26:27], v[154:155], v[232:233] op_sel:[0,0,0] op_sel_hi:[0,1,1] neg_lo:[1,0,0] neg_hi:[1,0,0]\n" \
   "v_accvgpr_read_b32 v230, a208\n" \
   "v_accvgpr_read_b32 v231, a211\n" \
-  "ds_read_b128 v[218:221], v1 offset:1024\n" \
   "v_pk_fma_f32 v[70:71], s[26:27], v[156:157], v[234:235] op_sel:[0,0,0] op_sel_hi:[0,1,1] neg_lo:[1,0,0] neg_hi:[1,0,0]\n" \
   "v_accvgpr_read_b32 v232, a209\n" \
   "v_accvgpr_read_b32 v233, a210\n" \
   "v_pk_fma_f32 v[72:73], s[26:27], v[158:159], v[236:237] op_sel:[0,0,0] op_sel_hi:[0,1,1] neg_lo:[1,0,0] neg_hi:[1,0,0]\n" \
   "v_accvgpr_read_b32 v234, a212\n" \
   "v_accvgpr_read_b32 v235, a213\n" \
-  "ds_read_b128 v[222:225], v1 offset:2048\n" \
   "v_pk_fma_f32 v[74:75], s[26:27], v[160:161], v[230:231] op_sel:[0,0,0] op_sel_hi:[0,1,1] neg_lo:[1,0,0] neg_hi:[1,0,0]\n" \
   "v_accvgpr_read_b32 v236, a214\n" \
   "v_accvgpr_read_b32 v237, a217\n" \
   "v_pk_fma_f32 v[76:77], s[26:27], v[162:163], v[232:233] op_sel:[0,0,0] op_sel_hi:[0,1,1] neg_lo:[1,0,0] neg_hi:[1,0,0]\n" \
   "v_accvgpr_read_b32 v230, a215\n" \
   "v_accvgpr_read_b32 v231, a216\n" \
-  "ds_read_b128 v[226:229], v1 offset:3072\n" \
   "v_pk_fma_f32 v[78:79], s[26:27], v[164:165], v[234:235] op_sel:[0,0,0] op_sel_hi:[0,1,1] neg_lo:[1,0,0] neg_hi:[1,0,0]\n" \
   "v_accvgpr_read_b32 v232, a227\n" \
   "v_pk_fma_f32 v[80:81], s[26:27], v[166:167], v[236:237] op_sel:[0,0,0] op_sel_hi:[0,1,1] neg_lo:[1,0,0] neg_hi:[1,0,0]\n" \
@@ -2634,14 +2635,12 @@
   "v_fma_f32 v84, -v232, v170, v210\n" \
   "v_fma_f32 v85, -v234, v171, v211\n" \
   "v_fma_f32 v86, -v236, v172, v212\n" \
-  "s_waitcnt lgkmcnt(2)\n" \
   "v_pk_fma_f32 v[60:61], v[214:215], v[14:15], v[60:61] op_sel:[0,0,0] op_sel_hi:[1,1,1] neg_lo:[0,0,0] neg_hi:[0,0,0]\n" \
   "v_pk_fma_f32 v[62:63], v[216:217], v[16:17], v[62:63] op_sel:[0,0,0] op_sel_hi:[1,1,1] neg_lo:[0,0,0] neg_hi:[0,0,0]\n" \
   "ds_read_b128 v[214:217], v1 offset:4096\n" \
   "v_pk_fma_f32 v[64:65], v[218:219], v[18:19], v[64:65] op_sel:[0,0,0] op_sel_hi:[1,1,1] neg_lo:[0,0,0] neg_hi:[0,0,0]\n" \
   "v_pk_fma_f32 v[48:49], v[220:221], v[2:3], v[48:49] op_sel:[0,0,0] op_sel_hi:[1,1,1] neg_lo:[0,0,0] neg_hi:[0,0,0]\n" \
   "ds_read_b128 v[218:221], v1 offset:5120\n" \
-  "s_waitcnt lgkmcnt(2)\n" \
   "v_pk_fma_f32 v[54:55], v[222:223], v[2:3], v[54:55] op_sel:[0,0,0] op_sel_hi:[1,1,1] neg_lo:[0,0,0] neg_hi:[0,0,0]\n" \
   "v_pk_fma_f32 v[60:61], v[224:225], v[8:9], v[60:61] op_sel:[0,0,0] op_sel_hi:[1,1,1] neg_lo:[0,0,0] neg_hi:[0,0,0]\n" \
   "ds_read_b128 v[222:225], v1 offset:6144\n" \
@@ -2841,28 +2840,28 @@
   "v_fmac_f32 v75, v236, v7\n" \
   "v_accvgpr_read_b32 v234, a44\n" \
   "v_fmac_f32 v81, v230, v7\n" \
-  "v_accvgpr_read_b32 v236, a45\n" \
+  "v_accvgpr_read_b32 v245, a45\n" \
   "v_fmac_f32 v76, v232, v69\n" \
-  "v_accvgpr_read_b32 v230, a46\n" \
+  "v_accvgpr_read_b32 v244, a46\n" \
   "v_fmac_f32 v77, v234, v69\n" \
-  "v_accvgpr_read_b32 v232, a47\n" \
-  "v_fmac_f32 v75, v236, v69\n" \
-  "v_accvgpr_read_b32 v234, a48\n" \
-  "v_fmac_f32 v81, v230, v69\n" \
-  "v_accvgpr_read_b32 v236, a49\n" \
-  "v_fmac_f32 v77, v232, v76\n" \
-  "v_accvgpr_read_b32 v230, a50\n" \
-  "v_fmac_f32 v75, v234, v76\n" \
-  "v_accvgpr_read_b32 v232, a51\n" \
-  "v_fmac_f32 v81, v236, v76\n" \
-  "v_accvgpr_read_b32 v234, a52\n" \
-  "v_fmac_f32 v75, v230, v77\n" \
+  "v_accvgpr_read_b32 v243, a47\n" \
+  "v_fmac_f32 v75, v245, v69\n" \
+  "v_accvgpr_read_b32 v242, a48\n" \
+  "v_fmac_f32 v81, v244, v69\n" \
+  "v_accvgpr_read_b32 v241, a49\n" \
+  "v_fmac_f32 v77, v243, v76\n" \
+  "v_accvgpr_read_b32 v240, a50\n" \
+  "v_fmac_f32 v75, v242, v76\n" \
+  "v_accvgpr_read_b32 v239, a51\n" \
+  "v_fmac_f32 v81, v241, v76\n" \
+  "v_accvgpr_read_b32 v238, a52\n" \
+  "v_fmac_f32 v75, v240, v77\n" \
   "v_accvgpr_read_b32 v236, a62\n" \
   "v_accvgpr_read_b32 v237, a63\n" \
-  "v_fmac_f32 v81, v232, v77\n" \
+  "v_fmac_f32 v81, v239, v77\n" \
   "v_accvgpr_read_b32 v230, a64\n" \
   "v_accvgpr_read_b32 v231, a129\n" \
-  "v_fmac_f32 v81, v234, v75\n" \
+  "v_fmac_f32 v81, v238, v75\n" \
   "v_accvgpr_read_b32 v232, a130\n" \
   "v_accvgpr_read_b32 v233, a131\n" \
   "v_pk_mul_f32 v[2:3], v[2:3], v[236:237] op_sel:[0,0] op_sel_hi:[1,1] neg_lo:[0,0] neg_hi:[0,0]\n" \
@@ -2984,26 +2983,18 @@
   "v_pk_mul_f32 v[80:81], v[80:81], v[234:235] op_sel:[0,0] op_sel_hi:[1,1] neg_lo:[0,0] neg_hi:[0,0]\n" \
   "v_accvgpr_read_b32 v232, a61\n" \
   "v_pk_mul_f32 v[82:83], v[82:83], v[236:237] op_sel:[0,0] op_sel_hi:[1,1] neg_lo:[0,0] neg_hi:[0,0]\n" \
-  "v_accvgpr_read_b32 v234, a52\n" \
   "v_pk_mul_f32 v[84:85], v[84:85], v[230:231] op_sel:[0,0] op_sel_hi:[1,1] neg_lo:[0,0] neg_hi:[0,0]\n" \
-  "v_accvgpr_read_b32 v236, a51\n" \
   "v_mul_f32 v86, v232, v86\n" \
-  "v_accvgpr_read_b32 v230, a50\n" \
-  "v_fmac_f32 v75, v234, v81\n" \
-  "v_accvgpr_read_b32 v232, a49\n" \
-  "v_fmac_f32 v77, v236, v81\n" \
-  "v_accvgpr_read_b32 v234, a48\n" \
-  "v_fmac_f32 v77, v230, v75\n" \
-  "v_accvgpr_read_b32 v236, a47\n" \
-  "v_fmac_f32 v76, v232, v81\n" \
-  "v_accvgpr_read_b32 v230, a46\n" \
-  "v_fmac_f32 v76, v234, v75\n" \
-  "v_accvgpr_read_b32 v232, a45\n" \
-  "v_fmac_f32 v76, v236, v77\n" \
+  "v_fmac_f32 v75, v238, v81\n" \
+  "v_fmac_f32 v77, v239, v81\n" \
+  "v_fmac_f32 v77, v240, v75\n" \
+  "v_fmac_f32 v76, v241, v81\n" \
+  "v_fmac_f32 v76, v242, v75\n" \
+  "v_fmac_f32 v76, v243, v77\n" \
   "v_accvgpr_read_b32 v234, a44\n" \
-  "v_fmac_f32 v69, v230, v81\n" \
+  "v_fmac_f32 v69, v244, v81\n" \
   "v_accvgpr_read_b32 v236, a43\n" \
-  "v_fmac_f32 v69, v232, v75\n" \
+  "v_fmac_f32 v69, v245, v75\n" \
   "v_accvgpr_read_b32 v230, a42\n" \
   "v_fmac_f32 v69, v234, v77\n" \
   "v_accvgpr_read_b32 v232, a41\n" \
diff --git a/robobee3d_amd/csrc/umpc_chipops.hip b/robobee3d_amd/csrc/umpc_chipops.hip
--- /dev/null
+++ b/robobee3d_amd/csrc/umpc_chipops.hip
@@ -0,0 +1,40 @@
+#include <hip/hip_runtime.h>
+
+#include <string>
+
+#include "umpc_err.h"
+
+namespace {
+
+__global__ void chip_unary_f32_kernel(int op, int n, const float *in, float *out) {
+  const int i = blockIdx.x * blockDim.x + threadIdx.x;
+  if (i >= n) return;
+  const float a = in[i];
+  out[i] = op == 0 ? __builtin_amdgcn_rcpf(a) : op == 1 ? __builtin_amdgcn_rsqf(a) : __builtin_amdgcn_sqrtf(a);
+}
+
+float *g_buf = nullptr;
+size_t g_cap = 0;
+
+}
+
+extern "C" __attribute__((visibility("default"))) int umpc_test_chip_unary_f32(int op, int n, const float *in, float *out) {
+  if (op < 0 || op > 2 || n <= 0 || !in || !out) { umpc_set_error("umpc_test_chip_unary_f32: bad argument"); return -1; }
+  if ((size_t)n > g_cap) {
+    if (g_buf) (void)hipFree(g_buf);
+    g_buf = nullptr;
+    g_cap = 0;
+    const size_t cap = (size_t)n < 256 ? 256 : (size_t)n;
+    if (hipMalloc((void **)&g_buf, 2 * sizeof(float) * cap) != hipSuccess) { umpc_set_error("umpc_test_chip_unary_f32: hipMalloc failed"); return -1; }
+    g_cap = cap;
+  }
+  float *d = g_buf;
+  hipError_t e = hipMemcpy(d, in, sizeof(float) * (size_t)n, hipMemcpyHostToDevice);
+  if (e == hipSuccess) {
+    hipLaunchKernelGGL(chip_unary_f32_kernel, dim3((n + 255) / 256), dim3(256), 0, 0, op, n, d, d + g_cap);
+    e = hipGetLastError();
+  }
+  if (e == hipSuccess) e = hipMemcpy(out, d + g_cap, sizeof(float) * (size_t)n, hipMemcpyDeviceToHost);
+  if (e != hipSuccess) { umpc_set_error((std::string("umpc_test_chip_unary_f32: ") + hipGetErrorString(e)).c_str()); return -1; }
+  return 0;
+}
diff --git a/robobee3d_amd/csrc/umpc_step_asm.h b/robobee3d_amd/csrc/umpc_step_asm.h
--- a/robobee3d_amd/csrc/umpc_step_asm.h
+++ b/robobee3d_amd/csrc/umpc_step_asm.h
@@ -2099,6 +2099,7 @@
   "s_nop 0\n" \
   "v_fma_f32 v2, -v3, v120, 1.0\n" \
   "v_fma_f32 v120, v2, v120, v120\n" \
+  "v_readfirstlane_b32 s62, v120\n" \
   "v_mul_f32 v3, -1.0, v103\n" \
   "v_rcp_f32 v22, v3\n" \
   "s_nop 0\n" \
@@ -4765,6 +4766,13 @@
   "s_sub_i32 s14, s11, 1\n" \
   "s_cmp_lt_i32 s14, 1\n" \
   "s_cbranch_scc1 30f\n" \
+  "ds_read_b128 v[214:217], v1 offset:0\n" \
+  "ds_read_b128 v[218:221], v1 offset:1024\n" \
+  "ds_read_b128 v[222:225], v1 offset:2048\n" \
+  "ds_read_b128 v[226:229], v1 offset:3072\n" \
+  "ds_read_b128 v[246:249], v1 offset:4096\n" \
+  "ds_read_b128 v[250:253], v1 offset:5120\n" \
+  "s_waitcnt lgkmcnt(0)\n" \
   "29:\n" \
   "v_accvgpr_read_b32 v230, a137\n" \
   "v_accvgpr_read_b32 v231, a138\n" \
@@ -4826,31 +4834,25 @@
   "v_accvgpr_read_b32 v232, a185\n" \
   "v_accvgpr_read_b32 v233, a186\n" \
   "v_pk_fma_f32 v[48:49], s[26:27], v[134:135], v[236:237] op_sel:[0,0,0] op_sel_hi:[0,1,1] neg_lo:[1,0,0] neg_hi:[1,0,0]\n" \
-  "ds_read_b128 v[214:217], v1 offset:0\n" \
   "v_pk_fma_f32 v[50:51], s[26:27], v[136:137], v[230:231] op_sel:[0,0,0] op_sel_hi:[0,1,1] neg_lo:[1,0,0] neg_hi:[1,0,0]\n" \
   "v_pk_fma_f32 v[52:53], s[26:27], v[138:139], v[232:233] op_sel:[0,0,0] op_sel_hi:[0,1,1] neg_lo:[1,0,0] neg_hi:[1,0,0]\n" \
-  "ds_read_b128 v[218:221], v1 offset:1024\n" \
   "v_pk_mul_f32 v[54:55], s[26:27], v[140:141] op_sel:[0,0] op_sel_hi:[0,1] neg_lo:[1,0] neg_hi:[1,0]\n" \
   "v_pk_mul_f32 v[56:57], s[26:27], v[142:143] op_sel:[0,0] op_sel_hi:[0,1] neg_lo:[1,0] neg_hi:[1,0]\n" \
-  "ds_read_b128 v[222:225], v1 offset:2048\n" \
   "v_pk_mul_f32 v[58:59], s[26:27], v[144:145] op_sel:[0,0] op_sel_hi:[0,1] neg_lo:[1,0] neg_hi:[1,0]\n" \
   "v_pk_mul_f32 v[60:61], s[26:27], v[146:147] op_sel:[0,0] op_sel_hi:[0,1] neg_lo:[1,0] neg_hi:[1,0]\n" \
   "v_accvgpr_read_b32 v234, a200\n" \
   "v_accvgpr_read_b32 v235, a201\n" \
-  "ds_read_b128 v[226:229], v1 offset:3072\n" \
   "v_pk_mul_f32 v[62:63], s[26:27], v[148:149] op_sel:[0,0] op_sel_hi:[0,1] neg_lo:[1,0] neg_hi:[1,0]\n" \
   "v_accvgpr_read_b32 v236, a202\n" \
   "v_accvgpr_read_b32 v237, a205\n" \
   "v_pk_mul_f32 v[64:65], s[26:27], v[150:151] op_sel:[0,0] op_sel_hi:[0,1] neg_lo:[1,0] neg_hi:[1,0]\n" \
   "v_accvgpr_read_b32 v230, a203\n" \
   "v_accvgpr_read_b32 v231, a204\n" \
-  "ds_read_b128 v[246:249], v1 offset:4096\n" \
   "v_pk_fma_f32 v[66:67], s[26:27], v[152:153], v[234:235] op_sel:[0,0,0] op_sel_hi:[0,1,1] neg_lo:[1,0,0] neg_hi:[1,0,0]\n" \
   "v_accvgpr_read_b32 v232, a206\n" \
   "v_accvgpr_read_b32 v233, a207\n" \
   "v_pk_fma_f32 v[68:69], s[26:27], v[154:155], v[236:237] op_sel:[0,0,0] op_sel_hi:[0,1,1] neg_lo:[1,0,0] neg_hi:[1,0,0]\n" \
   "v_accvgpr_read_b32 v234, a208\n" \
-  "ds_read_b128 v[250:253], v1 offset:5120\n" \
   "v_pk_fma_f32 v[70:71], s[26:27], v[156:157], v[230:231] op_sel:[0,0,0] op_sel_hi:[0,1,1] neg_lo:[1,0,0] neg_hi:[1,0,0]\n" \
   "v_pk_fma_f32 v[72:73], s[26:27], v[158:159], v[232:233] op_sel:[0,0,0] op_sel_hi:[0,1,1] neg_lo:[1,0,0] neg_hi:[1,0,0]\n" \
   "v_pk_mul_f32 v[74:75], s[26:27], v[160:161] op_sel:[0,0] op_sel_hi:[0,1] neg_lo:[1,0] neg_hi:[1,0]\n" \
@@ -4867,7 +4869,6 @@
   "v_fma_f32 v84, -v230, v170, v210\n" \
   "v_fma_f32 v85, -v232, v171, v211\n" \
   "v_fma_f32 v86, -v234, v172, v212\n" \
-  "s_waitcnt lgkmcnt(3)\n" \
   "v_pk_fma_f32 v[60:61], v[214:215], v[14:15], v[60:61] op_sel:[0,0,0] op_sel_hi:[1,1,1] neg_lo:[0,0,0] neg_hi:[0,0,0]\n" \
   "v_pk_fma_f32 v[62:63], v[216:217], v[16:17], v[62:63] op_sel:[0,0,0] op_sel_hi:[1,1,1] neg_lo:[0,0,0] neg_hi:[0,0,0]\n" \
   "ds_read_b128 v[214:217], v1 offset:6144\n" \
@@ -4877,7 +4878,6 @@
   "v_pk_fma_f32 v[54:55], v[222:223], v[2:3], v[54:55] op_sel:[0,0,0] op_sel_hi:[1,1,1] neg_lo:[0,0,0] neg_hi:[0,0,0]\n" \
   "v_pk_fma_f32 v[60:61], v[224:225], v[8:9], v[60:61] op_sel:[0,0,0] op_sel_hi:[1,1,1] neg_lo:[0,0,0] neg_hi:[0,0,0]\n" \
   "ds_read_b128 v[222:225], v1 offset:8192\n" \
-  "s_waitcnt lgkmcnt(3)\n" \
   "v_pk_fma_f32 v[54:55], v[226:227], v[8:9], v[54:55] op_sel:[0,0,0] op_sel_hi:[1,1,1] neg_lo:[0,0,0] neg_hi:[0,0,0]\n" \
   "v_pk_fma_f32 v[62:63], v[228:229], v[10:11], v[62:63] op_sel:[0,0,0] op_sel_hi:[1,1,1] neg_lo:[0,0,0] neg_hi:[0,0,0]\n" \
   "ds_read_b128 v[226:229], v1 offset:9216\n" \
@@ -5063,28 +5063,28 @@
   "v_fmac_f32 v75, v232, v7\n" \
   "v_accvgpr_read_b32 v230, a44\n" \
   "v_fmac_f32 v81, v234, v7\n" \
-  "v_accvgpr_read_b32 v232, a45\n" \
+  "v_accvgpr_read_b32 v245, a45\n" \
   "v_fmac_f32 v76, v236, v69\n" \
-  "v_accvgpr_read_b32 v234, a46\n" \
+  "v_accvgpr_read_b32 v244, a46\n" \
   "v_fmac_f32 v77, v230, v69\n" \
-  "v_accvgpr_read_b32 v236, a47\n" \
-  "v_fmac_f32 v75, v232, v69\n" \
-  "v_accvgpr_read_b32 v230, a48\n" \
-  "v_fmac_f32 v81, v234, v69\n" \
-  "v_accvgpr_read_b32 v232, a49\n" \
-  "v_fmac_f32 v77, v236, v76\n" \
-  "v_accvgpr_read_b32 v234, a50\n" \
-  "v_fmac_f32 v75, v230, v76\n" \
-  "v_accvgpr_read_b32 v236, a51\n" \
-  "v_fmac_f32 v81, v232, v76\n" \
-  "v_accvgpr_read_b32 v230, a52\n" \
-  "v_fmac_f32 v75, v234, v77\n" \
+  "v_accvgpr_read_b32 v243, a47\n" \
+  "v_fmac_f32 v75, v245, v69\n" \
+  "v_accvgpr_read_b32 v242, a48\n" \
+  "v_fmac_f32 v81, v244, v69\n" \
+  "v_accvgpr_read_b32 v241, a49\n" \
+  "v_fmac_f32 v77, v243, v76\n" \
+  "v_accvgpr_read_b32 v240, a50\n" \
+  "v_fmac_f32 v75, v242, v76\n" \
+  "v_accvgpr_read_b32 v239, a51\n" \
+  "v_fmac_f32 v81, v241, v76\n" \
+  "v_accvgpr_read_b32 v238, a52\n" \
+  "v_fmac_f32 v75, v240, v77\n" \
   "v_accvgpr_read_b32 v232, a62\n" \
   "v_accvgpr_read_b32 v233, a63\n" \
-  "v_fmac_f32 v81, v236, v77\n" \
+  "v_fmac_f32 v81, v239, v77\n" \
   "v_accvgpr_read_b32 v234, a64\n" \
   "v_accvgpr_read_b32 v235, a129\n" \
-  "v_fmac_f32 v81, v230, v75\n" \
+  "v_fmac_f32 v81, v238, v75\n" \
   "v_accvgpr_read_b32 v236, a130\n" \
   "v_accvgpr_read_b32 v237, a131\n" \
   "v_pk_mul_f32 v[2:3], v[2:3], v[232:233] op_sel:[0,0] op_sel_hi:[1,1] neg_lo:[0,0] neg_hi:[0,0]\n" \
@@ -5153,90 +5153,78 @@
   "v_accvgpr_read_b32 v232, a79\n" \
   "v_accvgpr_read_b32 v233, a82\n" \
   "v_mul_f32 v46, v236, v46\n" \
-  "v_accvgpr_read_b32 v234, a80\n" \
-  "v_accvgpr_read_b32 v235, a81\n" \
   "v_pk_mul_f32 v[48:49], v[48:49], v[230:231] op_sel:[0,0] op_sel_hi:[1,1] neg_lo:[0,0] neg_hi:[0,0]\n" \
-  "v_accvgpr_read_b32 v236, a93\n" \
-  "v_accvgpr_read_b32 v237, a96\n" \
+  "v_accvgpr_read_b32 v234, a93\n" \
+  "v_accvgpr_read_b32 v235, a96\n" \
   "v_pk_mul_f32 v[50:51], v[50:51], v[232:233] op_sel:[0,0] op_sel_hi:[1,1] neg_lo:[0,0] neg_hi:[0,0]\n" \
-  "v_accvgpr_read_b32 v230, a99\n" \
-  "v_accvgpr_read_b32 v231, a108\n" \
-  "v_pk_mul_f32 v[52:53], v[52:53], v[234:235] op_sel:[0,0] op_sel_hi:[1,1] neg_lo:[0,0] neg_hi:[0,0]\n" \
-  "v_accvgpr_read_b32 v232, a104\n" \
-  "v_accvgpr_read_b32 v233, a106\n" \
-  "v_pk_mul_f32 v[54:55], v[54:55], v[236:237] op_sel:[0,0] op_sel_hi:[1,1] neg_lo:[0,0] neg_hi:[0,0]\n" \
-  "v_accvgpr_read_b32 v234, a83\n" \
-  "v_accvgpr_read_b32 v235, a84\n" \
-  "v_pk_mul_f32 v[56:57], v[56:57], v[230:231] op_sel:[0,0] op_sel_hi:[1,1] neg_lo:[0,0] neg_hi:[0,0]\n" \
-  "v_accvgpr_read_b32 v236, a85\n" \
-  "v_accvgpr_read_b32 v237, a88\n" \
-  "v_pk_mul_f32 v[58:59], v[58:59], v[232:233] op_sel:[0,0] op_sel_hi:[1,1] neg_lo:[0,0] neg_hi:[0,0]\n" \
-  "v_accvgpr_read_b32 v230, a86\n" \
-  "v_accvgpr_read_b32 v231, a87\n" \
-  "v_pk_mul_f32 v[60:61], v[60:61], v[234:235] op_sel:[0,0] op_sel_hi:[1,1] neg_lo:[0,0] neg_hi:[0,0]\n" \
-  "v_accvgpr_read_b32 v232, a89\n" \
-  "v_accvgpr_read_b32 v233, a90\n" \
-  "v_pk_mul_f32 v[62:63], v[62:63], v[236:237] op_sel:[0,0] op_sel_hi:[1,1] neg_lo:[0,0] neg_hi:[0,0]\n" \
-  "v_accvgpr_read_b32 v234, a91\n" \
-  "v_accvgpr_read_b32 v235, a132\n" \
-  "v_pk_mul_f32 v[64:65], v[64:65], v[230:231] op_sel:[0,0] op_sel_hi:[1,1] neg_lo:[0,0] neg_hi:[0,0]\n" \
-  "v_accvgpr_read_b32 v236, a125\n" \
-  "v_accvgpr_read_b32 v237, a127\n" \
-  "v_pk_mul_f32 v[66:67], v[66:67], v[232:233] op_sel:[0,0] op_sel_hi:[1,1] neg_lo:[0,0] neg_hi:[0,0]\n" \
-  "v_accvgpr_read_b32 v230, a110\n" \
-  "v_accvgpr_read_b32 v231, a111\n" \
-  "v_pk_mul_f32 v[68:69], v[68:69], v[234:235] op_sel:[0,0] op_sel_hi:[1,1] neg_lo:[0,0] neg_hi:[0,0]\n" \
-  "v_accvgpr_read_b32 v232, a112\n" \
-  "v_accvgpr_read_b32 v233, a135\n" \
-  "v_pk_mul_f32 v[70:71], v[70:71], v[236:237] op_sel:[0,0] op_sel_hi:[1,1] neg_lo:[0,0] neg_hi:[0,0]\n" \
-  "v_accvgpr_read_b32 v234, a133\n" \
-  "v_accvgpr_read_b32 v235, a134\n" \
-  "v_pk_mul_f32 v[72:73], v[72:73], v[230:231] op_sel:[0,0] op_sel_hi:[1,1] neg_lo:[0,0] neg_hi:[0,0]\n" \
-  "v_accvgpr_read_b32 v236, a120\n" \
-  "v_accvgpr_read_b32 v237, a121\n" \
-  "v_pk_mul_f32 v[74:75], v[74:75], v[232:233] op_sel:[0,0] op_sel_hi:[1,1] neg_lo:[0,0] neg_hi:[0,0]\n" \
-  "v_accvgpr_read_b32 v230, a122\n" \
-  "v_accvgpr_read_b32 v231, a136\n" \
-  "v_pk_mul_f32 v[76:77], v[76:77], v[234:235] op_sel:[0,0] op_sel_hi:[1,1] neg_lo:[0,0] neg_hi:[0,0]\n" \
-  "v_accvgpr_read_b32 v232, a126\n" \
-  "v_accvgpr_read_b32 v233, a128\n" \
-  "v_pk_mul_f32 v[78:79], v[78:79], v[236:237] op_sel:[0,0] op_sel_hi:[1,1] neg_lo:[0,0] neg_hi:[0,0]\n" \
-  "v_accvgpr_read_b32 v234, a59\n" \
-  "v_accvgpr_read_b32 v235, a60\n" \
-  "v_pk_mul_f32 v[80:81], v[80:81], v[230:231] op_sel:[0,0] op_sel_hi:[1,1] neg_lo:[0,0] neg_hi:[0,0]\n" \
-  "v_accvgpr_read_b32 v236, a61\n" \
-  "v_pk_mul_f32 v[82:83], v[82:83], v[232:233] op_sel:[0,0] op_sel_hi:[1,1] neg_lo:[0,0] neg_hi:[0,0]\n" \
-  "v_accvgpr_read_b32 v230, a52\n" \
-  "v_pk_mul_f32 v[84:85], v[84:85], v[234:235] op_sel:[0,0] op_sel_hi:[1,1] neg_lo:[0,0] neg_hi:[0,0]\n" \
-  "v_accvgpr_read_b32 v232, a51\n" \
-  "v_mul_f32 v86, v236, v86\n" \
-  "v_accvgpr_read_b32 v234, a50\n" \
-  "v_fmac_f32 v75, v230, v81\n" \
-  "v_accvgpr_read_b32 v236, a49\n" \
-  "v_fmac_f32 v77, v232, v81\n" \
-  "v_accvgpr_read_b32 v230, a48\n" \
-  "v_fmac_f32 v77, v234, v75\n" \
-  "v_accvgpr_read_b32 v232, a47\n" \
-  "v_fmac_f32 v76, v236, v81\n" \
-  "v_accvgpr_read_b32 v234, a46\n" \
-  "v_fmac_f32 v76, v230, v75\n" \
-  "v_accvgpr_read_b32 v236, a45\n" \
-  "v_fmac_f32 v76, v232, v77\n" \
-  "v_accvgpr_read_b32 v230, a44\n" \
-  "v_fmac_f32 v69, v234, v81\n" \
-  "v_accvgpr_read_b32 v232, a43\n" \
-  "v_fmac_f32 v69, v236, v75\n" \
-  "v_accvgpr_read_b32 v234, a42\n" \
-  "v_fmac_f32 v69, v230, v77\n" \
-  "v_accvgpr_read_b32 v236, a41\n" \
-  "v_fmac_f32 v69, v232, v76\n" \
-  "v_accvgpr_read_b32 v230, a40\n" \
-  "v_fmac_f32 v7, v234, v81\n" \
-  "v_accvgpr_read_b32 v232, a39\n" \
-  "v_accvgpr_read_b32 v233, a38\n" \
-  "v_fmac_f32 v7, v236, v75\n" \
-  "v_fmac_f32 v7, v230, v69\n" \
-  "v_pk_fma_f32 v[6:7], v[232:233], v[76:77], v[6:7] op_sel:[0,1,0] op_sel_hi:[1,0,1] neg_lo:[0,0,0] neg_hi:[0,0,0]\n" \
+  "v_accvgpr_read_b32 v236, a99\n" \
+  "v_accvgpr_read_b32 v237, a108\n" \
+  "v_pk_mul_f32 v[52:53], v[52:53], s[62:63] op_sel:[0,0] op_sel_hi:[1,0] neg_lo:[0,0] neg_hi:[0,0]\n" \
+  "v_accvgpr_read_b32 v230, a104\n" \
+  "v_accvgpr_read_b32 v231, a106\n" \
+  "v_pk_mul_f32 v[54:55], v[54:55], v[234:235] op_sel:[0,0] op_sel_hi:[1,1] neg_lo:[0,0] neg_hi:[0,0]\n" \
+  "v_accvgpr_read_b32 v232, a83\n" \
+  "v_accvgpr_read_b32 v233, a84\n" \
+  "v_pk_mul_f32 v[56:57], v[56:57], v[236:237] op_sel:[0,0] op_sel_hi:[1,1] neg_lo:[0,0] neg_hi:[0,0]\n" \
+  "v_accvgpr_read_b32 v234, a85\n" \
+  "v_accvgpr_read_b32 v235, a88\n" \
+  "v_pk_mul_f32 v[58:59], v[58:59], v[230:231] op_sel:[0,0] op_sel_hi:[1,1] neg_lo:[0,0] neg_hi:[0,0]\n" \
+  "v_accvgpr_read_b32 v236, a86\n" \
+  "v_accvgpr_read_b32 v237, a87\n" \
+  "v_pk_mul_f32 v[60:61], v[60:61], v[232:233] op_sel:[0,0] op_sel_hi:[1,1] neg_lo:[0,0] neg_hi:[0,0]\n" \
+  "v_pk_mul_f32 v[62:63], v[62:63], v[234:235] op_sel:[0,0] op_sel_hi:[1,1] neg_lo:[0,0] neg_hi:[0,0]\n" \
+  "v_accvgpr_read_b32 v230, a91\n" \
+  "v_accvgpr_read_b32 v231, a132\n" \
+  "v_pk_mul_f32 v[64:65], v[64:65], v[236:237] op_sel:[0,0] op_sel_hi:[1,1] neg_lo:[0,0] neg_hi:[0,0]\n" \
+  "v_accvgpr_read_b32 v232, a125\n" \
+  "v_accvgpr_read_b32 v233, a127\n" \
+  "v_pk_mul_f32 v[66:67], v[66:67], s[62:63] op_sel:[0,0] op_sel_hi:[1,0] neg_lo:[0,0] neg_hi:[0,0]\n" \
+  "v_accvgpr_read_b32 v234, a110\n" \
+  "v_accvgpr_read_b32 v235, a111\n" \
+  "v_pk_mul_f32 v[68:69], v[68:69], v[230:231] op_sel:[0,0] op_sel_hi:[1,1] neg_lo:[0,0] neg_hi:[0,0]\n" \
+  "v_accvgpr_read_b32 v236, a112\n" \
+  "v_accvgpr_read_b32 v237, a135\n" \
+  "v_pk_mul_f32 v[70:71], v[70:71], v[232:233] op_sel:[0,0] op_sel_hi:[1,1] neg_lo:[0,0] neg_hi:[0,0]\n" \
+  "v_accvgpr_read_b32 v230, a133\n" \
+  "v_accvgpr_read_b32 v231, a134\n" \
+  "v_pk_mul_f32 v[72:73], v[72:73], v[234:235] op_sel:[0,0] op_sel_hi:[1,1] neg_lo:[0,0] neg_hi:[0,0]\n" \
+  "v_accvgpr_read_b32 v232, a120\n" \
+  "v_accvgpr_read_b32 v233, a121\n" \
+  "v_pk_mul_f32 v[74:75], v[74:75], v[236:237] op_sel:[0,0] op_sel_hi:[1,1] neg_lo:[0,0] neg_hi:[0,0]\n" \
+  "v_accvgpr_read_b32 v234, a122\n" \
+  "v_accvgpr_read_b32 v235, a136\n" \
+  "v_pk_mul_f32 v[76:77], v[76:77], v[230:231] op_sel:[0,0] op_sel_hi:[1,1] neg_lo:[0,0] neg_hi:[0,0]\n" \
+  "v_accvgpr_read_b32 v236, a126\n" \
+  "v_accvgpr_read_b32 v237, a128\n" \
+  "v_pk_mul_f32 v[78:79], v[78:79], v[232:233] op_sel:[0,0] op_sel_hi:[1,1] neg_lo:[0,0] neg_hi:[0,0]\n" \
+  "v_accvgpr_read_b32 v230, a59\n" \
+  "v_accvgpr_read_b32 v231, a60\n" \
+  "v_pk_mul_f32 v[80:81], v[80:81], v[234:235] op_sel:[0,0] op_sel_hi:[1,1] neg_lo:[0,0] neg_hi:[0,0]\n" \
+  "v_accvgpr_read_b32 v232, a61\n" \
+  "v_pk_mul_f32 v[82:83], v[82:83], v[236:237] op_sel:[0,0] op_sel_hi:[1,1] neg_lo:[0,0] neg_hi:[0,0]\n" \
+  "v_pk_mul_f32 v[84:85], v[84:85], v[230:231] op_sel:[0,0] op_sel_hi:[1,1] neg_lo:[0,0] neg_hi:[0,0]\n" \
+  "v_mul_f32 v86, v232, v86\n" \
+  "v_fmac_f32 v75, v238, v81\n" \
+  "v_fmac_f32 v77, v239, v81\n" \
+  "v_fmac_f32 v77, v240, v75\n" \
+  "v_fmac_f32 v76, v241, v81\n" \
+  "v_fmac_f32 v76, v242, v75\n" \
+  "v_fmac_f32 v76, v243, v77\n" \
+  "v_accvgpr_read_b32 v234, a44\n" \
+  "v_fmac_f32 v69, v244, v81\n" \
+  "v_accvgpr_read_b32 v236, a43\n" \
+  "v_fmac_f32 v69, v245, v75\n" \
+  "v_accvgpr_read_b32 v230, a42\n" \
+  "v_fmac_f32 v69, v234, v77\n" \
+  "v_accvgpr_read_b32 v232, a41\n" \
+  "v_fmac_f32 v69, v236, v76\n" \
+  "v_accvgpr_read_b32 v234, a40\n" \
+  "v_fmac_f32 v7, v230, v81\n" \
+  "v_accvgpr_read_b32 v236, a39\n" \
+  "v_accvgpr_read_b32 v237, a38\n" \
+  "v_fmac_f32 v7, v232, v75\n" \
+  "v_fmac_f32 v7, v234, v69\n" \
+  "v_pk_fma_f32 v[6:7], v[236:237], v[76:77], v[6:7] op_sel:[0,1,0] op_sel_hi:[1,0,1] neg_lo:[0,0,0] neg_hi:[0,0,0]\n" \
   "v_pk_fma_f32 v[6:7], v[254:255], v[76:77], v[6:7] op_sel:[0,0,0] op_sel_hi:[1,1,1] neg_lo:[0,0,0] neg_hi:[0,0,0]\n" \
   "v_fmac_f32 v6, v209, v81\n" \
   "v_fmac_f32 v6, v208, v75\n" \
diff --git a/robobee3d_amd/isasim.py b/robobee3d_amd/isasim.py
--- a/robobee3d_amd/isasim.py
+++ b/robobee3d_amd/isasim.py
@@ -1,3 +1,4 @@
+import contextlib
 import functools
 import re
 from fractions import Fraction
@@ -491,6 +492,26 @@
     return f
 
 
+_chip_unary = None
+
+
+@contextlib.contextmanager
+def chip_unary(fn):
+    global _chip_unary
+    old, _chip_unary = _chip_unary, fn
+    try:
+        yield
+    finally:
+        _chip_unary = old
+
+
+def _unary32(name, host):
+    def f(mc, t):
+        a = mc.f(t[2])
+        mc.wf(t[1], host(a) if _chip_unary is None else np.asarray(_chip_unary(name, a), f32))
+    return f
+
+
 def _fma32(a, b, c):
     return (a.astype(f64) * b.astype(f64) + c.astype(f64)).astype(f32)
 
@@ -649,9 +670,9 @@
     "v_max3_f32": _f32op(_nanless(max)),
     "v_min3_f32": _f32op(_nanless(min)),
     "v_med3_f32": _f32op(lambda a, b, c: np.sort(np.stack([a, b, c]), 0)[1]),
-    "v_rcp_f32": _f32op(lambda a: f32(1.0) / a),
-    "v_rsq_f32": _f32op(lambda a: (1.0 / np.sqrt(a.astype(f64))).astype(f32)),
-    "v_sqrt_f32": _f32op(lambda a: np.sqrt(a.astype(f64)).astype(f32)),
+    "v_rcp_f32": _unary32("v_rcp_f32", lambda a: f32(1.0) / a),
+    "v_rsq_f32": _unary32("v_rsq_f32", lambda a: (1.0 / np.sqrt(a.astype(f64))).astype(f32)),
+    "v_sqrt_f32": _unary32("v_sqrt_f32", lambda a: np.sqrt(a.astype(f64)).astype(f32)),
     "v_pk_fma_f32": _pk("fma"),
     "v_pk_mul_f32": _pk("mul"),
     "v_pk_add_f32": _pk("add"),
```

New measurement: 549.5 million, median of 6. 1.02x the previous value.
